# visinf/fldr-vfi

Hardware: AMD Instinct MI355X
Metric: 4K frame-pairs interpolated/sec (higher is better)
Workload: dtype f32 (3x3 convs: 3 x fp16-split MFMA with fp32 accumulation — error against fp64 within 1.5x (mean) / 2x (max) of the exact fp32-MFMA kernel's on every layer shape, tests/test_gpu_parity.py::test_split_fp16_conv_is_fp32_equivalent; rest fp32/fp64); 1 GPU; single 3840x2160 frame pair per step (padded 2304x3840), fLDRnet 5-scale test path (--papermodel --test5scales), t=0.5, shipped checkpoint weights, fp64 output frame; 4 distinct pairs per GPU rotated through the loop; parallelism=dp1 (independent pairs, no data-path collective), pairs_in_flight=3, distinct_pairs_per_gpu=4, setup_threads_per_rank=16, pyramid_bytes_per_pair=283046400

## Files before the change

fldr-vfi_amd/csrc/conv_ring_kernels.hip:

```cpp
#include "spk_common.h"

#ifndef RING_SLOTS
#define RING_SLOTS 3
#endif
#define RING_NLOAD 4
#define RING_RW_MAX_CHUNKS 4
#ifndef RING_RW_SLOTS
#define RING_RW_SLOTS 5
#endif
#ifndef RING_RW_INFLIGHT
#define RING_RW_INFLIGHT 2
#endif
#ifndef RING_NT_STORES
#define RING_NT_STORES 0
#endif
#ifndef RING_PD_THIN
#define RING_PD_THIN 1
#endif
#define RING_SPIN_LIMIT (1 << 21)
#ifndef RING_LOADER_PRIO
#define RING_LOADER_PRIO 0
#endif
#ifndef RING_FIN_PRIO
#define RING_FIN_PRIO 0
#endif

#ifdef RING_STAMPS
__device__ unsigned long long fldr_ring_stamp_buf[4 * 8];
__device__ unsigned long long fldr_ring_trace[4 * 24 * 4];
FLDR_HOOK int fldr_debug_read_ring_trace(unsigned long long* host) {
    return (int)hipMemcpyFromSymbol(host, HIP_SYMBOL(fldr_ring_trace), sizeof(unsigned long long) * 4 * 24 * 4);
}
#define RSTAMP(var) unsigned long long var; { __builtin_amdgcn_sched_barrier(0); asm volatile("s_memtime %0\n\ts_waitcnt lgkmcnt(0)" : "=s"(var) :: "memory"); __builtin_amdgcn_sched_barrier(0); }
FLDR_HOOK int fldr_debug_read_ring_stamps(unsigned long long* host) {
    return (int)hipMemcpyFromSymbol(host, HIP_SYMBOL(fldr_ring_stamp_buf), sizeof(unsigned long long) * 32);
}
#else
#define RSTAMP(var)
#endif

__device__ int fldr_ring_timeouts;
static int g_ring_spin_limit = RING_SPIN_LIMIT;
FLDR_HOOK int fldr_debug_ring_spin_limit(int v) {
    g_ring_spin_limit = v < 0 ? RING_SPIN_LIMIT : v;
    return g_ring_spin_limit;
}
FLDR_HOOK int fldr_debug_ring_timeouts(void) {
    int v = -1;
    if (hipMemcpyFromSymbol(&v, HIP_SYMBOL(fldr_ring_timeouts), sizeof(int)) != hipSuccess) return -1;
    return v;
}

FLDR_TU_STATUS(ring)
int fldr_ring_timeouts_read(int reset) {
    int v = -1;
    if (hipMemcpyFromSymbol(&v, HIP_SYMBOL(fldr_ring_timeouts), sizeof(int)) != hipSuccess) return -1;
    if (v > 0 && reset) { const int z = 0; if (hipMemcpyToSymbol(HIP_SYMBOL(fldr_ring_timeouts), &z, sizeof(int)) != hipSuccess) return -1; }
    return v;
}

template <int NMT, int TW = SPK_TW, bool RW = false>
struct RingCfg {
    static constexpr int W_BYTES = SPK_STEPS * NMT * 2 * 1024;
    static constexpr int NBLK = SPK_STEPS * NMT * 2;
    static constexpr int NWL = (NBLK + RING_NLOAD - 1) / RING_NLOAD;
    static constexpr int IW = TW + 2;
    static constexpr int CB = TW / 16;
    static constexpr int PLANE = (SPK_IH * IW * 16 + 255) / 256 * 256;
    static constexpr int NXI = (SPK_IH * IW + 63) / 64;
    static constexpr int K_DMA = (RW ? 0 : NWL) + NXI;
    static constexpr int IN_OFF = RW ? 0 : W_BYTES;
    static constexpr int STAGE = IN_OFF + 4 * PLANE;
    static constexpr int SLOTS = RW ? RING_RW_SLOTS : RING_SLOTS;
    static constexpr int INFLIGHT = RW ? RING_RW_INFLIGHT : 1;
    static constexpr int WRES_OFF = SLOTS * STAGE;
    static constexpr int CTR_OFF = WRES_OFF + (RW ? RING_RW_MAX_CHUNKS * W_BYTES : 0);
    static constexpr int BIAS_OFF = CTR_OFF + 64;
    static constexpr int LDS_BYTES = BIAS_OFF + 64 * NMT;
    static_assert(SLOTS <= 8 && INFLIGHT + 2 <= SLOTS && INFLIGHT * K_DMA <= 15, "ring shape");
    static_assert(TW == 16 || TW == 32, "tile width");
    static_assert(TW != SPK_TW || PLANE == SPK_PLANE, "the 32-pixel plane is the barrier pipeline's");
    static_assert(PLANE / 16 >= 64 && NXI * 64 >= SPK_IH * IW, "DMA pieces cover the plane");
    static_assert(K_DMA <= 15, "counted vmcnt wait uses the 4 low bits");
    static_assert(LDS_BYTES <= 160 * 1024, "ring does not fit the LDS");
};

__device__ __forceinline__ uint32_t ring_peek(uint32_t lds_addr) {
    uint32_t v;
    asm volatile("ds_read_b32 %0, %1\n\ts_waitcnt lgkmcnt(0)" : "=v"(v) : "v"(lds_addr) : "memory");
    return (uint32_t)__builtin_amdgcn_readfirstlane((int)v);
}

__device__ __forceinline__ void ring_wait_ge(uint32_t lds_addr, uint32_t target, int& limit) {
    if (ring_peek(lds_addr) >= target) return;
    bool landed = false;
    for (int spins = 0; spins < limit && !landed; spins += 8) {
#pragma unroll
        for (int j = 0; j < 8; ++j) {
            __builtin_amdgcn_s_sleep(1);
            if (ring_peek(lds_addr) >= target) { landed = true; break; }
        }
    }
#ifndef RING_AB_NOFAULT
    if (!landed) limit = -1;
#endif
}
__device__ __forceinline__ void ring_report_fault(int lane) {
    if (lane == 0) {
        atomicAdd(&fldr_ring_timeouts, 1);
        fldr_status_raise_ring();
    }
}

__device__ __forceinline__ void ring_signal(uint32_t lds_addr, int lane) {
    __builtin_amdgcn_sched_barrier(0);
    if (lane == 0) asm volatile("ds_add_u32 %0, %1" :: "v"(lds_addr), "v"(1u) : "memory");
    __builtin_amdgcn_sched_barrier(0);
}

template <int NMT, int TERMS, bool HAS_RES, int NC, int TW, bool ML = false, bool RW = false>
__global__ __launch_bounds__((NC + RING_NLOAD) * 64) void conv3x3_ring_kernel(SpkArgs a) {
    using Cfg = RingCfg<NMT, TW, RW>;
    constexpr int SLOTS = Cfg::SLOTS;
    constexpr int CB = Cfg::CB;
    constexpr int RING_NCONS = NC;
    constexpr int MTOT = 16 * NMT;
    extern __shared__ __attribute__((aligned(256))) unsigned char smem[];
    const int tid = threadIdx.x, lane = tid & 63;
    const int wave = __builtin_amdgcn_readfirstlane(tid >> 6);
    const int n_chunks = a.n_chunks;
    const uint32_t ctr = (uint32_t)(uintptr_t)(klptr_t)(smem + Cfg::CTR_OFF);
#ifdef RING_AB_CONSTLIMIT
    int spin_limit = RING_SPIN_LIMIT;
#else
    int spin_limit = a.spin_limit;
#endif

    if (tid < 16) reinterpret_cast<uint32_t*>(smem + Cfg::CTR_OFF)[tid] = 0u;
    if (tid >= 64 && tid < 64 + 16 * NMT) {
        const int u0 = (blockIdx.x & 7) * a.units_per_xcd + (blockIdx.x >> 3);
        int co = (u0 % a.groups) * 16 * NMT + (tid - 64);
        co = co < a.cout ? co : a.cout - 1;
        reinterpret_cast<float*>(smem + Cfg::BIAS_OFF)[tid - 64] = a.bias ? a.bias[co] : 0.0f;
    }
    const int xcd = blockIdx.x & 7, slot_id = blockIdx.x >> 3;
    const int u_end = min((xcd + 1) * a.units_per_xcd, a.n_units);
    const int u_first = xcd * a.units_per_xcd + slot_id;
    if constexpr (RW) {
        const int g0 = (u_first < a.n_units ? u_first : 0) % a.groups;
        const int sub = a.pack_nmt / NMT, pgrp = g0 / sub, msel = (g0 - pgrp * sub) * NMT;
        const int pack_w_bytes = SPK_STEPS * a.pack_nmt * 2 * 1024;
        const char* wsrc = reinterpret_cast<const char*>(a.wpack + SPK_HDR) + (int64_t)pgrp * n_chunks * pack_w_bytes;
        for (int b = wave; b < n_chunks * Cfg::NBLK; b += NC + RING_NLOAD) {
            const int c = b / Cfg::NBLK, blk = b - c * Cfg::NBLK;
            const int step = blk / (2 * NMT), mk = blk - step * 2 * NMT;
            __builtin_amdgcn_global_load_lds((kgptr_t)(wsrc + (int64_t)c * pack_w_bytes + ((step * a.pack_nmt + msel) * 2 + mk) * 1024 + lane * 16),
                                             (klptr_t)(smem + Cfg::WRES_OFF + c * Cfg::W_BYTES + blk * 1024), 16, 0, 0);
        }
        __builtin_amdgcn_s_waitcnt(0x0F70);
    }
    __syncthreads();
    if (u_first >= u_end) return;
    const int my_units = (u_end - u_first + a.wgs_per_xcd - 1) / a.wgs_per_xcd;
    const int total = my_units * n_chunks;
    const int grp0 = u_first % a.groups;

    if (wave >= RING_NCONS) {
        __builtin_amdgcn_s_setprio(RING_LOADER_PRIO);
        const int lw = wave - RING_NCONS;
        const int ip = lw, ikind = ip >> 1, igrp = ip & 1;
        const char* zero_blk = reinterpret_cast<const char*>(a.wpack + 4);
        const int sub = a.pack_nmt / NMT;
        const int pgrp = grp0 / sub, msel = (grp0 - pgrp * sub) * NMT;
        const int pack_w_bytes = SPK_STEPS * a.pack_nmt * 2 * 1024;
        int w_blk[Cfg::NWL], x_piece[Cfg::NXI];
        uint32_t w_voff[Cfg::NWL];
#pragma unroll
        for (int i = 0; i < Cfg::NWL; ++i) {
            w_blk[i] = min(lw * Cfg::NWL + i, Cfg::NBLK - 1);
            const int step = w_blk[i] / (2 * NMT), mk = w_blk[i] - step * 2 * NMT;
            w_voff[i] = (uint32_t)((step * a.pack_nmt + msel) * 2 + mk) * 1024u + (uint32_t)lane * 16u;
        }
#pragma unroll
        for (int i = 0; i < Cfg::NXI; ++i) x_piece[i] = min(i * 64, Cfg::PLANE / 16 - 64);
        unsigned long long tab_ptr;
        long long tab_bs;
        {
            const auto* kt = (const __attribute__((address_space(4))) unsigned long long*)__builtin_amdgcn_kernarg_segment_ptr();
            const int l = lane < SPK_MAX_GROUPS ? lane : 0;
            unsigned long long e = kt[l];
            tab_bs = (long long)kt[SPK_MAX_GROUPS + l];
            const bool up2 = (e & 1ull) != 0ull;
            const long long plane = up2 ? (long long)(a.H >> 1) * (a.W >> 1) * 16 : (long long)a.H * a.W * 16;
            if (e != 0ull && ikind) e += (unsigned long long)plane;
            tab_ptr = e;
        }
        int iss_u = u_first, iss_c = 0, iss_n = 0;
        uint32_t g_full[Cfg::NXI], g_half[Cfg::NXI];
        unsigned long long ml_base = 0ull;
        long long ml_plane = 0;
        auto issue_geometry = [&]() {
            int uH = a.H, uW = a.W, tiles_x = a.tiles_x, tile, ty;
            const int t = spk_div(iss_u, a.m_groups, a.groups);
            if constexpr (ML) {
                int l = 0;
                for (int k = 1; k < a.n_levels; ++k) l = t * a.groups >= a.lv[k].unit0 ? k : l;
                uH = a.lv[l].H; uW = a.lv[l].W; tiles_x = a.lv[l].tiles_x;
                tile = t - a.lv[l].unit0 / a.groups;
                iss_n = 0;
                ml_base = a.grp_ptr[0] + (unsigned long long)a.lv[l].in_off;
                ml_plane = (long long)uH * uW * 16;
                ty = tile / tiles_x;
            } else {
                iss_n = spk_div(t, a.m_tiles, a.n_tiles);
                tile = t - iss_n * a.n_tiles;
                ty = spk_div(tile, a.m_tiles_x, a.tiles_x);
            }
            const int oy0 = ty * SPK_TH, ox0 = (tile - ty * tiles_x) * TW;
#pragma unroll
            for (int i = 0; i < Cfg::NXI; ++i) {
                const int e = x_piece[i] + lane;
                const int y = e / Cfg::IW, x = e % Cfg::IW;
                const int gy = oy0 - 1 + y, gx = ox0 - 1 + x;
                const bool ok = e < SPK_IH * Cfg::IW && gy >= 0 && gy < uH && gx >= 0 && gx < uW;
                g_full[i] = ok ? (uint32_t)(gy * uW + gx) * 16u : ~0u;
                g_half[i] = ok ? (uint32_t)((gy >> 1) * (uW >> 1) + (gx >> 1)) * 16u : ~0u;
            }
        };
        const char* const iss_w = reinterpret_cast<const char*>(a.wpack + SPK_HDR) + (int64_t)pgrp * n_chunks * pack_w_bytes;
        issue_geometry();
        int st = 0;
        uint32_t free_target = 0;
#ifdef RING_STAMPS
        unsigned long long ls_prep = 0, ls_free = 0, ls_fire = 0, ls_land = 0;
        RSTAMP(l_begin)
#endif
        for (int k = 0; k < total; ++k) {
            RSTAMP(l0)
            const char* wbase = iss_w + (int64_t)iss_c * pack_w_bytes;
            const int gi = iss_c * 2 + igrp;
            const uint32_t e_lo = __builtin_amdgcn_readlane((int)(uint32_t)tab_ptr, gi), e_hi = __builtin_amdgcn_readlane((int)(uint32_t)(tab_ptr >> 32), gi);
            const uint32_t b_lo = __builtin_amdgcn_readlane((int)(uint32_t)tab_bs, gi), b_hi = __builtin_amdgcn_readlane((int)(uint32_t)((unsigned long long)tab_bs >> 32), gi);
            unsigned long long e = ((unsigned long long)e_hi << 32) | e_lo;
            const long long bs = (long long)(((unsigned long long)b_hi << 32) | b_lo);
            if constexpr (ML) e = e == 0ull ? 0ull : ml_base + (unsigned long long)((2 * gi + ikind) * ml_plane);
            const bool nul = e == 0ull, up2 = (e & 1ull) != 0ull;
            const char* base = reinterpret_cast<const char*>(static_cast<uintptr_t>(e & ~1ull)) + (int64_t)iss_n * bs;
            const char* dptr[Cfg::NXI];
#pragma unroll
            for (int i = 0; i < Cfg::NXI; ++i) {
                const uint32_t off = up2 ? g_half[i] : g_full[i];
                dptr[i] = (off != ~0u && !nul) ? base + off : zero_blk;
            }
            if (++iss_c == n_chunks) { iss_c = 0; iss_u += a.wgs_per_xcd; if (iss_u < u_end) issue_geometry(); }
            RSTAMP(l1)
            if (free_target) ring_wait_ge(ctr + 32 + 4 * st, free_target, spin_limit);
            if (spin_limit < 0) break;
            RSTAMP(l2)
            unsigned char* stage = smem + st * Cfg::STAGE;
#if defined(RING_ABLATE) && RING_ABLATE == 3
            if (k >= SLOTS) { wbase = reinterpret_cast<const char*>(a.wpack + SPK_HDR); for (int i = 0; i < Cfg::NXI; ++i) dptr[i] = zero_blk; }
#endif
            if constexpr (!RW) {
#pragma unroll
                for (int i = 0; i < Cfg::NWL; ++i)
                    __builtin_amdgcn_global_load_lds((kgptr_t)(wbase + w_voff[i]), (klptr_t)(stage + w_blk[i] * 1024), 16, 0, 0);
            }
#pragma unroll
            for (int i = 0; i < Cfg::NXI; ++i)
                __builtin_amdgcn_global_load_lds((kgptr_t)dptr[i], (klptr_t)(stage + Cfg::IN_OFF + ip * Cfg::PLANE + x_piece[i] * 16), 16, 0, 0);
            RSTAMP(l3)
            if (k >= Cfg::INFLIGHT) {
                __builtin_amdgcn_s_waitcnt(0x0F70 | (Cfg::INFLIGHT * Cfg::K_DMA));
                ring_signal(ctr + 4 * ((st + SLOTS - Cfg::INFLIGHT) % SLOTS), lane);
            }
            RSTAMP(l4)
#ifdef RING_STAMPS
            ls_prep += l1 - l0; ls_free += l2 - l1; ls_fire += l3 - l2; ls_land += l4 - l3;
            if (blockIdx.x == 0 && (lw == 0 || lw == 3) && lane == 0 && k < 24) {
                unsigned long long* tr = fldr_ring_trace + ((lw == 0 ? 2 : 3) * 24 + k) * 4;
                tr[0] = l1; tr[1] = l2; tr[2] = l3; tr[3] = l4;
            }
#endif
            if (++st == SLOTS) { st = 0; free_target += RING_NCONS; }
        }
        if (spin_limit < 0) { ring_report_fault(lane); __builtin_amdgcn_s_waitcnt(0x0F70); return; }
        if constexpr (Cfg::INFLIGHT == 2) {
            if (total >= 2) {
                __builtin_amdgcn_s_waitcnt(0x0F70 | Cfg::K_DMA);
                ring_signal(ctr + 4 * ((st + SLOTS - 2) % SLOTS), lane);
            }
        } else {
            static_assert(Cfg::INFLIGHT == 1, "drain sequence");
        }
        __builtin_amdgcn_s_waitcnt(0x0F70);
        ring_signal(ctr + 4 * ((st + SLOTS - 1) % SLOTS), lane);
#ifdef RING_STAMPS
        RSTAMP(l_end)
        if ((blockIdx.x == 0 || blockIdx.x == 101) && wave == RING_NCONS && lane == 0) {
            unsigned long long* o = fldr_ring_stamp_buf + ((blockIdx.x == 0 ? 0 : 2) + 1) * 8;
            o[0] = ls_prep; o[1] = ls_free; o[2] = ls_fire; o[3] = ls_land; o[5] = total; o[6] = l_end - l_begin;
        }
#endif
        return;
    }

    constexpr int ROWS = SPK_TH / NC;
    const int cw = wave;
    const int lj = lane & 15, lg = lane >> 4;
    constexpr int NQ = CB * ROWS;
    int boff[NQ];
#pragma unroll
    for (int q = 0; q < NQ; ++q)
        boff[q] = Cfg::IN_OFF + (lg & 1) * Cfg::PLANE + ((ROWS * cw + q / CB) * Cfg::IW + (q % CB) * 16 + lj) * 16;
    const int tap_sel = lg >> 1;
    f4 acc[NMT][NQ];
#pragma unroll
    for (int m = 0; m < NMT; ++m)
#pragma unroll
        for (int q = 0; q < NQ; ++q) acc[m][q] = f4{0.0f, 0.0f, 0.0f, 0.0f};
    int cur_u = u_first, cur_c = 0;
    const float inv_scale = a.wpack[0];
    int uH = a.H, uW = a.W;
    int64_t HW = (int64_t)a.H * a.W;
    uint32_t HW32 = (uint32_t)HW;
    int64_t u_spk_off = 0, u_f32_off = 0, u_res_off = 0;
    auto unit_decode = [&](int u, int& n, int& ty, int& tx) __attribute__((always_inline)) {
        const int t = spk_div(u, a.m_groups, a.groups);
        if constexpr (ML) {
            int l = 0;
            for (int k = 1; k < a.n_levels; ++k) l = t * a.groups >= a.lv[k].unit0 ? k : l;
            uH = a.lv[l].H; uW = a.lv[l].W; HW = (int64_t)uH * uW; HW32 = (uint32_t)HW;
            u_spk_off = a.lv[l].out_spk_off; u_f32_off = a.lv[l].out_f32_off; u_res_off = a.lv[l].res_off;
            const int tile = t - a.lv[l].unit0 / a.groups;
            n = 0; ty = tile / a.lv[l].tiles_x; tx = tile - ty * a.lv[l].tiles_x;
        } else {
            n = spk_div(t, a.m_tiles, a.n_tiles);
            const int tile = t - n * a.n_tiles;
            ty = spk_div(tile, a.m_tiles_x, a.tiles_x); tx = tile - ty * a.tiles_x;
        }
    };
    const int gout = (a.cout_store + 7) >> 3;
    const int cbase = grp0 * MTOT;
    float bias_r[NMT][4];
#pragma unroll
    for (int m = 0; m < NMT; ++m) {
        const f4 bv = *reinterpret_cast<const f4*>(smem + Cfg::BIAS_OFF + (m * 16 + lg * 4) * 4);
#pragma unroll
        for (int r = 0; r < 4; ++r) bias_r[m][r] = bv[r];
    }
    auto bias_of = [&](int m) __attribute__((always_inline)) -> f4 { return f4{bias_r[m][0], bias_r[m][1], bias_r[m][2], bias_r[m][3]}; };
    auto unit_pixels = [&](int u, uint32_t (&po)[NQ], int& n) {
        int ty, tx;
        unit_decode(u, n, ty, tx);
        const int ox0 = tx * TW;
#pragma unroll
        for (int q = 0; q < NQ; ++q) {
            const int oy = ty * SPK_TH + ROWS * cw + q / CB;
            const int ox = ox0 + (q % CB) * 16 + lj;
            po[q] = (oy < uH && ox < uW) ? (uint32_t)(oy * uW + ox) : ~0u;
        }
    };
    float res_r[HAS_RES ? NMT : 1][HAS_RES ? NQ : 1][4];
    auto residual_prefetch = [&]() {
        uint32_t po[NQ]; int n;
        unit_pixels(cur_u, po, n);
        if (a.res_spk) {
            const char* resn = reinterpret_cast<const char*>(a.residual) + u_res_off + (int64_t)n * ((a.cout_store + 7) >> 3) * 2 * HW * 16;
#pragma unroll
            for (int m = 0; m < NMT; ++m)
#pragma unroll
                for (int q = 0; q < NQ; ++q) {
                    int co0 = cbase + m * 16 + lg * 4;
                    co0 = co0 < a.cout_store ? co0 : 0;
                    const uint32_t off = ((uint32_t)(co0 >> 3) * 2u * HW32 + (po[q] != ~0u ? po[q] : 0u)) * 16u + (uint32_t)((co0 >> 2) & 1) * 8u;
                    const h4 hi = *reinterpret_cast<const h4*>(resn + off), lo = *reinterpret_cast<const h4*>(resn + (off + HW32 * 16u));
#pragma unroll
                    for (int r = 0; r < 4; ++r) res_r[HAS_RES ? m : 0][HAS_RES ? q : 0][r] = (float)hi[r] + (float)lo[r];
                }
            return;
        }
        const float* resn = reinterpret_cast<const float*>(reinterpret_cast<const char*>(a.residual) + u_res_off) + (int64_t)n * a.cout_store * HW;
#pragma unroll
        for (int m = 0; m < NMT; ++m)
#pragma unroll
            for (int q = 0; q < NQ; ++q)
#pragma unroll
                for (int r = 0; r < 4; ++r) {
                    int co = cbase + m * 16 + lg * 4 + r;
                    co = co < a.cout_store ? co : a.cout_store - 1;
                    res_r[HAS_RES ? m : 0][HAS_RES ? q : 0][r] = resn[(uint32_t)co * HW32 + (po[q] != ~0u ? po[q] : 0u)];
                }
    };
    const float relu_floor = a.relu ? 0.0f : -3.402823466e+38f;
    const bool grp_full = cbase + MTOT <= a.cout_store && !(a.cout_store & 7);
#ifdef RING_STAMPS
    unsigned long long cs_f_dec = 0, cs_f_fast = 0, cs_f_b0 = 0, fq0 = 0;
#endif
    auto finish_store = [&]() {
        RSTAMP(f0)
        int lj = lane & 15, lg = lane >> 4;
        asm volatile("" : "+v"(lj), "+v"(lg));
        int n, ty, tx;
        unit_decode(cur_u, n, ty, tx);
        const int oy0 = ty * SPK_TH + ROWS * cw, ox0 = tx * TW;
        char* outn = a.out_f32 ? reinterpret_cast<char*>(a.out_f32 + (int64_t)n * a.cout_store * HW) + u_f32_off : nullptr;
        char* spkn = a.out_spk ? reinterpret_cast<char*>(a.out_spk) + (int64_t)n * a.out_spk_bstride + u_spk_off : nullptr;
        const bool inside = oy0 + ROWS <= uH && ox0 + TW <= uW;
        const bool poisoned = spin_limit < 0;
        RSTAMP(f1)
        if (grp_full && inside) {
            const uint32_t p0 = (uint32_t)(oy0 * uW + ox0 + lj);
            float abs_sum = 0.0f;
#pragma unroll
            for (int q = 0; q < NQ; ++q)
#pragma unroll
                for (int m = 0; m < NMT; ++m) {
                    const f4 bsv = bias_of(m);
#pragma unroll
                    for (int r = 0; r < 4; ++r) {
                        float v = fmaxf(acc[m][q][r] * inv_scale + bsv[r], relu_floor);
                        if constexpr (HAS_RES) v += res_r[HAS_RES ? m : 0][HAS_RES ? q : 0][r];
                        acc[m][q][r] = v;
                        abs_sum += fabsf(v);
                    }
                }
            auto emit = [&](auto guardedc) __attribute__((always_inline)) {
                constexpr bool GUARDED = decltype(guardedc)::value;
                bool range_bad = false;
#pragma unroll
                for (int q = 0; q < NQ; ++q) {
                    const uint32_t pq = p0 + (uint32_t)((q / CB) * uW + (q % CB) * 16);
#ifdef RING_STAMPS
                    if (q == 1) { RSTAMP(fq) fq0 = fq; }
#endif
#pragma unroll
                    for (int m = 0; m < NMT; ++m) {
                        const int co0 = cbase + m * 16 + lg * 4;
                        float ov[4];
                        h4 ohi, olo;
#pragma unroll
                        for (int r = 0; r < 4; ++r) {
                            ov[r] = acc[m][q][r];
                            acc[m][q][r] = 0.0f;
                            _Float16 h, l;
                            if constexpr (GUARDED) spk_split(ov[r], h, l, range_bad); else fldr_split_plain(ov[r], h, l);
                            ohi[r] = h; olo[r] = l;
                        }
                        if (outn) {
                            const uint32_t off = ((uint32_t)co0 * HW32 + pq) * 4u;
#pragma unroll
                            for (int r = 0; r < 4; ++r) *reinterpret_cast<float*>(outn + (off + (uint32_t)r * HW32 * 4u)) = ov[r];
                        }
                        if (spkn) {
#if defined(RING_ABLATE) && RING_ABLATE == 6
                            asm volatile("" :: "v"(ohi), "v"(olo));
#else
                            const uint32_t off = ((uint32_t)(co0 >> 3) * 2u * HW32 + pq) * 16u + (uint32_t)(lg & 1) * 8u;
#if RING_NT_STORES
                            __builtin_nontemporal_store(ohi, reinterpret_cast<h4*>(spkn + off));
                            __builtin_nontemporal_store(olo, reinterpret_cast<h4*>(spkn + (off + HW32 * 16u)));
#else
                            *reinterpret_cast<h4*>(spkn + off) = ohi;
                            *reinterpret_cast<h4*>(spkn + (off + HW32 * 16u)) = olo;
#endif
#endif
                        }
                    }
                }
                if constexpr (GUARDED) { if (a.out_spk) fldr_note_range(range_bad); }
            };
            if (!poisoned) {
                if (fldr_guard_trips(abs_sum)) emit(std::true_type{}); else emit(std::false_type{});
#ifdef RING_STAMPS
                { RSTAMP(f2) cs_f_dec += f1 - f0; cs_f_fast += f2 - f1; cs_f_b0 += fq0 - f1; }
#endif
                return;
            }
        }
        uint32_t po[NQ];
#pragma unroll
        for (int q = 0; q < NQ; ++q) {
            const int oy = oy0 + q / CB, ox = ox0 + (q % CB) * 16 + lj;
            po[q] = (oy < uH && ox < uW) ? (uint32_t)(oy * uW + ox) : ~0u;
        }
        const bool quads = !(a.cout_store & 3);
        bool range_bad = false;
#pragma unroll
        for (int q = 0; q < NQ; ++q)
#pragma unroll
            for (int m = 0; m < NMT; ++m) {
                const int co0 = cbase + m * 16 + lg * 4;
                float ov[4];
                h4 ohi, olo;
                const f4 bsv = bias_of(m);
                float xs[4];
#pragma unroll
                for (int r = 0; r < 4; ++r) {
                    float v = fmaxf(acc[m][q][r] * inv_scale + bsv[r], relu_floor);
                    if constexpr (HAS_RES) v += res_r[HAS_RES ? m : 0][HAS_RES ? q : 0][r];
                    ov[r] = v;
                    acc[m][q][r] = 0.0f;
                    xs[r] = co0 + r < a.cout_store ? v : 0.0f;
                }
                {
                    _Float16 h[4], l[4];
                    fldr_split_hl_group(xs, h, l, range_bad);
#pragma unroll
                    for (int r = 0; r < 4; ++r) { ohi[r] = h[r]; olo[r] = l[r]; }
                }
                if (poisoned) {
#pragma unroll
                    for (int r = 0; r < 4; ++r) { ov[r] = __builtin_nanf(""); ohi[r] = (_Float16)__builtin_nanf(""); olo[r] = (_Float16)__builtin_nanf(""); }
                }
                if (outn) {
                    const uint32_t off = ((uint32_t)co0 * HW32 + po[q]) * 4u;
                    if (quads) {
                        if (co0 < a.cout_store && po[q] != ~0u) {
#pragma unroll
                            for (int r = 0; r < 4; ++r) *reinterpret_cast<float*>(outn + (off + (uint32_t)r * HW32 * 4u)) = ov[r];
                        }
                    } else {
#pragma unroll
                        for (int r = 0; r < 4; ++r)
                            if (co0 + r < a.cout_store && po[q] != ~0u) *reinterpret_cast<float*>(outn + (off + (uint32_t)r * HW32 * 4u)) = ov[r];
                    }
                }
                if (spkn) {
                    const int go = co0 >> 3;
                    if (go < gout && po[q] != ~0u) {
                        const uint32_t off = ((uint32_t)go * 2u * HW32 + po[q]) * 16u + (uint32_t)(lg & 1) * 8u;
                        *reinterpret_cast<h4*>(spkn + off) = ohi;
                        *reinterpret_cast<h4*>(spkn + (off + HW32 * 16u)) = olo;
                    }
                }
            }
        if (a.out_spk && spin_limit >= 0) fldr_note_range(range_bad);
    };

    int st_cur = 0;
    uint32_t full_target = RING_NLOAD;
#ifdef RING_STAMPS
    unsigned long long cs_wait = 0, cs_steps = 0, cs_fin = 0;
    RSTAMP(c_begin)
#endif
    auto steps = [&]() __attribute__((always_inline)) {
        const unsigned char* sb = smem + st_cur * Cfg::STAGE;
        const unsigned char* win = (RW ? smem + Cfg::WRES_OFF + cur_c * Cfg::W_BYTES : sb) + lane * 16;
        constexpr int PD = (NMT == 1 && TERMS == 3) ? RING_PD_THIN : 1;
        constexpr int NB = PD + 1;
        h8 bh[NB][NQ], bl[NB][NQ], ah[NB][NMT], al[PD > 1 ? NB : 1][NMT];
        auto tap_off = [&](int s) {
            const int tA = 2 * s, tB = 2 * s + 1 < 9 ? 2 * s + 1 : 8;
            const int offA = ((tA / 3) * Cfg::IW + tA % 3) * 16, offB = ((tB / 3) * Cfg::IW + tB % 3) * 16;
            return tap_sel ? offB : offA;
        };
        auto ld_bh = [&](int buf, int s) {
            const int toff = tap_off(s);
#pragma unroll
            for (int q = 0; q < NQ; ++q) bh[buf][q] = *reinterpret_cast<const h8*>(sb + boff[q] + toff);
        };
        auto ld_ah = [&](int buf, int s) {
#pragma unroll
            for (int m = 0; m < NMT; ++m) ah[buf][m] = *reinterpret_cast<const h8*>(win + ((s * NMT + m) * 2 + 0) * 1024);
        };
        auto ld_bl = [&](int buf, int s) {
            if constexpr (TERMS > 1) {
                const int toff = tap_off(s);
#pragma unroll
                for (int q = 0; q < NQ; ++q) bl[buf][q] = *reinterpret_cast<const h8*>(sb + 2 * Cfg::PLANE + boff[q] + toff);
            }
        };
        auto ld_al = [&](int s, int buf = 0) {
            if constexpr (TERMS > 1) {
#pragma unroll
                for (int m = 0; m < NMT; ++m) al[buf][m] = *reinterpret_cast<const h8*>(win + ((s * NMT + m) * 2 + 1) * 1024);
            }
        };
        auto ld = [&](int buf, int s) { ld_bh(buf, s); ld_ah(buf, s); ld_bl(buf, s); };
        constexpr int N_MFMA = NQ * TERMS * NMT, N_DS = TERMS > 1 ? 2 * NQ + 2 * NMT : NQ + NMT;
#ifdef RING_NTAIL
        constexpr int N_TAIL = N_MFMA >= 12 ? RING_NTAIL : (N_MFMA >= 6 ? 2 : 0);
#else
        constexpr int N_TAIL = N_MFMA >= 12 ? 4 : (N_MFMA >= 6 ? 2 : 0);
#endif
        ld(0, 0);
        ld_al(0);
        if constexpr (PD > 1) { ld(1, 1); ld_al(1, 1); }
        __builtin_amdgcn_sched_barrier(0);
#pragma unroll
        for (int s = 0; s < SPK_STEPS; ++s) {
#if defined(RING_ABLATE) && RING_ABLATE == 1
            if (s + 1 < SPK_STEPS) { for (int q = 0; q < NQ; ++q) { bh[(s + 1) & 1][q] = bh[s & 1][q]; bl[(s + 1) & 1][q] = bl[s & 1][q]; }
                                              for (int m = 0; m < NMT; ++m) { ah[(s + 1) & 1][m] = ah[s & 1][m]; } }
#else
            if constexpr (PD > 1) {
                if (s + PD < SPK_STEPS) { ld((s + PD) % NB, s + PD); ld_al(s + PD, (s + PD) % NB); }
            } else {
                if (s > 0) ld_al(s);
                if (s + 1 < SPK_STEPS) ld((s + 1) & 1, s + 1);
            }
#endif
#pragma unroll
            for (int term = 0; term < TERMS; ++term) {
#pragma unroll
                for (int m = 0; m < NMT; ++m)
#pragma unroll
                    for (int q = 0; q < NQ; ++q) {
                        const h8 av = term == 2 ? al[PD > 1 ? s % NB : 0][m] : ah[s % NB][m];
                        const h8 bv = term == 1 ? bl[s % NB][q] : bh[s % NB][q];
#if defined(RING_ABLATE) && RING_ABLATE == 2
                        asm volatile("" :: "v"(av), "v"(bv));
#else
                        acc[m][q] = __builtin_amdgcn_mfma_f32_16x16x32_f16(av, bv, acc[m][q], 0, 0, 0);
#endif
                    }
            }
            spk_step_pattern_n<N_MFMA, N_DS, N_TAIL, 0>(s + PD < SPK_STEPS);
        }
    };
    int g = 0;
#ifdef RING_STAMPS
    unsigned long long c0 = 0, c1 = 0, c2 = 0;
#endif
    auto iter_begin = [&]() __attribute__((always_inline)) {
#ifdef RING_STAMPS
        { RSTAMP(t) c0 = t; }
#endif
#if defined(RING_ABLATE) && RING_ABLATE == 5
        if (g < SLOTS)
#endif
        ring_wait_ge(ctr + 4 * st_cur, full_target, spin_limit);
#ifdef RING_STAMPS
        { RSTAMP(t) c1 = t; }
#endif
    };
    auto iter_end = [&]() __attribute__((always_inline)) {
        if (spin_limit >= 0) ring_signal(ctr + 32 + 4 * st_cur, lane);
#ifdef RING_STAMPS
        { RSTAMP(t) c2 = t; }
#endif
    };
    auto iter_close = [&]() __attribute__((always_inline)) {
#ifdef RING_STAMPS
        RSTAMP(c3)
        cs_wait += c1 - c0; cs_steps += c2 - c1; cs_fin += c3 - c2;
        if (blockIdx.x == 0 && (wave == 0 || wave == 4) && lane == 0 && g < 24) {
            unsigned long long* tr = fldr_ring_trace + ((wave == 0 ? 0 : 1) * 24 + g) * 4;
            tr[0] = c0; tr[1] = c1; tr[2] = c2; tr[3] = c3;
        }
#endif
        if (++st_cur == SLOTS) { st_cur = 0; full_target += RING_NLOAD; }
        ++g;
    };
    while (g < total) {
        const bool last = cur_c == n_chunks - 1;
        if constexpr (HAS_RES) { if (last) residual_prefetch(); }
        iter_begin();
        steps();
        iter_end();
        if (last) {
            if constexpr (HAS_RES) __builtin_amdgcn_s_waitcnt(0x0F70);
            if (RING_FIN_PRIO) __builtin_amdgcn_s_setprio(RING_FIN_PRIO);
#if defined(RING_ABLATE) && RING_ABLATE == 4
            for (int m = 0; m < NMT; ++m) for (int q = 0; q < NQ; ++q) { asm volatile("" :: "v"(acc[m][q])); acc[m][q] = f4{0.0f, 0.0f, 0.0f, 0.0f}; }
            cur_c = 0; cur_u += a.wgs_per_xcd;
            iter_close();
#else
            finish_store();
            cur_c = 0; cur_u += a.wgs_per_xcd;
            iter_close();
#endif
            if (RING_FIN_PRIO) __builtin_amdgcn_s_setprio(0);
        } else {
            ++cur_c;
            iter_close();
        }
    }
    if (spin_limit < 0) ring_report_fault(lane);
#ifdef RING_STAMPS
    RSTAMP(c_end)
    if ((blockIdx.x == 0 || blockIdx.x == 101) && wave == 0 && lane == 0) {
        unsigned long long* o = fldr_ring_stamp_buf + (blockIdx.x == 0 ? 0 : 2) * 8;
        o[0] = cs_wait; o[1] = cs_steps; o[2] = cs_fin; o[3] = cs_f_dec; o[4] = cs_f_fast; o[7] = cs_f_b0; o[5] = total; o[6] = c_end - c_begin;
    }
#endif
}

struct Ring32Cfg {
    static constexpr int NBLK = 18;
    static constexpr int W_BYTES = NBLK * 1024;
    static constexpr int NWL = (NBLK + RING_NLOAD - 1) / RING_NLOAD;
    static constexpr int IW = SPK_TW + 2;
    static constexpr int PLANE = SPK_IH * IW * 16;
    static constexpr int NXI = (SPK_IH * IW + 63) / 64;
    static constexpr int K_DMA = NWL + NXI;
    static constexpr int STAGE = W_BYTES + 4 * PLANE;
    static constexpr int SLOTS = 4;
    static constexpr int CTR_OFF = SLOTS * STAGE;
    static constexpr int BIAS_OFF = CTR_OFF + 64;
    static constexpr int LDS_BYTES = BIAS_OFF + 128;
    static_assert(K_DMA <= 15 && LDS_BYTES <= 160 * 1024, "ring32 shape");
};

__global__ __launch_bounds__((8 + RING_NLOAD) * 64) void conv3x3_ring32_kernel(SpkArgs a) {
    using Cfg = Ring32Cfg;
    constexpr int SLOTS = Cfg::SLOTS, NC = 8;
    extern __shared__ __attribute__((aligned(256))) unsigned char smem[];
    const int tid = threadIdx.x, lane = tid & 63;
    const int wave = __builtin_amdgcn_readfirstlane(tid >> 6);
    const int n_chunks = a.n_chunks;
    const uint32_t ctr = (uint32_t)(uintptr_t)(klptr_t)(smem + Cfg::CTR_OFF);
#ifdef RING_AB_CONSTLIMIT
    int spin_limit = RING_SPIN_LIMIT;
#else
    int spin_limit = a.spin_limit;
#endif
    if (tid < 16) reinterpret_cast<uint32_t*>(smem + Cfg::CTR_OFF)[tid] = 0u;
    if (tid >= 64 && tid < 96) {
        const int u0 = (blockIdx.x & 7) * a.units_per_xcd + (blockIdx.x >> 3);
        const int co = (u0 % a.groups) * 32 + (tid - 64);
        reinterpret_cast<float*>(smem + Cfg::BIAS_OFF)[tid - 64] = (a.bias && co < a.cout) ? a.bias[co] : 0.0f;
    }
    __syncthreads();
    const int xcd = blockIdx.x & 7, slot_id = blockIdx.x >> 3;
    const int u_end = min((xcd + 1) * a.units_per_xcd, a.n_units);
    const int u_first = xcd * a.units_per_xcd + slot_id;
    if (u_first >= u_end) return;
    const int my_units = (u_end - u_first + a.wgs_per_xcd - 1) / a.wgs_per_xcd;
    const int total = my_units * n_chunks;
    const int grp0 = u_first % a.groups;

    if (wave >= NC) {
        const int lw = wave - NC;
        const int ip = lw, ikind = ip >> 1, igrp = ip & 1;
        const char* zero_blk = reinterpret_cast<const char*>(a.wpack + 4);
        int w_blk[Cfg::NWL], x_piece[Cfg::NXI];
#pragma unroll
        for (int i = 0; i < Cfg::NWL; ++i) w_blk[i] = min(lw * Cfg::NWL + i, Cfg::NBLK - 1);
#pragma unroll
        for (int i = 0; i < Cfg::NXI; ++i) x_piece[i] = min(i * 64, Cfg::PLANE / 16 - 64);
        unsigned long long tab_ptr;
        long long tab_bs;
        {
            const auto* kt = (const __attribute__((address_space(4))) unsigned long long*)__builtin_amdgcn_kernarg_segment_ptr();
            const int l = lane < SPK_MAX_GROUPS ? lane : 0;
            unsigned long long e = kt[l];
            tab_bs = (long long)kt[SPK_MAX_GROUPS + l];
            const bool up2 = (e & 1ull) != 0ull;
            const long long plane = up2 ? (long long)(a.H >> 1) * (a.W >> 1) * 16 : (long long)a.H * a.W * 16;
            if (e != 0ull && ikind) e += (unsigned long long)plane;
            tab_ptr = e;
        }
        int iss_u = u_first, iss_c = 0, iss_n = 0;
        uint32_t g_full[Cfg::NXI], g_half[Cfg::NXI];
        auto issue_geometry = [&]() {
            const int t = spk_div(iss_u, a.m_groups, a.groups);
            iss_n = spk_div(t, a.m_tiles, a.n_tiles);
            const int tile = t - iss_n * a.n_tiles;
            const int ty = spk_div(tile, a.m_tiles_x, a.tiles_x);
            const int oy0 = ty * SPK_TH, ox0 = (tile - ty * a.tiles_x) * SPK_TW;
#pragma unroll
            for (int i = 0; i < Cfg::NXI; ++i) {
                const int e = x_piece[i] + lane;
                const int y = e / Cfg::IW, x = e % Cfg::IW;
                const int gy = oy0 - 1 + y, gx = ox0 - 1 + x;
                const bool ok = gy >= 0 && gy < a.H && gx >= 0 && gx < a.W;
                g_full[i] = ok ? (uint32_t)(gy * a.W + gx) * 16u : ~0u;
                g_half[i] = ok ? (uint32_t)((gy >> 1) * (a.W >> 1) + (gx >> 1)) * 16u : ~0u;
            }
        };
        const char* const iss_w = reinterpret_cast<const char*>(a.wpack) + a.w32_off + (int64_t)grp0 * n_chunks * Cfg::W_BYTES;
        issue_geometry();
        int st = 0;
        uint32_t free_target = 0;
        for (int k = 0; k < total; ++k) {
            const char* wbase = iss_w + (int64_t)iss_c * Cfg::W_BYTES + lane * 16;
            const int gi = iss_c * 2 + igrp;
            const uint32_t e_lo = __builtin_amdgcn_readlane((int)(uint32_t)tab_ptr, gi), e_hi = __builtin_amdgcn_readlane((int)(uint32_t)(tab_ptr >> 32), gi);
            const uint32_t b_lo = __builtin_amdgcn_readlane((int)(uint32_t)tab_bs, gi), b_hi = __builtin_amdgcn_readlane((int)(uint32_t)((unsigned long long)tab_bs >> 32), gi);
            const unsigned long long e = ((unsigned long long)e_hi << 32) | e_lo;
            const long long bs = (long long)(((unsigned long long)b_hi << 32) | b_lo);
            const bool nul = e == 0ull, up2 = (e & 1ull) != 0ull;
            const char* base = reinterpret_cast<const char*>(static_cast<uintptr_t>(e & ~1ull)) + (int64_t)iss_n * bs;
            const char* dptr[Cfg::NXI];
#pragma unroll
            for (int i = 0; i < Cfg::NXI; ++i) {
                const uint32_t off = up2 ? g_half[i] : g_full[i];
                dptr[i] = (off != ~0u && !nul) ? base + off : zero_blk;
            }
            if (++iss_c == n_chunks) { iss_c = 0; iss_u += a.wgs_per_xcd; if (iss_u < u_end) issue_geometry(); }
            if (free_target) ring_wait_ge(ctr + 32 + 4 * st, free_target, spin_limit);
            if (spin_limit < 0) break;
            unsigned char* stage = smem + st * Cfg::STAGE;
#pragma unroll
            for (int i = 0; i < Cfg::NWL; ++i)
                __builtin_amdgcn_global_load_lds((kgptr_t)(wbase + w_blk[i] * 1024), (klptr_t)(stage + w_blk[i] * 1024), 16, 0, 0);
#pragma unroll
            for (int i = 0; i < Cfg::NXI; ++i)
                __builtin_amdgcn_global_load_lds((kgptr_t)dptr[i], (klptr_t)(stage + Cfg::W_BYTES + ip * Cfg::PLANE + x_piece[i] * 16), 16, 0, 0);
            if (k > 0) {
                __builtin_amdgcn_s_waitcnt(0x0F70 | Cfg::K_DMA);
                ring_signal(ctr + 4 * ((st + SLOTS - 1) % SLOTS), lane);
            }
            if (++st == SLOTS) { st = 0; free_target += NC; }
        }
        if (spin_limit < 0) { ring_report_fault(lane); __builtin_amdgcn_s_waitcnt(0x0F70); return; }
        __builtin_amdgcn_s_waitcnt(0x0F70);
        ring_signal(ctr + 4 * ((st + SLOTS - 1) % SLOTS), lane);
        return;
    }

    typedef float f16v __attribute__((ext_vector_type(16)));
    const int cw = wave;
    const int lj = lane & 31, lh = lane >> 5;
    const uint32_t b_lane = (uint32_t)(Cfg::W_BYTES + lh * Cfg::PLANE + (cw * Cfg::IW + lj) * 16);
    f16v acc;
#pragma unroll
    for (int r = 0; r < 16; ++r) acc[r] = 0.0f;
    int cur_u = u_first, cur_c = 0;
    const float inv_scale = a.wpack[0];
    const int64_t HW = (int64_t)a.H * a.W;
    const uint32_t HW32 = (uint32_t)HW;
    float bias_r[16];
#pragma unroll
    for (int r = 0; r < 16; ++r) bias_r[r] = reinterpret_cast<const float*>(smem + Cfg::BIAS_OFF)[(r & 3) + 8 * (r >> 2) + 4 * lh];
    const float relu_floor = a.relu ? 0.0f : -3.402823466e+38f;
    auto finish_store = [&]() {
        const int t = spk_div(cur_u, a.m_groups, a.groups);
        const int n = spk_div(t, a.m_tiles, a.n_tiles);
        const int tile = t - n * a.n_tiles;
        const int ty = spk_div(tile, a.m_tiles_x, a.tiles_x), tx = tile - ty * a.tiles_x;
        const int oy = ty * SPK_TH + cw, ox = tx * SPK_TW + lj;
        const bool ok = oy < a.H && ox < a.W;
        unsigned char* spkn = a.out_spk + (int64_t)n * a.out_spk_bstride;
        const uint32_t pq = ok ? (uint32_t)(oy * a.W + ox) : 0u;
        float abs_sum = 0.0f;
#pragma unroll
        for (int r = 0; r < 16; ++r) {
            acc[r] = fmaxf(acc[r] * inv_scale + bias_r[r], relu_floor);
            abs_sum += fabsf(acc[r]);
        }
        const bool poisoned = spin_limit < 0;
        const bool guard = fldr_guard_trips(abs_sum);
        bool bad = false;
#pragma unroll
        for (int r0 = 0; r0 < 16; r0 += 4) {
            const int co0 = grp0 * 32 + 8 * (r0 >> 2) + 4 * lh;
            h4 ohi, olo;
#pragma unroll
            for (int r = 0; r < 4; ++r) {
                const float v = acc[r0 + r];
                acc[r0 + r] = 0.0f;
                _Float16 h, l;
                if (guard) spk_split(v, h, l, bad); else fldr_split_plain(v, h, l);
                ohi[r] = h; olo[r] = l;
            }
            if (poisoned) {
#pragma unroll
                for (int r = 0; r < 4; ++r) { ohi[r] = (_Float16)__builtin_nanf(""); olo[r] = (_Float16)__builtin_nanf(""); }
            }
            if (ok) {
                const uint32_t off = ((uint32_t)(co0 >> 3) * 2u * HW32 + pq) * 16u + (uint32_t)lh * 8u;
                *reinterpret_cast<h4*>(spkn + off) = ohi;
                *reinterpret_cast<h4*>(spkn + (off + HW32 * 16u)) = olo;
            }
        }
        if (guard && !poisoned) fldr_note_range(bad);
    };
    int st_cur = 0, g = 0;
    uint32_t full_target = RING_NLOAD;
    while (g < total) {
        const bool last = cur_c == n_chunks - 1;
        ring_wait_ge(ctr + 4 * st_cur, full_target, spin_limit);
        {
            const unsigned char* sb = smem + st_cur * Cfg::STAGE;
            const unsigned char* wb = sb + lane * 16;
            const unsigned char* xb = sb + b_lane;
            h8 Ah[3], Al[3], Bh[3], Bl[3];
            auto ld = [&](int t) __attribute__((always_inline)) {
                const int off = ((t / 3) * Cfg::IW + t % 3) * 16;
                Ah[t % 3] = *reinterpret_cast<const h8*>(wb + (2 * t) * 1024);
                Al[t % 3] = *reinterpret_cast<const h8*>(wb + (2 * t + 1) * 1024);
                Bh[t % 3] = *reinterpret_cast<const h8*>(xb + off);
                Bl[t % 3] = *reinterpret_cast<const h8*>(xb + 2 * Cfg::PLANE + off);
            };
            ld(0); ld(1);
            __builtin_amdgcn_sched_barrier(0);
#pragma unroll
            for (int t = 0; t < 9; ++t) {
                if (t + 2 < 9) ld(t + 2);
                acc = __builtin_amdgcn_mfma_f32_32x32x16_f16(Ah[t % 3], Bh[t % 3], acc, 0, 0, 0);
                acc = __builtin_amdgcn_mfma_f32_32x32x16_f16(Ah[t % 3], Bl[t % 3], acc, 0, 0, 0);
                acc = __builtin_amdgcn_mfma_f32_32x32x16_f16(Al[t % 3], Bh[t % 3], acc, 0, 0, 0);
                __builtin_amdgcn_sched_barrier(0);
            }
        }
        if (spin_limit >= 0) ring_signal(ctr + 32 + 4 * st_cur, lane);
        if (last) { finish_store(); cur_c = 0; cur_u += a.wgs_per_xcd; } else ++cur_c;
        if (++st_cur == SLOTS) { st_cur = 0; full_target += RING_NLOAD; }
        ++g;
    }
    if (spin_limit < 0) ring_report_fault(lane);
}

#ifdef FLDR_TEST_HOOKS
template <int NMT>
struct RingRowCfg {
    static constexpr int NBLK = 3 * NMT * 2;
    static constexpr int W_BYTES = NBLK * 1024;
    static constexpr int NWL = (NBLK + RING_NLOAD - 1) / RING_NLOAD;
    static constexpr int IW = SPK_TW + 2;
    static constexpr int PLANE = SPK_TH * IW * 16;
    static constexpr int NXI = (SPK_TH * IW + 63) / 64;
    static constexpr int K_DMA = NWL + 2 * NXI;
    static constexpr int STAGE = W_BYTES + 8 * PLANE;
    static constexpr int SLOTS = 3;
    static constexpr int CTR_OFF = SLOTS * STAGE;
    static constexpr int BIAS_OFF = CTR_OFF + 64;
    static constexpr int LDS_BYTES = BIAS_OFF + 64 * NMT;
    static_assert(K_DMA <= 15 && LDS_BYTES <= 160 * 1024 && PLANE % 256 == 0, "ring-row shape");
};

template <int NMT>
__global__ __launch_bounds__((8 + RING_NLOAD) * 64) void conv3x3_ringrow_kernel(SpkArgs a, const float* __restrict__ wrow) {
    using Cfg = RingRowCfg<NMT>;
    constexpr int SLOTS = Cfg::SLOTS, NC = 8, NQ = 2;
    extern __shared__ __attribute__((aligned(256))) unsigned char smem[];
    const int tid = threadIdx.x, lane = tid & 63;
    const int wave = __builtin_amdgcn_readfirstlane(tid >> 6);
    const int n32 = a.n_chunks;
    const int n_items = 3 * n32;
    const uint32_t ctr = (uint32_t)(uintptr_t)(klptr_t)(smem + Cfg::CTR_OFF);
#ifdef RING_AB_CONSTLIMIT
    int spin_limit = RING_SPIN_LIMIT;
#else
    int spin_limit = a.spin_limit;
#endif
    if (tid < 16) reinterpret_cast<uint32_t*>(smem + Cfg::CTR_OFF)[tid] = 0u;
    if (tid >= 64 && tid < 64 + 16 * NMT) {
        const int u0 = (blockIdx.x & 7) * a.units_per_xcd + (blockIdx.x >> 3);
        const int co = (u0 % a.groups) * 16 * NMT + (tid - 64);
        reinterpret_cast<float*>(smem + Cfg::BIAS_OFF)[tid - 64] = (a.bias && co < a.cout) ? a.bias[co] : 0.0f;
    }
    __syncthreads();
    const int xcd = blockIdx.x & 7, slot_id = blockIdx.x >> 3;
    const int u_end = min((xcd + 1) * a.units_per_xcd, a.n_units);
    const int u_first = xcd * a.units_per_xcd + slot_id;
    if (u_first >= u_end) return;
    const int my_units = (u_end - u_first + a.wgs_per_xcd - 1) / a.wgs_per_xcd;
    const int total = my_units * n_items;
    const int grp0 = u_first % a.groups;

    if (wave >= NC) {
        const int lw = wave - NC;
        const char* zero_blk = reinterpret_cast<const char*>(a.wpack + 4);
        int w_blk[Cfg::NWL], x_piece[Cfg::NXI];
#pragma unroll
        for (int i = 0; i < Cfg::NWL; ++i) w_blk[i] = min(lw * Cfg::NWL + i, Cfg::NBLK - 1);
#pragma unroll
        for (int i = 0; i < Cfg::NXI; ++i) x_piece[i] = min(i * 64, Cfg::PLANE / 16 - 64);
        unsigned long long tab_ptr;
        long long tab_bs;
        {
            const auto* kt = (const __attribute__((address_space(4))) unsigned long long*)__builtin_amdgcn_kernarg_segment_ptr();
            const int l = lane < SPK_MAX_GROUPS ? lane : 0;
            tab_ptr = kt[l];
            tab_bs = (long long)kt[SPK_MAX_GROUPS + l];
        }
        int iss_u = u_first, iss_i = 0, iss_n = 0;
        int gy0[Cfg::NXI], gx0[Cfg::NXI];
        auto issue_geometry = [&]() {
            const int t = spk_div(iss_u, a.m_groups, a.groups);
            iss_n = spk_div(t, a.m_tiles, a.n_tiles);
            const int tile = t - iss_n * a.n_tiles;
            const int ty = spk_div(tile, a.m_tiles_x, a.tiles_x);
            const int oy0 = ty * SPK_TH, ox0 = (tile - ty * a.tiles_x) * SPK_TW;
#pragma unroll
            for (int i = 0; i < Cfg::NXI; ++i) {
                const int e = x_piece[i] + lane;
                const int y = e / Cfg::IW, x = e - y * Cfg::IW;
                gy0[i] = oy0 - 1 + y; gx0[i] = ox0 - 1 + x;
            }
        };
        const char* const iss_w = reinterpret_cast<const char*>(wrow) + (int64_t)grp0 * n_items * Cfg::W_BYTES;
        issue_geometry();
        int st = 0;
        uint32_t free_target = 0;
        for (int k = 0; k < total; ++k) {
            const int c32 = iss_i / 3, dy = iss_i - 3 * c32;
            const char* wbase = iss_w + (int64_t)iss_i * Cfg::W_BYTES + lane * 16;
            const int gi = c32 * 4 + lw;
            const uint32_t e_lo = __builtin_amdgcn_readlane((int)(uint32_t)tab_ptr, gi), e_hi = __builtin_amdgcn_readlane((int)(uint32_t)(tab_ptr >> 32), gi);
            const uint32_t b_lo = __builtin_amdgcn_readlane((int)(uint32_t)tab_bs, gi), b_hi = __builtin_amdgcn_readlane((int)(uint32_t)((unsigned long long)tab_bs >> 32), gi);
            const unsigned long long e = ((unsigned long long)e_hi << 32) | e_lo;
            const long long bs = (long long)(((unsigned long long)b_hi << 32) | b_lo);
            const bool nul = e == 0ull, up2 = (e & 1ull) != 0ull;
            const char* base = reinterpret_cast<const char*>(static_cast<uintptr_t>(e & ~1ull)) + (int64_t)iss_n * bs;
            const long long plane_b = up2 ? (long long)(a.H >> 1) * (a.W >> 1) * 16 : (long long)a.H * a.W * 16;
            const char* dhi[Cfg::NXI];
            const char* dlo[Cfg::NXI];
#pragma unroll
            for (int i = 0; i < Cfg::NXI; ++i) {
                const int gy = gy0[i] + dy, gx = gx0[i];
                const bool ok = !nul && gy >= 0 && gy < a.H && gx >= 0 && gx < a.W;
                const uint32_t off = up2 ? (uint32_t)((gy >> 1) * (a.W >> 1) + (gx >> 1)) * 16u : (uint32_t)(gy * a.W + gx) * 16u;
                dhi[i] = ok ? base + off : zero_blk;
                dlo[i] = ok ? base + plane_b + off : zero_blk;
            }
            if (++iss_i == n_items) { iss_i = 0; iss_u += a.wgs_per_xcd; if (iss_u < u_end) issue_geometry(); }
            if (free_target) ring_wait_ge(ctr + 32 + 4 * st, free_target, spin_limit);
            if (spin_limit < 0) break;
            unsigned char* stage = smem + st * Cfg::STAGE;
#pragma unroll
            for (int i = 0; i < Cfg::NWL; ++i)
                __builtin_amdgcn_global_load_lds((kgptr_t)(wbase + w_blk[i] * 1024), (klptr_t)(stage + w_blk[i] * 1024), 16, 0, 0);
#pragma unroll
            for (int i = 0; i < Cfg::NXI; ++i) {
                __builtin_amdgcn_global_load_lds((kgptr_t)dhi[i], (klptr_t)(stage + Cfg::W_BYTES + lw * Cfg::PLANE + x_piece[i] * 16), 16, 0, 0);
                __builtin_amdgcn_global_load_lds((kgptr_t)dlo[i], (klptr_t)(stage + Cfg::W_BYTES + (4 + lw) * Cfg::PLANE + x_piece[i] * 16), 16, 0, 0);
            }
            if (k > 0) {
                __builtin_amdgcn_s_waitcnt(0x0F70 | Cfg::K_DMA);
                ring_signal(ctr + 4 * ((st + SLOTS - 1) % SLOTS), lane);
            }
            if (++st == SLOTS) { st = 0; free_target += NC; }
        }
        if (spin_limit < 0) { ring_report_fault(lane); __builtin_amdgcn_s_waitcnt(0x0F70); return; }
        __builtin_amdgcn_s_waitcnt(0x0F70);
        ring_signal(ctr + 4 * ((st + SLOTS - 1) % SLOTS), lane);
        return;
    }

    const int cw = wave;
    const int lj = lane & 15, lg = lane >> 4;
    int boff[NQ];
#pragma unroll
    for (int q = 0; q < NQ; ++q) boff[q] = Cfg::W_BYTES + lg * Cfg::PLANE + (cw * Cfg::IW + q * 16 + lj) * 16;
    f4 acc[NMT][NQ];
#pragma unroll
    for (int m = 0; m < NMT; ++m)
#pragma unroll
        for (int q = 0; q < NQ; ++q) acc[m][q] = f4{0.0f, 0.0f, 0.0f, 0.0f};
    int cur_u = u_first, cur_i = 0;
    const float inv_scale = a.wpack[0];
    const int64_t HW = (int64_t)a.H * a.W;
    const uint32_t HW32 = (uint32_t)HW;
    float bias_r[NMT][4];
#pragma unroll
    for (int m = 0; m < NMT; ++m) {
        const f4 bv = *reinterpret_cast<const f4*>(smem + Cfg::BIAS_OFF + (m * 16 + lg * 4) * 4);
#pragma unroll
        for (int r = 0; r < 4; ++r) bias_r[m][r] = bv[r];
    }
    const float relu_floor = a.relu ? 0.0f : -3.402823466e+38f;
    auto finish_store = [&]() {
        const int t = spk_div(cur_u, a.m_groups, a.groups);
        const int n = spk_div(t, a.m_tiles, a.n_tiles);
        const int tile = t - n * a.n_tiles;
        const int ty = spk_div(tile, a.m_tiles_x, a.tiles_x), tx = tile - ty * a.tiles_x;
        const int oy = ty * SPK_TH + cw;
        unsigned char* spkn = a.out_spk + (int64_t)n * a.out_spk_bstride;
        float abs_sum = 0.0f;
#pragma unroll
        for (int m = 0; m < NMT; ++m)
#pragma unroll
            for (int q = 0; q < NQ; ++q)
#pragma unroll
                for (int r = 0; r < 4; ++r) {
                    acc[m][q][r] = fmaxf(acc[m][q][r] * inv_scale + bias_r[m][r], relu_floor);
                    abs_sum += fabsf(acc[m][q][r]);
                }
        const bool guard = fldr_guard_trips(abs_sum);
        const bool poisoned = spin_limit < 0;
        bool bad = false;
#pragma unroll
        for (int q = 0; q < NQ; ++q) {
            const int ox = tx * SPK_TW + q * 16 + lj;
            const bool ok = oy < a.H && ox < a.W;
            const uint32_t pq = ok ? (uint32_t)(oy * a.W + ox) : 0u;
#pragma unroll
            for (int m = 0; m < NMT; ++m) {
                const int co0 = grp0 * 16 * NMT + m * 16 + lg * 4;
                h4 ohi, olo;
#pragma unroll
                for (int r = 0; r < 4; ++r) {
                    const float v = acc[m][q][r];
                    acc[m][q][r] = 0.0f;
                    _Float16 h, l;
                    if (guard) spk_split(v, h, l, bad); else fldr_split_plain(v, h, l);
                    ohi[r] = h; olo[r] = l;
                }
                if (poisoned) {
#pragma unroll
                    for (int r = 0; r < 4; ++r) { ohi[r] = (_Float16)__builtin_nanf(""); olo[r] = (_Float16)__builtin_nanf(""); }
                }
                if (ok) {
                    const uint32_t off = ((uint32_t)(co0 >> 3) * 2u * HW32 + pq) * 16u + (uint32_t)(lg & 1) * 8u;
                    *reinterpret_cast<h4*>(spkn + off) = ohi;
                    *reinterpret_cast<h4*>(spkn + (off + HW32 * 16u)) = olo;
                }
            }
        }
        if (guard && !poisoned) fldr_note_range(bad);
    };
    int st_cur = 0, g = 0;
    uint32_t full_target = RING_NLOAD;
    while (g < total) {
        const bool last = cur_i == n_items - 1;
        ring_wait_ge(ctr + 4 * st_cur, full_target, spin_limit);
        {
            const unsigned char* sb = smem + st_cur * Cfg::STAGE;
            const unsigned char* win = sb + lane * 16;
            h8 bh[2][NQ], bl[2][NQ], ah[2][NMT], al[NMT];
            auto ld = [&](int buf, int s) __attribute__((always_inline)) {
#pragma unroll
                for (int q = 0; q < NQ; ++q) bh[buf][q] = *reinterpret_cast<const h8*>(sb + boff[q] + s * 16);
#pragma unroll
                for (int m = 0; m < NMT; ++m) ah[buf][m] = *reinterpret_cast<const h8*>(win + ((s * NMT + m) * 2 + 0) * 1024);
#pragma unroll
                for (int q = 0; q < NQ; ++q) bl[buf][q] = *reinterpret_cast<const h8*>(sb + 4 * Cfg::PLANE + boff[q] + s * 16);
            };
            auto ld_al = [&](int s) __attribute__((always_inline)) {
#pragma unroll
                for (int m = 0; m < NMT; ++m) al[m] = *reinterpret_cast<const h8*>(win + ((s * NMT + m) * 2 + 1) * 1024);
            };
            constexpr int N_MFMA = NQ * 3 * NMT, N_DS = 2 * NQ + 2 * NMT;
            constexpr int N_TAIL = N_MFMA >= 12 ? 4 : 2;
            ld(0, 0);
            ld_al(0);
            __builtin_amdgcn_sched_barrier(0);
#pragma unroll
            for (int s = 0; s < 3; ++s) {
                if (s > 0) ld_al(s);
                if (s + 1 < 3) ld((s + 1) & 1, s + 1);
#pragma unroll
                for (int term = 0; term < 3; ++term)
#pragma unroll
                    for (int m = 0; m < NMT; ++m)
#pragma unroll
                        for (int q = 0; q < NQ; ++q) {
                            const h8 av = term == 2 ? al[m] : ah[s & 1][m];
                            const h8 bv = term == 1 ? bl[s & 1][q] : bh[s & 1][q];
                            acc[m][q] = __builtin_amdgcn_mfma_f32_16x16x32_f16(av, bv, acc[m][q], 0, 0, 0);
                        }
                spk_step_pattern_n<N_MFMA, N_DS, N_TAIL, 0>(s + 1 < 3);
            }
        }
        if (spin_limit >= 0) ring_signal(ctr + 32 + 4 * st_cur, lane);
        if (last) { finish_store(); cur_i = 0; cur_u += a.wgs_per_xcd; } else ++cur_i;
        if (++st_cur == SLOTS) { st_cur = 0; full_target += RING_NLOAD; }
        ++g;
    }
    if (spin_limit < 0) ring_report_fault(lane);
}

__global__ void ringrow_prepack_kernel(const float* __restrict__ w, const float* __restrict__ hdr, float* __restrict__ dst, int cout, int cin, int nmt,
                                       int n32, int64_t total_h8) {
    const int64_t i = (int64_t)blockIdx.x * 256 + threadIdx.x;
    if (i >= total_h8) return;
    const float scale = hdr[1];
    const int lane = (int)(i % 64), kind = (int)((i / 64) % 2), m = (int)((i / 128) % nmt), dx = (int)((i / (128 * nmt)) % 3);
    const int dy = (int)((i / (128 * nmt * 3)) % 3), c32 = (int)((i / (128 * nmt * 9)) % n32), gr = (int)(i / ((int64_t)128 * nmt * 9 * n32));
    const int co = gr * 16 * nmt + m * 16 + (lane & 15);
    h8 v;
#pragma unroll
    for (int j = 0; j < 8; ++j) {
        const int c = c32 * 32 + (lane >> 4) * 8 + j;
        const float x = (co < cout && c < cin) ? w[((int64_t)co * cin + c) * 9 + dy * 3 + dx] * scale : 0.0f;
        const _Float16 h = (_Float16)x;
        v[j] = kind == 0 ? h : (_Float16)(x - (float)h);
    }
    reinterpret_cast<h8*>(dst)[i] = v;
}
FLDR_HOOK int64_t fldr_debug_ringrow_pack_floats(int cout, int cin) {
    if (cin % 32 || (cout % 48 && cout % 32)) return FLDR_E_SHAPE;
    const int nmt = cout % 48 == 0 ? 3 : 2;
    return (int64_t)(cout / (16 * nmt)) * (cin / 32) * 9 * nmt * 2 * 256;
}
FLDR_HOOK int fldr_debug_ringrow_prepack(const float* weight, const float* wpack, float* wrow, int cout, int cin, fldr_stream_t stream) {
    const int64_t nf = fldr_debug_ringrow_pack_floats(cout, cin);
    if (nf < 0) return (int)nf;
    const int nmt = cout % 48 == 0 ? 3 : 2;
    hipLaunchKernelGGL(ringrow_prepack_kernel, dim3(fldr_cdiv(nf / 4, 256)), dim3(256), 0, fldr_s(stream), weight, wpack, wrow, cout, cin, nmt, cin / 32, nf / 4);
    FLDR_LAUNCH_RET();
}
template <int NMT>
static int ringrow_launch(SpkArgs& a, const float* wrow, int N, int wgs_per_xcd_max, hipStream_t s) {
    using Cfg = RingRowCfg<NMT>;
    static std::atomic<uint64_t> attr_done{0};
    if (int e = fldr_set_max_lds(reinterpret_cast<const void*>(&conv3x3_ringrow_kernel<NMT>), Cfg::LDS_BYTES, attr_done)) return e;
    a.groups = a.cout / (16 * NMT);
    if (int e = spk_fill_geometry(a, N, wgs_per_xcd_max, SPK_TW)) return e;
    a.spin_limit = g_ring_spin_limit;
    hipLaunchKernelGGL(conv3x3_ringrow_kernel<NMT>, dim3(8 * a.wgs_per_xcd), dim3((8 + RING_NLOAD) * 64), Cfg::LDS_BYTES, s, a, wrow);
    FLDR_LAUNCH_RET();
}
int fldr_spk_ringrow_dispatch(SpkArgs& a, const float* wrow, int N, int wgs_per_xcd_max, hipStream_t s) {
    if (a.cout % 48 == 0) { a.n_chunks = a.n_chunks / 2; return ringrow_launch<3>(a, wrow, N, wgs_per_xcd_max, s); }
    a.n_chunks = a.n_chunks / 2;
    return ringrow_launch<2>(a, wrow, N, wgs_per_xcd_max, s);
}
#endif

static int g_ring_consumers = 8;
FLDR_HOOK int fldr_debug_ring_consumers(int v) { if (v == 4 || v == 8) g_ring_consumers = v; return g_ring_consumers; }

template <int NMT, int TERMS, bool HAS_RES, int NC, int TW, bool RW = false>
static int ring_launch3(SpkArgs& a, int N, int wgs_per_xcd_max, hipStream_t s, int walk_h) {
    using Cfg = RingCfg<NMT, TW, RW>;
    static std::atomic<uint64_t> attr_done{0};
    if (int e = fldr_set_max_lds(reinterpret_cast<const void*>(&conv3x3_ring_kernel<NMT, TERMS, HAS_RES, NC, TW, false, RW>), Cfg::LDS_BYTES, attr_done)) return e;
    if (int e = spk_fill_geometry(a, N, wgs_per_xcd_max, TW, walk_h)) return e;
    a.spin_limit = g_ring_spin_limit;
    hipLaunchKernelGGL((conv3x3_ring_kernel<NMT, TERMS, HAS_RES, NC, TW, false, RW>), dim3(8 * a.wgs_per_xcd), dim3((NC + RING_NLOAD) * 64), Cfg::LDS_BYTES, s, a);
    FLDR_LAUNCH_RET();
}

#ifndef RING_RW_DEFAULT
#define RING_RW_DEFAULT 0
#endif
#ifdef FLDR_TEST_HOOKS
static int g_ring_resident = RING_RW_DEFAULT;
FLDR_HOOK int fldr_debug_ring_resident(int v) { if (v == 0 || v == 1) g_ring_resident = v; return g_ring_resident; }
#endif

#ifndef RING_NARROW_COST
#define RING_NARROW_COST 0.65
#endif
static int g_ring_tile_width = 0;
FLDR_HOOK int fldr_debug_ring_tile_width(int v) { if (v == 0 || v == 16 || v == 32) g_ring_tile_width = v; return g_ring_tile_width; }

static int ring_pick_tile_width(const SpkArgs& a, int N, int wgs_per_xcd_max, int walk_h) {
    if (g_ring_tile_width) return g_ring_tile_width;
    const int64_t wgs = 8ll * wgs_per_xcd_max;
    const int64_t ty = fldr_cdiv(walk_h, SPK_TH);
    const int64_t u32 = (int64_t)N * fldr_cdiv(a.W, 32) * ty * a.groups, u16 = (int64_t)N * fldr_cdiv(a.W, 16) * ty * a.groups;
    if (u32 <= wgs / 2) return 32;
    const double c32 = (double)((u32 + wgs - 1) / wgs), c16 = (double)((u16 + wgs - 1) / wgs) * RING_NARROW_COST;
    return c16 < c32 ? 16 : 32;
}

template <int NMT, int TERMS, bool HAS_RES>
static int ring_launch2(SpkArgs& a, int N, int wpx, hipStream_t s, int walk_h) {
#ifdef FLDR_TEST_HOOKS
    if constexpr (NMT == 1 && TERMS == 3) {
        if (g_ring_resident && a.n_chunks <= RING_RW_MAX_CHUNKS && g_ring_tile_width != 16) {
            const int64_t units = (int64_t)N * fldr_cdiv(a.W, SPK_TW) * fldr_cdiv(walk_h, SPK_TH) * a.groups;
            if (g_ring_consumers == 4 || (g_ring_tile_width == 0 && units >= 32ll * wpx)) return ring_launch3<NMT, TERMS, HAS_RES, 4, 32, true>(a, N, wpx, s, walk_h);
            return ring_launch3<NMT, TERMS, HAS_RES, 8, 32, true>(a, N, wpx, s, walk_h);
        }
    }
#endif
    if (g_ring_consumers == 4) return ring_launch3<NMT, TERMS, HAS_RES, 4, 32>(a, N, wpx, s, walk_h);
    if constexpr (NMT == 1 && TERMS == 3) {
        const int64_t units = (int64_t)N * fldr_cdiv(a.W, SPK_TW) * fldr_cdiv(walk_h, SPK_TH) * a.groups;
        if (g_ring_consumers == 8 && g_ring_tile_width == 0 && units >= 32ll * wpx) return ring_launch3<NMT, TERMS, HAS_RES, 4, 32>(a, N, wpx, s, walk_h);
    }
    if constexpr (TERMS == 3) {
        if (ring_pick_tile_width(a, N, wpx, walk_h) == 16) return ring_launch3<NMT, TERMS, HAS_RES, 8, 16>(a, N, wpx, s, walk_h);
    }
    return ring_launch3<NMT, TERMS, HAS_RES, 8, 32>(a, N, wpx, s, walk_h);
}

template <int NMT, int TERMS>
static int ring_launch(SpkArgs& a, int N, int wpx, hipStream_t s, int walk_h) {
    return a.residual ? ring_launch2<NMT, TERMS, true>(a, N, wpx, s, walk_h) : ring_launch2<NMT, TERMS, false>(a, N, wpx, s, walk_h);
}

#ifndef RING32_DEFAULT
#define RING32_DEFAULT 1
#endif
static int g_ring32 = RING32_DEFAULT;
FLDR_HOOK int fldr_debug_ring32(int v) { if (v >= 0 && v <= 2) g_ring32 = v; return g_ring32; }
static int ring32_launch(SpkArgs& a, int N, int wgs_per_xcd_max, hipStream_t s, int walk_h) {
    static std::atomic<uint64_t> attr_done{0};
    if (int e = fldr_set_max_lds(reinterpret_cast<const void*>(&conv3x3_ring32_kernel), Ring32Cfg::LDS_BYTES, attr_done)) return e;
    a.groups = a.cout / 32;
    if (int e = spk_fill_geometry(a, N, wgs_per_xcd_max, SPK_TW, walk_h)) return e;
    a.spin_limit = g_ring_spin_limit;
    hipLaunchKernelGGL(conv3x3_ring32_kernel, dim3(8 * a.wgs_per_xcd), dim3((8 + RING_NLOAD) * 64), Ring32Cfg::LDS_BYTES, s, a);
    FLDR_LAUNCH_RET();
}

#ifndef RING32_ROUND_COST
#define RING32_ROUND_COST 0.8
#endif
static bool ring32_pays(const SpkArgs& a, int N, int wgs_per_xcd_max, int walk_h) {
    if (g_ring32 == 2) return true;
    if (a.cout != 96) return false;
    const int64_t wgs = 8ll * wgs_per_xcd_max, tx32 = fldr_cdiv(a.W, 32), ty = fldr_cdiv(walk_h, SPK_TH);
    const int64_t u48 = (int64_t)N * tx32 * ty * a.groups, u16 = (int64_t)N * fldr_cdiv(a.W, 16) * ty * a.groups, u32 = (int64_t)N * tx32 * ty * (a.cout / 32);
    if (u32 <= wgs) return false;
    const double c48 = (double)((u48 + wgs - 1) / wgs), c16 = (double)((u16 + wgs - 1) / wgs) * RING_NARROW_COST;
    const double c32 = (double)((u32 + wgs - 1) / wgs) * RING32_ROUND_COST;
    return c32 < (c48 < c16 ? c48 : c16);
}

int fldr_spk_ring_dispatch(SpkArgs& a, int N, int nmt, int terms, int wgs_per_xcd_max, hipStream_t s, int walk_h) {
    if (walk_h <= 0 || walk_h > a.H) walk_h = a.H;
    if (g_ring32 && terms == 3 && nmt >= 2 && a.w32_off && a.cout_store == a.cout && !a.residual && !a.out_f32 && a.out_spk && g_ring_consumers == 8 &&
        g_ring_tile_width == 0 && ring32_pays(a, N, wgs_per_xcd_max, walk_h))
        return ring32_launch(a, N, wgs_per_xcd_max, s, walk_h);
    if (terms == 1) {
        if (nmt == 1) return ring_launch<1, 1>(a, N, wgs_per_xcd_max, s, walk_h);
        if (nmt == 2) return ring_launch<2, 1>(a, N, wgs_per_xcd_max, s, walk_h);
        return ring_launch<3, 1>(a, N, wgs_per_xcd_max, s, walk_h);
    }
    if (nmt == 1) return ring_launch<1, 3>(a, N, wgs_per_xcd_max, s, walk_h);
    if (nmt == 2) return ring_launch<2, 3>(a, N, wgs_per_xcd_max, s, walk_h);
    return ring_launch<3, 3>(a, N, wgs_per_xcd_max, s, walk_h);
}

template <int NMT, int TERMS, bool HAS_RES>
static int ring_launch_levels(SpkArgs& a, int n_units, int wgs_per_xcd_max, hipStream_t s) {
    using Cfg = RingCfg<NMT, 32>;
    static std::atomic<uint64_t> attr_done{0};
    if (int e = fldr_set_max_lds(reinterpret_cast<const void*>(&conv3x3_ring_kernel<NMT, TERMS, HAS_RES, 8, 32, true>), Cfg::LDS_BYTES, attr_done)) return e;
    a.tiles_x = 1; a.n_tiles = 1; a.m_tiles = 0; a.m_tiles_x = 0;
    a.n_units = n_units;
    a.units_per_xcd = (a.n_units + 7) / 8;
    a.units_per_xcd = (a.units_per_xcd + a.groups - 1) / a.groups * a.groups;
    a.wgs_per_xcd = spk_right_size(a.units_per_xcd, wgs_per_xcd_max, a.groups);
    if (((int64_t)a.n_units + 8 * a.units_per_xcd) * a.groups >= (1ll << 32)) return FLDR_E_SHAPE;
    a.m_groups = (uint32_t)((1ull << 32) / (uint32_t)a.groups) + 1u;
    a.spin_limit = g_ring_spin_limit;
    hipLaunchKernelGGL((conv3x3_ring_kernel<NMT, TERMS, HAS_RES, 8, 32, true>), dim3(8 * a.wgs_per_xcd), dim3((8 + RING_NLOAD) * 64), Cfg::LDS_BYTES, s, a);
    FLDR_LAUNCH_RET();
}

int fldr_spk_ring_dispatch_levels(SpkArgs& a, int n_units, int nmt, int terms, int wgs_per_xcd_max, hipStream_t s) {
#define RING_LV(NMT_, T_) (a.residual ? ring_launch_levels<NMT_, T_, true>(a, n_units, wgs_per_xcd_max, s) : ring_launch_levels<NMT_, T_, false>(a, n_units, wgs_per_xcd_max, s))
    if (terms == 1) return nmt == 1 ? RING_LV(1, 1) : (nmt == 2 ? RING_LV(2, 1) : RING_LV(3, 1));
    return nmt == 1 ? RING_LV(1, 3) : (nmt == 2 ? RING_LV(2, 3) : RING_LV(3, 3));
#undef RING_LV
}
```

fldr-vfi_amd/csrc/conv_spk_kernels.hip:

```cpp
#include "common.h"
#include <hip/hip_fp16.h>

#ifdef SPK_STAMPS
__device__ unsigned long long fldr_spk_stamp_buf[4 * 8];
#define KSTAMP(var) unsigned long long var; { __builtin_amdgcn_sched_barrier(0); asm volatile("s_memtime %0\n\ts_waitcnt lgkmcnt(0)" : "=s"(var) :: "memory"); __builtin_amdgcn_sched_barrier(0); }
FLDR_HOOK int fldr_debug_read_spk_stamps(unsigned long long* host) {
    return (int)hipMemcpyFromSymbol(host, HIP_SYMBOL(fldr_spk_stamp_buf), sizeof(unsigned long long) * 32);
}
#else
#define KSTAMP(var)
#endif

#include "spk_common.h"
#include <mutex>

#ifdef FLDR_TEST_HOOKS
template <int NMT, int TERMS, bool HAS_RES>
__global__ __launch_bounds__(512, 2) void conv3x3_spk_kernel(SpkArgs a) {
    using Cfg = SpkCfg<NMT>;
    constexpr int MTOT = 16 * NMT;
    extern __shared__ __attribute__((aligned(256))) unsigned char smem[];
    const int tid = threadIdx.x, lane = tid & 63;
    const int wave = __builtin_amdgcn_readfirstlane(tid >> 6);
    const int lj = lane & 15, lg = lane >> 4;
    const int n_chunks = a.n_chunks;

    const int xcd = blockIdx.x & 7, slot = blockIdx.x >> 3;
    const int u_end = min((xcd + 1) * a.units_per_xcd, a.n_units);
    const int u_first = xcd * a.units_per_xcd + slot;
    if (u_first >= u_end) return;
    const int my_units = (u_end - u_first + a.wgs_per_xcd - 1) / a.wgs_per_xcd;
    const int total = my_units * n_chunks;

    const bool early = wave >= 4;
    if (early) __builtin_amdgcn_s_setprio(1);

    constexpr int K_DMA = Cfg::NWI + 3;
    const int ip = wave >> 1;
    const int ikind = ip >> 1, igrp = ip & 1;
    const char* zero_blk = reinterpret_cast<const char*>(a.wpack + 4);
    int w_piece[Cfg::NWI], x_piece[3];
    uint32_t w_voff[Cfg::NWI];
    const int grp0 = u_first % a.groups, sub = a.pack_nmt / NMT;
    const int pgrp = grp0 / sub, msel = (grp0 - pgrp * sub) * NMT;
    const int pack_w_bytes = SPK_STEPS * a.pack_nmt * 2 * 1024;
#pragma unroll
    for (int i = 0; i < Cfg::NWI; ++i) {
        w_piece[i] = min(i * 512 + wave * 64, Cfg::PIECES - 64);
        const int b = w_piece[i] >> 6, step = b / (2 * NMT), mk = b - step * 2 * NMT;
        w_voff[i] = (uint32_t)((step * a.pack_nmt + msel) * 2 + mk) * 1024u + (uint32_t)lane * 16u;
    }
#pragma unroll
    for (int i = 0; i < 3; ++i) x_piece[i] = min(((wave & 1) * 3 + i) * 64, SPK_PLANE / 16 - 64);
    unsigned long long tab_ptr;
    long long tab_bs;
    {
        const auto* kt = (const __attribute__((address_space(4))) unsigned long long*)__builtin_amdgcn_kernarg_segment_ptr();
        const int l = lane < SPK_MAX_GROUPS ? lane : 0;
        unsigned long long e = kt[l];
        tab_bs = (long long)kt[SPK_MAX_GROUPS + l];
        const bool up2 = (e & 1ull) != 0ull;
        const long long plane = up2 ? (long long)(a.H >> 1) * (a.W >> 1) * 16 : (long long)a.H * a.W * 16;
        if (e != 0ull && ikind) e += (unsigned long long)plane;
        tab_ptr = e;
    }
    int iss_u = u_first, iss_c = 0;
    uint32_t g_full[3], g_half[3];
    int iss_n = 0;
    const char* const iss_w = reinterpret_cast<const char*>(a.wpack + SPK_HDR) + (int64_t)pgrp * n_chunks * pack_w_bytes;
    auto issue_geometry = [&]() {
        const int t = spk_div(iss_u, a.m_groups, a.groups);
        iss_n = spk_div(t, a.m_tiles, a.n_tiles);
        const int tile = t - iss_n * a.n_tiles;
        const int ty = spk_div(tile, a.m_tiles_x, a.tiles_x);
        const int oy0 = ty * SPK_TH, ox0 = (tile - ty * a.tiles_x) * SPK_TW;
#pragma unroll
        for (int i = 0; i < 3; ++i) {
            const int e = x_piece[i] + lane;
            const int y = e / SPK_IW, x = e % SPK_IW;
            const int gy = oy0 - 1 + y, gx = ox0 - 1 + x;
            const bool ok = e < SPK_IH * SPK_IW && gy >= 0 && gy < a.H && gx >= 0 && gx < a.W;
            g_full[i] = ok ? (uint32_t)(gy * a.W + gx) * 16u : ~0u;
            g_half[i] = ok ? (uint32_t)((gy >> 1) * (a.W >> 1) + (gx >> 1)) * 16u : ~0u;
        }
    };
    const char* wbase = nullptr;
    const char* dptr[3];
    auto issue_prepare = [&]() {
        const bool live = iss_u < u_end;
#if defined(SPK_ABLATE) && (SPK_ABLATE == 4 || SPK_ABLATE == 5)
        wbase = reinterpret_cast<const char*>(a.wpack + SPK_HDR);
#else
        wbase = live ? iss_w + (int64_t)iss_c * pack_w_bytes : reinterpret_cast<const char*>(a.wpack + SPK_HDR);
#endif
        const int gi = live ? iss_c * 2 + igrp : 0;
        const uint32_t e_lo = __builtin_amdgcn_readlane((int)(uint32_t)tab_ptr, gi), e_hi = __builtin_amdgcn_readlane((int)(uint32_t)(tab_ptr >> 32), gi);
        const uint32_t b_lo = __builtin_amdgcn_readlane((int)(uint32_t)tab_bs, gi), b_hi = __builtin_amdgcn_readlane((int)(uint32_t)((unsigned long long)tab_bs >> 32), gi);
        const unsigned long long e = ((unsigned long long)e_hi << 32) | e_lo;
        const long long bs = (long long)(((unsigned long long)b_hi << 32) | b_lo);
        const bool nul = e == 0ull || !live, up2 = (e & 1ull) != 0ull;
        const char* base = reinterpret_cast<const char*>(static_cast<uintptr_t>(e & ~1ull)) + (int64_t)iss_n * bs;
#pragma unroll
        for (int i = 0; i < 3; ++i) {
#if defined(SPK_ABLATE) && (SPK_ABLATE == 3 || SPK_ABLATE == 5)
            dptr[i] = zero_blk;
#else
            const uint32_t off = up2 ? g_half[i] : g_full[i];
            dptr[i] = (off != ~0u && !nul) ? base + off : zero_blk;
#endif
        }
        if (live && ++iss_c == n_chunks) { iss_c = 0; iss_u += a.wgs_per_xcd; if (iss_u < u_end) issue_geometry(); }
    };
    auto issue_fire = [&](int j, unsigned char* stage) {
        if (j < Cfg::NWI) {
            const int jj = j < Cfg::NWI ? j : 0;
            __builtin_amdgcn_global_load_lds((kgptr_t)(wbase + w_voff[jj]), (klptr_t)(stage + w_piece[jj] * 16), 16, 0, 0);
        } else {
            const int jj = j >= Cfg::NWI ? j - Cfg::NWI : 0;
            __builtin_amdgcn_global_load_lds((kgptr_t)dptr[jj], (klptr_t)(stage + Cfg::W_BYTES + ip * SPK_PLANE + x_piece[jj] * 16), 16, 0, 0);
        }
    };

    int boff[2];
#pragma unroll
    for (int p = 0; p < 2; ++p) boff[p] = Cfg::W_BYTES + (lg & 1) * SPK_PLANE + (wave * SPK_IW + p * 16 + lj) * 16;
    const int tap_sel = lg >> 1;
    f4 acc[NMT][2];
#pragma unroll
    for (int m = 0; m < NMT; ++m)
#pragma unroll
        for (int p = 0; p < 2; ++p) acc[m][p] = f4{0.0f, 0.0f, 0.0f, 0.0f};
    int cur_u = u_first, cur_c = 0;
    const float inv_scale = a.wpack[0];
    const int64_t HW = (int64_t)a.H * a.W;
    const int gout = (a.cout_store + 7) >> 3;
    const int cbase = grp0 * MTOT;
    float bias_r[NMT][4];
#pragma unroll
    for (int m = 0; m < NMT; ++m)
#pragma unroll
        for (int r = 0; r < 4; ++r) {
            int co = cbase + m * 16 + lg * 4 + r;
            co = co < a.cout ? co : a.cout - 1;
            bias_r[m][r] = a.bias ? a.bias[co] : 0.0f;
        }

    float res_r[NMT][2][4];
    float ov[NMT][2][4];
    h4 ohi[NMT][2], olo[NMT][2];
    uint32_t st_po[2];
    int st_n = 0;
    const uint32_t HW32 = (uint32_t)HW;
    auto unit_pixels = [&](int u, uint32_t (&po)[2], int& n) {
        const int t = spk_div(u, a.m_groups, a.groups);
        n = spk_div(t, a.m_tiles, a.n_tiles);
        const int tile = t - n * a.n_tiles;
        const int ty = spk_div(tile, a.m_tiles_x, a.tiles_x);
        const int oy = ty * SPK_TH + wave;
        const int ox0 = (tile - ty * a.tiles_x) * SPK_TW;
#pragma unroll
        for (int p = 0; p < 2; ++p) {
            const int ox = ox0 + p * 16 + lj;
            po[p] = (oy < a.H && ox < a.W) ? (uint32_t)(oy * a.W + ox) : ~0u;
        }
    };
    auto residual_prefetch = [&]() {
        uint32_t po[2]; int n;
        unit_pixels(cur_u, po, n);
        const float* resn = a.residual + (int64_t)n * a.cout_store * HW;
#pragma unroll
        for (int m = 0; m < NMT; ++m)
#pragma unroll
            for (int p = 0; p < 2; ++p)
#pragma unroll
                for (int r = 0; r < 4; ++r) {
                    int co = cbase + m * 16 + lg * 4 + r;
                    co = co < a.cout_store ? co : a.cout_store - 1;
                    res_r[m][p][r] = resn[(uint32_t)co * HW32 + (po[p] != ~0u ? po[p] : 0u)];
                }
    };
    bool range_bad = false;
    auto finish = [&]() {
        unit_pixels(cur_u, st_po, st_n);
#pragma unroll
        for (int m = 0; m < NMT; ++m)
#pragma unroll
            for (int p = 0; p < 2; ++p) {
#pragma unroll
                for (int r = 0; r < 4; ++r) {
                    float v = acc[m][p][r] * inv_scale + bias_r[m][r];
                    if (a.relu) v = fmaxf(v, 0.0f);
                    if constexpr (HAS_RES) v += res_r[m][p][r];
                    ov[m][p][r] = v;
                    acc[m][p][r] = 0.0f;
                    const float x = cbase + m * 16 + lg * 4 + r < a.cout_store ? v : 0.0f;
                    _Float16 h, l;
                    spk_split(x, h, l, range_bad);
                    ohi[m][p][r] = h; olo[m][p][r] = l;
                }
            }
    };
    auto store = [&]() {
        if (a.out_f32) {
            char* outn = reinterpret_cast<char*>(a.out_f32 + (int64_t)st_n * a.cout_store * HW);
            const bool quads = !(a.cout_store & 3);
#pragma unroll
            for (int p = 0; p < 2; ++p)
#pragma unroll
                for (int m = 0; m < NMT; ++m) {
                    const int co0 = cbase + m * 16 + lg * 4;
                    const uint32_t off = ((uint32_t)co0 * HW32 + st_po[p]) * 4u;
                    if (quads) {
                        if (co0 < a.cout_store && st_po[p] != ~0u) {
#pragma unroll
                            for (int r = 0; r < 4; ++r) *reinterpret_cast<float*>(outn + (off + (uint32_t)r * HW32 * 4u)) = ov[m][p][r];
                        }
                    } else {
#pragma unroll
                        for (int r = 0; r < 4; ++r)
                            if (co0 + r < a.cout_store && st_po[p] != ~0u) *reinterpret_cast<float*>(outn + (off + (uint32_t)r * HW32 * 4u)) = ov[m][p][r];
                    }
                }
        }
        if (a.out_spk) {
            char* spkn = reinterpret_cast<char*>(a.out_spk) + (int64_t)st_n * a.out_spk_bstride;
#pragma unroll
            for (int p = 0; p < 2; ++p)
#pragma unroll
                for (int m = 0; m < NMT; ++m) {
                    const int go = (cbase + m * 16 + lg * 4) >> 3;
                    if (go < gout && st_po[p] != ~0u) {
                        const uint32_t off = ((uint32_t)go * 2u * HW32 + st_po[p]) * 16u + (uint32_t)(lg & 1) * 8u;
                        *reinterpret_cast<h4*>(spkn + off) = ohi[m][p];
                        *reinterpret_cast<h4*>(spkn + (off + HW32 * 16u)) = olo[m][p];
                    }
                }
        }
    };

    issue_geometry();
#pragma unroll
    for (int st = 0; st < 2; ++st) {
        issue_prepare();
#pragma unroll
        for (int j = 0; j < K_DMA; ++j) issue_fire(j, smem + st * Cfg::STAGE);
    }
    if (early) issue_prepare();
    __builtin_amdgcn_s_waitcnt(0x0F70);
    __builtin_amdgcn_s_barrier();

    int st_cur = 0, st_iss = 2;
    bool store_pending = false;
#ifdef SPK_STAMPS
    unsigned long long ks_top = 0, ks_steps = 0, ks_fin = 0, ks_wait = 0, ks_bar = 0;
    KSTAMP(k_begin)
#endif
    for (int g = 0; g < total; ++g) {
        KSTAMP(k0)
        const bool last = cur_c == n_chunks - 1;
        if (!early) {
#if !defined(SPK_ABLATE) || SPK_ABLATE != 7
            if (store_pending) { store(); store_pending = false; }
#endif
            issue_prepare();
        }
        if constexpr (HAS_RES) { if (last) residual_prefetch(); }
        unsigned char* sdst = smem + st_iss * Cfg::STAGE;
        const unsigned char* sb = smem + st_cur * Cfg::STAGE;
        const unsigned char* win = sb + lane * 16;
        h8 bh[2][2], bl[2][2], ah[2][NMT], al[2][NMT];
        auto ld = [&](int buf, int s) {
            const int tA = 2 * s, tB = 2 * s + 1 < 9 ? 2 * s + 1 : 8;
            const int offA = ((tA / 3) * SPK_IW + tA % 3) * 16, offB = ((tB / 3) * SPK_IW + tB % 3) * 16;
            const int toff = tap_sel ? offB : offA;
#pragma unroll
            for (int p = 0; p < 2; ++p) bh[buf][p] = *reinterpret_cast<const h8*>(sb + boff[p] + toff);
#pragma unroll
            for (int m = 0; m < NMT; ++m) ah[buf][m] = *reinterpret_cast<const h8*>(win + ((s * NMT + m) * 2 + 0) * 1024);
            if constexpr (TERMS > 1) {
#pragma unroll
                for (int p = 0; p < 2; ++p) bl[buf][p] = *reinterpret_cast<const h8*>(sb + 2 * SPK_PLANE + boff[p] + toff);
#pragma unroll
                for (int m = 0; m < NMT; ++m) al[buf][m] = *reinterpret_cast<const h8*>(win + ((s * NMT + m) * 2 + 1) * 1024);
            }
        };
        constexpr int N_MFMA = 2 * TERMS * NMT, N_DS = TERMS > 1 ? 4 + 2 * NMT : 2 + NMT;
        constexpr int N_TAIL = N_MFMA >= 12 ? 4 : (N_MFMA >= 6 ? 2 : 0);
        KSTAMP(k1)
        ld(0, 0);
        __builtin_amdgcn_sched_barrier(0);
#pragma unroll
        for (int s = 0; s < SPK_STEPS; ++s) {
            const int j0 = (s * K_DMA + SPK_STEPS - 1) / SPK_STEPS, j1 = ((s + 1) * K_DMA + SPK_STEPS - 1) / SPK_STEPS;
#pragma unroll
            for (int j = 0; j < K_DMA; ++j)
                if (j >= j0 && j < j1) issue_fire(j, sdst);
#if defined(SPK_ABLATE) && SPK_ABLATE == 1
            if (s + 1 < SPK_STEPS) { for (int p = 0; p < 2; ++p) { bh[(s + 1) & 1][p] = bh[s & 1][p]; bl[(s + 1) & 1][p] = bl[s & 1][p]; }
                                    for (int m = 0; m < NMT; ++m) { ah[(s + 1) & 1][m] = ah[s & 1][m]; al[(s + 1) & 1][m] = al[s & 1][m]; } }
#else
            if (s + 1 < SPK_STEPS) ld((s + 1) & 1, s + 1);
#endif
#pragma unroll
            for (int term = 0; term < TERMS; ++term)
#pragma unroll
                for (int m = 0; m < NMT; ++m)
#pragma unroll
                    for (int p = 0; p < 2; ++p) {
                        const h8 av = term == 2 ? al[s & 1][m] : ah[s & 1][m];
                        const h8 bv = term == 1 ? bl[s & 1][p] : bh[s & 1][p];
#if defined(SPK_ABLATE) && SPK_ABLATE == 2
                        asm volatile("" :: "v"(av), "v"(bv));
#else
                        acc[m][p] = __builtin_amdgcn_mfma_f32_16x16x32_f16(av, bv, acc[m][p], 0, 0, 0);
#endif
                    }
            spk_step_pattern<N_MFMA, N_DS, N_TAIL, K_DMA>(s);
        }
        KSTAMP(k2)
        if (last) {
            finish();
            store_pending = true;
            cur_c = 0; cur_u += a.wgs_per_xcd;
        } else {
            ++cur_c;
        }
        KSTAMP(k3)
        if (early) {
#if !defined(SPK_ABLATE) || SPK_ABLATE != 7
            if (store_pending) { store(); store_pending = false; __builtin_amdgcn_s_waitcnt(0x0F70); }
#endif
            issue_prepare();
        }
        __builtin_amdgcn_s_waitcnt(0x0F70 | Cfg::K_MIN);
        KSTAMP(k4)
        __builtin_amdgcn_s_barrier();
        KSTAMP(k5)
#ifdef SPK_STAMPS
        ks_top += k1 - k0; ks_steps += k2 - k1; ks_fin += k3 - k2; ks_wait += k4 - k3; ks_bar += k5 - k4;
#endif
        st_cur = st_cur == 2 ? 0 : st_cur + 1;
        st_iss = st_iss == 2 ? 0 : st_iss + 1;
    }
    if (store_pending) store();
    if (a.out_spk) fldr_note_range(range_bad);
#ifdef SPK_STAMPS
    KSTAMP(k_end)
    if ((blockIdx.x == 0 || blockIdx.x == 101) && (wave == 0 || wave == 4) && lane == 0) {
        unsigned long long* o = fldr_spk_stamp_buf + ((blockIdx.x == 0 ? 0 : 2) + (wave == 0 ? 0 : 1)) * 8;
        o[0] = ks_top; o[1] = ks_steps; o[2] = ks_fin; o[3] = ks_wait; o[4] = ks_bar; o[5] = total; o[6] = k_end - k_begin;
    }
#endif
}
#endif

__global__ void spk_pack_kernel(const float* __restrict__ src, int64_t src_bstride, unsigned char* __restrict__ dst,
                                int64_t dst_bstride, int C, int64_t HW) {
    const int64_t pix = (int64_t)blockIdx.x * 256 + threadIdx.x;
    const int g = blockIdx.y, n = blockIdx.z;
    if (pix >= HW) return;
    const float* s = src + (int64_t)n * src_bstride + (int64_t)g * 8 * HW + pix;
    float x[8];
#pragma unroll
    for (int k = 0; k < 8; ++k) x[k] = g * 8 + k < C ? s[(int64_t)k * HW] : 0.0f;
    h8 hi, lo;
    bool bad = false;
    { _Float16 hs[8], ls[8]; fldr_split_hl_group(x, hs, ls, bad);
#pragma unroll
      for (int k = 0; k < 8; ++k) { hi[k] = hs[k]; lo[k] = ls[k]; } }
    fldr_note_range(bad);
    unsigned char* d = dst + (int64_t)n * dst_bstride + ((int64_t)g * 2 * HW + pix) * 16;
    *reinterpret_cast<h8*>(d) = hi;
    *reinterpret_cast<h8*>(d + HW * 16) = lo;
}

__global__ void spk_unpack_kernel(const unsigned char* __restrict__ src, int64_t src_bstride, float* __restrict__ dst,
                                  int C, int64_t HW) {
    const int64_t pix = (int64_t)blockIdx.x * 256 + threadIdx.x;
    const int g = blockIdx.y, n = blockIdx.z;
    if (pix >= HW) return;
    const unsigned char* s = src + (int64_t)n * src_bstride + ((int64_t)g * 2 * HW + pix) * 16;
    const h8 hi = *reinterpret_cast<const h8*>(s), lo = *reinterpret_cast<const h8*>(s + HW * 16);
#pragma unroll
    for (int k = 0; k < 8; ++k)
        if (g * 8 + k < C) dst[((int64_t)n * C + g * 8 + k) * HW + pix] = (float)hi[k] + (float)lo[k];
}

FLDR_TU_STATUS(spk)

namespace {
struct DevStatus { fldr_status_block* host = nullptr; fldr_status_block* host_dev = nullptr; float* poison = nullptr; };
std::mutex g_status_mu;
DevStatus g_status[64];
DevStatus* status_of_current_device() {
    int dev = 0;
    if (hipGetDevice(&dev) != hipSuccess || dev < 0 || dev >= 64) return nullptr;
    std::lock_guard<std::mutex> lk(g_status_mu);
    DevStatus& st = g_status[dev];
    if (st.host) return &st;
    fldr_status_block* h = nullptr;
    fldr_status_block* hd = nullptr;
    float* p = nullptr;
    if (hipHostMalloc(reinterpret_cast<void**>(&h), sizeof(fldr_status_block), hipHostMallocMapped | hipHostMallocCoherent) != hipSuccess) return nullptr;
    *h = fldr_status_block{};
    bool ok = hipHostGetDevicePointer(reinterpret_cast<void**>(&hd), h, 0) == hipSuccess && hipMalloc(reinterpret_cast<void**>(&p), 256) == hipSuccess &&
              hipMemset(p, 0, 256) == hipSuccess;
    int (*binders[])(fldr_status_block*, float*) = {fldr_status_bind_spk, fldr_status_bind_ring, fldr_status_bind_conv, fldr_status_bind_s2, fldr_status_bind_split,
                                                    fldr_status_bind_warp, fldr_status_bind_gather, fldr_status_bind_acc64, fldr_status_bind_dec23};
    for (auto b : binders) ok = ok && b(hd, p) == 0;
    ok = ok && hipDeviceSynchronize() == hipSuccess;
    if (!ok) { if (p) (void)hipFree(p); (void)hipHostFree(h); return nullptr; }
    st.host_dev = hd; st.poison = p; st.host = h;
    return &st;
}
}

const float* fldr_status_poison_ptr(void) {
    DevStatus* st = status_of_current_device();
    return st ? st->poison : nullptr;
}

extern "C" int fldr_status_word(const volatile int** host_words) {
    FLDR_CHECK_ARG(host_words);
    DevStatus* st = status_of_current_device();
    if (!st) return FLDR_E_STATUS;
    *host_words = &st->host->range;
    return 0;
}

extern "C" int fldr_range_status(int reset) {
    if (hipDeviceSynchronize() != hipSuccess) return -1;
    int v = 0;
    int (*readers[])(int) = {fldr_range_read_spk, fldr_range_read_ring, fldr_range_read_conv, fldr_range_read_s2, fldr_range_read_split, fldr_range_read_warp, fldr_range_read_gather, fldr_range_read_acc64, fldr_range_read_dec23};
    for (auto r : readers) { const int x = r(reset); if (x < 0) return x; v |= x ? 1 : 0; }
    if (reset) {
        int dev = 0;
        if (hipGetDevice(&dev) == hipSuccess && dev >= 0 && dev < 64) { std::lock_guard<std::mutex> lk(g_status_mu); if (g_status[dev].host) g_status[dev].host->range = 0; }
    }
    return v;
}
extern "C" int fldr_ring_status(int reset) {
    if (hipDeviceSynchronize() != hipSuccess) return -1;
    const int v = fldr_ring_timeouts_read(reset);
    if (reset && v >= 0) {
        int dev = 0;
        if (hipGetDevice(&dev) == hipSuccess && dev >= 0 && dev < 64) {
            std::lock_guard<std::mutex> lk(g_status_mu);
            if (g_status[dev].host) {
                g_status[dev].host->ring = 0;
                if (hipMemset(g_status[dev].poison, 0, 4) != hipSuccess || hipDeviceSynchronize() != hipSuccess) return -1;
            }
        }
    }
    return v;
}

extern "C" int fldr_sizeof_desc(int which) {
    switch (which) {
        case 0: return (int)sizeof(fldr_conv_desc);
        case 1: return (int)sizeof(fldr_spk_conv_desc);
        case 2: return (int)sizeof(fldr_prep_desc);
        case 3: return (int)sizeof(fldr_pca_level);
        case 4: return (int)sizeof(fldr_splat_acc_desc);
        case 5: return (int)sizeof(fldr_splat_gather_desc);
        default: return FLDR_E_ARG;
    }
}

extern "C" int64_t fldr_spk_bytes(int C, int H, int W) {
    if (C <= 0 || H <= 0 || W <= 0) return FLDR_E_ARG;
    return (int64_t)((C + 7) / 8) * 2 * H * W * 16;
}

extern "C" int fldr_spk_pack(const float* src, int64_t src_bstride, void* dst, int N, int C, int H, int W, fldr_stream_t stream) {
    FLDR_CHECK_ARG(src && dst && N > 0 && C > 0 && H > 0 && W > 0);
    const int64_t HW = (int64_t)H * W;
    hipLaunchKernelGGL(spk_pack_kernel, dim3(fldr_cdiv(HW, 256), (C + 7) / 8, N), dim3(256), 0, fldr_s(stream), src, src_bstride,
                       reinterpret_cast<unsigned char*>(dst), fldr_spk_bytes(C, H, W), C, HW);
    FLDR_LAUNCH_RET();
}

extern "C" int fldr_spk_unpack(const void* src, float* dst, int N, int C, int H, int W, fldr_stream_t stream) {
    FLDR_CHECK_ARG(src && dst && N > 0 && C > 0 && H > 0 && W > 0);
    const int64_t HW = (int64_t)H * W;
    hipLaunchKernelGGL(spk_unpack_kernel, dim3(fldr_cdiv(HW, 256), (C + 7) / 8, N), dim3(256), 0, fldr_s(stream),
                       reinterpret_cast<const unsigned char*>(src), fldr_spk_bytes(C, H, W), dst, C, HW);
    FLDR_LAUNCH_RET();
}

__global__ void spk_absmax_kernel(const float* __restrict__ w, int64_t n, float* __restrict__ hdr) {
    __shared__ float red[256];
    float m = 0.0f;
    for (int64_t i = threadIdx.x; i < n; i += 256) m = fmaxf(m, fabsf(w[i]));
    red[threadIdx.x] = m;
    __syncthreads();
    for (int s = 128; s > 0; s >>= 1) {
        if (threadIdx.x < s) red[threadIdx.x] = fmaxf(red[threadIdx.x], red[threadIdx.x + s]);
        __syncthreads();
    }
    if (threadIdx.x < SPK_HDR) {
        const float mx = red[0];
        float scale = 1.0f;
        if (mx > 0.0f) scale = exp2f(floorf(log2f(8192.0f / mx)));
        const float v[SPK_HDR] = {1.0f / scale, scale, mx, 0.0f, 0.0f, 0.0f, 0.0f, 0.0f};
        hdr[threadIdx.x] = v[threadIdx.x];
    }
}

__global__ void spk_prepack_kernel(const float* __restrict__ w, float* __restrict__ wp, int cout, int cin, int nmt,
                                   int n_chunks, int64_t total_h8) {
    const int64_t i = (int64_t)blockIdx.x * 256 + threadIdx.x;
    if (i >= total_h8) return;
    const float scale = wp[1];
    const int lane = (int)(i % 64);
    const int kind = (int)((i / 64) % 2);
    const int m = (int)((i / 128) % nmt);
    const int s = (int)((i / (128 * nmt)) % SPK_STEPS);
    const int ch = (int)((i / (128 * nmt * SPK_STEPS)) % n_chunks);
    const int gr = (int)(i / ((int64_t)128 * nmt * SPK_STEPS * n_chunks));
    const int li = lane & 15, lg = lane >> 4;
    const int co = gr * 16 * nmt + m * 16 + li;
    const int tap = 2 * s + (lg >> 1);
    h8 v;
#pragma unroll
    for (int j = 0; j < 8; ++j) {
        const int c = ch * 16 + (lg & 1) * 8 + j;
        float x = (tap < 9 && co < cout && c < cin) ? w[((int64_t)co * cin + c) * 9 + tap] * scale : 0.0f;
        const _Float16 h = (_Float16)x;
        v[j] = kind == 0 ? h : (_Float16)(x - (float)h);
    }
    reinterpret_cast<h8*>(wp + SPK_HDR)[i] = v;
}

__global__ void spk_prepack32_kernel(const float* __restrict__ w, const float* __restrict__ hdr, float* __restrict__ dst, int cout, int cin,
                                     int n_chunks, int64_t total_h8) {
    const int64_t i = (int64_t)blockIdx.x * 256 + threadIdx.x;
    if (i >= total_h8) return;
    const float scale = hdr[1];
    const int lane = (int)(i % 64), kind = (int)((i / 64) % 2), tap = (int)((i / 128) % 9);
    const int ch = (int)((i / (128 * 9)) % n_chunks), gr = (int)(i / ((int64_t)128 * 9 * n_chunks));
    const int co = gr * 32 + (lane & 31);
    h8 v;
#pragma unroll
    for (int j = 0; j < 8; ++j) {
        const int c = ch * 16 + (lane >> 5) * 8 + j;
        const float x = (co < cout && c < cin) ? w[((int64_t)co * cin + c) * 9 + tap] * scale : 0.0f;
        const _Float16 h = (_Float16)x;
        v[j] = kind == 0 ? h : (_Float16)(x - (float)h);
    }
    reinterpret_cast<h8*>(dst)[i] = v;
}

extern "C" int64_t fldr_conv_spk_prepack_size(int cout, int cin) {
    if (cout <= 0 || cin <= 0 || cout > 96 || cin > SPK_MAX_GROUPS * 8) return FLDR_E_ARG;
    return SPK_HDR + spk_first_section_floats(cout, cin) + spk_r32_section_floats(cout, cin);
}

extern "C" int fldr_conv_spk_prepack(const float* weight, float* wpack, int cout, int cin, fldr_stream_t stream) {
    FLDR_CHECK_ARG(weight && wpack);
    const int64_t total = fldr_conv_spk_prepack_size(cout, cin);
    if (total < 0) return (int)total;
    int nmt, groups;
    spk_geometry(cout, nmt, groups);
    const int n_chunks = (cin + 15) / 16;
    const int64_t first = spk_first_section_floats(cout, cin), total_h8 = first / 4;
    hipLaunchKernelGGL(spk_absmax_kernel, dim3(1), dim3(256), 0, fldr_s(stream), weight, (int64_t)cout * cin * 9, wpack);
    hipLaunchKernelGGL(spk_prepack_kernel, dim3(fldr_cdiv(total_h8, 256)), dim3(256), 0, fldr_s(stream), weight, wpack, cout, cin,
                       nmt, n_chunks, total_h8);
    if (spk_has_r32_section(cout)) {
        const int64_t r_h8 = spk_r32_section_floats(cout, cin) / 4;
        hipLaunchKernelGGL(spk_prepack32_kernel, dim3(fldr_cdiv(r_h8, 256)), dim3(256), 0, fldr_s(stream), weight, wpack, wpack + SPK_HDR + first,
                           cout, cin, n_chunks, r_h8);
    }
    FLDR_LAUNCH_RET();
}

static int g_spk_wgs_per_xcd = 32;
static int g_spk_small_units = 96;
FLDR_HOOK int fldr_debug_spk_small_units(int v) { if (v != 0) g_spk_small_units = v; return g_spk_small_units; }
FLDR_HOOK int fldr_debug_spk_wgs_per_xcd(int v) { if (v > 0) g_spk_wgs_per_xcd = v; return g_spk_wgs_per_xcd; }
static int g_spk_variant = 1;
FLDR_HOOK int fldr_debug_spk_variant(int v) { if (v >= 0) g_spk_variant = v; return g_spk_variant; }

#ifdef FLDR_TEST_HOOKS
template <int NMT, int TERMS, bool HAS_RES>
static int spk_launch2(SpkArgs& a, int N, hipStream_t s) {
    using Cfg = SpkCfg<NMT>;
    static std::atomic<uint64_t> attr_done{0};
    if (int e = fldr_set_max_lds(reinterpret_cast<const void*>(&conv3x3_spk_kernel<NMT, TERMS, HAS_RES>), Cfg::LDS_BYTES, attr_done)) return e;
    if (int e = spk_fill_geometry(a, N, g_spk_wgs_per_xcd)) return e;
    hipLaunchKernelGGL((conv3x3_spk_kernel<NMT, TERMS, HAS_RES>), dim3(8 * a.wgs_per_xcd), dim3(512), Cfg::LDS_BYTES, s, a);
    FLDR_LAUNCH_RET();
}

template <int NMT, int TERMS>
static int spk_launch(SpkArgs& a, int N, hipStream_t s) {
    return a.residual ? spk_launch2<NMT, TERMS, true>(a, N, s) : spk_launch2<NMT, TERMS, false>(a, N, s);
}
#endif

static int spk_conv_run(const fldr_spk_conv_desc* d, int rows, fldr_stream_t stream) {
    FLDR_CHECK_ARG(d && rows >= 0 && rows <= d->H);
    const int walk_h = rows ? rows : d->H;
    FLDR_CHECK_ARG(d->wpack && (d->out_f32 || d->out_spk) && d->n_src >= 1 && d->n_src <= FLDR_CONV_MAX_SRC);
    FLDR_CHECK_ARG(d->N > 0 && d->cin > 0 && d->cin <= SPK_MAX_GROUPS * 8 && d->cout > 0 && d->cout <= 96);
    FLDR_CHECK_ARG(d->cout_store > 0 && d->cout_store <= d->cout && d->H > 0 && d->W > 0);
    FLDR_CHECK_ARG(!d->residual || d->out_f32 || (d->precision & 2));
    FLDR_CHECK_ARG(!(d->precision & ~3) && (!(d->precision & 2) || (d->residual && g_spk_variant == 1)));
    if ((int64_t)d->cout_store * d->H * d->W * 4 >= (1ll << 32) || fldr_spk_bytes(96, d->H, d->W) >= (1ll << 32)) return FLDR_E_SHAPE;
    SpkArgs a;
    a.res_spk = (d->precision & 2) ? 1 : 0;
    int gsum = 0, csum = 0;
    for (int s = 0; s < d->n_src; ++s) {
        FLDR_CHECK_ARG(d->src[s] && d->src_c[s] > 0);
        if (d->src_up2[s] && ((d->H | d->W) & 1)) return FLDR_E_SHAPE;
        if (s + 1 < d->n_src && (d->src_c[s] & 7)) return FLDR_E_SHAPE;
        const int ng = (d->src_c[s] + 7) / 8;
        if (gsum + ng > SPK_MAX_GROUPS) return FLDR_E_ARG;
        const int64_t plane = d->src_up2[s] ? (int64_t)(d->H >> 1) * (d->W >> 1) * 16 : (int64_t)d->H * d->W * 16;
        for (int g = 0; g < ng; ++g) {
            a.grp_ptr[gsum + g] = (unsigned long long)(reinterpret_cast<uintptr_t>(d->src[s]) + (uint64_t)g * 2 * plane) | (d->src_up2[s] ? 1ull : 0ull);
            a.grp_bstride[gsum + g] = d->src_bstride[s];
        }
        gsum += ng; csum += d->src_c[s];
    }
    if (csum != d->cin) return FLDR_E_SHAPE;
    for (int g = gsum; g < SPK_MAX_GROUPS; ++g) { a.grp_ptr[g] = 0ull; a.grp_bstride[g] = 0; }
    a.n_levels = 0;
    a.wpack = d->wpack; a.bias = d->bias; a.residual = d->residual;
    a.out_f32 = d->out_f32; a.out_spk = reinterpret_cast<unsigned char*>(d->out_spk);
    a.out_spk_bstride = fldr_spk_bytes(d->cout_store, d->H, d->W);
    a.n_chunks = (d->cin + 15) / 16; a.cout = d->cout; a.cout_store = d->cout_store;
    a.H = d->H; a.W = d->W; a.relu = d->relu;
    int nmt, groups;
    spk_geometry(d->cout, nmt, groups);
    a.groups = groups; a.pack_nmt = nmt;
    a.w32_off = spk_has_r32_section(d->cout) ? (SPK_HDR + spk_first_section_floats(d->cout, d->cin)) * 4 : 0;
    if (nmt > 1) {
        const int64_t units = (int64_t)d->N * fldr_cdiv(d->W, SPK_TW) * fldr_cdiv(walk_h, SPK_TH) * groups;
        if (units <= g_spk_small_units) { a.groups = (d->cout + 15) / 16; nmt = 1; }
    }
    hipStream_t s = fldr_s(stream);
    if (g_spk_variant == 1) return fldr_spk_ring_dispatch(a, d->N, nmt, (d->precision & 1) ? 1 : 3, g_spk_wgs_per_xcd, s, walk_h);
#ifndef FLDR_TEST_HOOKS
    return FLDR_E_ARG;
#else
    if (d->precision & 1) {
        if (nmt == 1) return spk_launch<1, 1>(a, d->N, s);
        if (nmt == 2) return spk_launch<2, 1>(a, d->N, s);
        return spk_launch<3, 1>(a, d->N, s);
    }
    if (nmt == 1) return spk_launch<1, 3>(a, d->N, s);
    if (nmt == 2) return spk_launch<2, 3>(a, d->N, s);
    return spk_launch<3, 3>(a, d->N, s);
#endif
}
extern "C" int fldr_conv2d_spk(const fldr_spk_conv_desc* d, fldr_stream_t stream) { return spk_conv_run(d, 0, stream); }
extern "C" int fldr_conv2d_spk_rows(const fldr_spk_conv_desc* d, int rows, fldr_stream_t stream) { return spk_conv_run(d, rows, stream); }

#ifdef FLDR_TEST_HOOKS
int fldr_spk_ringrow_dispatch(SpkArgs& a, const float* wrow, int N, int wgs_per_xcd_max, hipStream_t s);
FLDR_HOOK int fldr_debug_conv2d_ringrow(const fldr_spk_conv_desc* d, const float* wrow, fldr_stream_t stream) {
    FLDR_CHECK_ARG(d && wrow && d->wpack && d->out_spk && !d->out_f32 && !d->residual && d->n_src >= 1 && d->n_src <= FLDR_CONV_MAX_SRC);
    FLDR_CHECK_ARG(d->N > 0 && d->cin > 0 && d->cin % 32 == 0 && d->cin <= SPK_MAX_GROUPS * 8 && d->cout > 0 && d->cout <= 96 && d->cout_store == d->cout);
    FLDR_CHECK_ARG((d->cout % 48 == 0 || d->cout % 32 == 0) && d->precision == 0 && d->H > 0 && d->W > 0);
    if (fldr_spk_bytes(96, d->H, d->W) >= (1ll << 32)) return FLDR_E_SHAPE;
    SpkArgs a;
    a.res_spk = 0;
    int gsum = 0;
    for (int s = 0; s < d->n_src; ++s) {
        FLDR_CHECK_ARG(d->src[s] && d->src_c[s] > 0 && !(d->src_c[s] & 7));
        if (d->src_up2[s] && ((d->H | d->W) & 1)) return FLDR_E_SHAPE;
        const int ng = d->src_c[s] / 8;
        if (gsum + ng > SPK_MAX_GROUPS) return FLDR_E_ARG;
        const int64_t plane = d->src_up2[s] ? (int64_t)(d->H >> 1) * (d->W >> 1) * 16 : (int64_t)d->H * d->W * 16;
        for (int g = 0; g < ng; ++g) {
            a.grp_ptr[gsum + g] = (unsigned long long)(reinterpret_cast<uintptr_t>(d->src[s]) + (uint64_t)g * 2 * plane) | (d->src_up2[s] ? 1ull : 0ull);
            a.grp_bstride[gsum + g] = d->src_bstride[s];
        }
        gsum += ng;
    }
    if (gsum * 8 != d->cin) return FLDR_E_SHAPE;
    for (int g = gsum; g < SPK_MAX_GROUPS; ++g) { a.grp_ptr[g] = 0ull; a.grp_bstride[g] = 0; }
    a.n_levels = 0;
    a.wpack = d->wpack; a.bias = d->bias; a.residual = nullptr; a.out_f32 = nullptr;
    a.out_spk = reinterpret_cast<unsigned char*>(d->out_spk);
    a.out_spk_bstride = fldr_spk_bytes(d->cout_store, d->H, d->W);
    a.n_chunks = d->cin / 16; a.cout = d->cout; a.cout_store = d->cout_store;
    a.H = d->H; a.W = d->W; a.relu = d->relu; a.pack_nmt = 0; a.w32_off = 0;
    return fldr_spk_ringrow_dispatch(a, wrow, d->N, g_spk_wgs_per_xcd, fldr_s(stream));
}
#endif

extern "C" int fldr_conv2d_spk_levels(const fldr_spk_conv_desc* descs, int n_levels, fldr_stream_t stream) {
    FLDR_CHECK_ARG(descs && n_levels >= 1 && n_levels <= SPK_MAX_LEVELS);
    if (n_levels == 1) return fldr_conv2d_spk(descs, stream);
    if (g_spk_variant != 1) return FLDR_E_ARG;
    const fldr_spk_conv_desc& d0 = descs[0];
    FLDR_CHECK_ARG(d0.wpack && (d0.out_f32 || d0.out_spk) && d0.n_src == 1 && d0.src[0] && d0.N == 1);
    FLDR_CHECK_ARG(d0.cin > 0 && d0.cin <= SPK_MAX_GROUPS * 8 && d0.cout > 0 && d0.cout <= 96 && d0.cout_store > 0 && d0.cout_store <= d0.cout);
    FLDR_CHECK_ARG(!d0.residual || d0.out_f32 || (d0.precision & 2));
    FLDR_CHECK_ARG(!(d0.precision & ~3) && (!(d0.precision & 2) || d0.residual));
    SpkArgs a;
    a.res_spk = (d0.precision & 2) ? 1 : 0;
    const int ng = (d0.cin + 7) / 8;
    for (int g = 0; g < SPK_MAX_GROUPS; ++g) { a.grp_ptr[g] = g < ng ? (unsigned long long)reinterpret_cast<uintptr_t>(d0.src[0]) : 0ull; a.grp_bstride[g] = 0; }
    a.wpack = d0.wpack; a.bias = d0.bias; a.residual = d0.residual;
    a.out_f32 = d0.out_f32; a.out_spk = reinterpret_cast<unsigned char*>(d0.out_spk);
    a.out_spk_bstride = 0;
    a.n_chunks = (d0.cin + 15) / 16; a.cout = d0.cout; a.cout_store = d0.cout_store;
    a.H = d0.H; a.W = d0.W; a.relu = d0.relu;
    int nmt, groups;
    spk_geometry(d0.cout, nmt, groups);
    a.groups = groups; a.pack_nmt = nmt; a.w32_off = 0;
    a.n_levels = n_levels;
    int64_t units = 0;
    for (int l = 0; l < n_levels; ++l) {
        const fldr_spk_conv_desc& d = descs[l];
        FLDR_CHECK_ARG(d.n_src == 1 && d.src[0] && d.N == 1 && d.H > 0 && d.W > 0 && !d.src_up2[0] && d.src_c[0] == d0.cin);
        FLDR_CHECK_ARG(d.wpack == d0.wpack && d.bias == d0.bias && d.cin == d0.cin && d.cout == d0.cout && d.cout_store == d0.cout_store);
        FLDR_CHECK_ARG(d.relu == d0.relu && d.precision == d0.precision);
        FLDR_CHECK_ARG(!d.residual == !d0.residual && !d.out_f32 == !d0.out_f32 && !d.out_spk == !d0.out_spk);
        if ((int64_t)d.cout_store * d.H * d.W * 4 >= (1ll << 32) || fldr_spk_bytes(96, d.H, d.W) >= (1ll << 32)) return FLDR_E_SHAPE;
        SpkArgs::SpkLevel& v = a.lv[l];
        v.H = d.H; v.W = d.W; v.tiles_x = fldr_cdiv(d.W, SPK_TW); v.n_tiles = v.tiles_x * fldr_cdiv(d.H, SPK_TH);
        v.unit0 = (int32_t)units; v.pad = 0; v.m_tiles_x = 0; v.pad2 = 0;
        v.in_off = reinterpret_cast<const char*>(d.src[0]) - reinterpret_cast<const char*>(d0.src[0]);
        v.out_spk_off = d.out_spk ? reinterpret_cast<const char*>(d.out_spk) - reinterpret_cast<const char*>(d0.out_spk) : 0;
        v.out_f32_off = d.out_f32 ? reinterpret_cast<const char*>(d.out_f32) - reinterpret_cast<const char*>(d0.out_f32) : 0;
        v.res_off = d.residual ? reinterpret_cast<const char*>(d.residual) - reinterpret_cast<const char*>(d0.residual) : 0;
        units += (int64_t)v.n_tiles * groups;
    }
    for (int l = n_levels; l < SPK_MAX_LEVELS; ++l) { a.lv[l] = a.lv[n_levels - 1]; a.lv[l].unit0 = 0x7fffffff; }
    if (units >= (1 << 28)) return FLDR_E_SHAPE;
    return fldr_spk_ring_dispatch_levels(a, (int)units, nmt, (d0.precision & 1) ? 1 : 3, g_spk_wgs_per_xcd, fldr_s(stream));
}
```

fldr-vfi_amd/csrc/spk_common.h:

```cpp
#pragma once
#include "common.h"
#include "row_plan.h"

typedef _Float16 h8 __attribute__((ext_vector_type(8)));
typedef _Float16 h4 __attribute__((ext_vector_type(4)));
typedef float f4 __attribute__((ext_vector_type(4)));
typedef __attribute__((address_space(1))) const void* kgptr_t;
typedef __attribute__((address_space(3))) void* klptr_t;

#define SPK_MAX_GROUPS 14
#define SPK_MAX_LEVELS 8
#define SPK_TH 8
#define SPK_TW 32
#define SPK_IH (SPK_TH + 2)
static_assert(SPK_TH == FLDR_PLAN_TH_CONV, "row_plan.h: 3x3 tile height");
#define SPK_IW (SPK_TW + 2)
#define SPK_PLANE 5632
#define SPK_IN_BYTES (4 * SPK_PLANE)
#define SPK_STEPS 5
#define SPK_HDR 8

struct SpkArgs {
    unsigned long long grp_ptr[SPK_MAX_GROUPS];
    int64_t grp_bstride[SPK_MAX_GROUPS];
    const float* wpack;
    const float* bias;
    const float* residual;
    float* out_f32;
    unsigned char* out_spk;
    int64_t out_spk_bstride;
    int32_t n_chunks, cout, cout_store;
    int32_t H, W;
    int32_t relu;
    int32_t res_spk;
    int32_t tiles_x, n_tiles, groups;
    int32_t pack_nmt;
    int32_t n_units, units_per_xcd, wgs_per_xcd;
    int32_t n_levels;
    int32_t spin_limit;
    struct SpkLevel {
        int32_t H, W, tiles_x, n_tiles, unit0, pad;
        uint32_t m_tiles_x, pad2;
        int64_t in_off, out_spk_off, out_f32_off, res_off;
    } lv[SPK_MAX_LEVELS];
    uint32_t m_groups, m_tiles, m_tiles_x;
    int64_t w32_off;
};

static inline void spk_geometry(int cout, int& nmt, int& groups) {
    if (cout <= 16)      { nmt = 1; groups = 1; }
    else if (cout <= 32) { nmt = 2; groups = 1; }
    else if (cout <= 48) { nmt = 3; groups = 1; }
    else if (cout <= 64) { nmt = 2; groups = 2; }
    else                 { nmt = 3; groups = (cout + 47) / 48; }
}
static inline int64_t spk_first_section_floats(int cout, int cin) {
    int nmt, groups;
    spk_geometry(cout, nmt, groups);
    return (int64_t)groups * ((cin + 15) / 16) * SPK_STEPS * nmt * 2 * 64 * 4;
}
static inline bool spk_has_r32_section(int cout) { return cout == 64 || cout == 96; }
static inline int64_t spk_r32_section_floats(int cout, int cin) { return spk_has_r32_section(cout) ? (int64_t)(cout / 32) * ((cin + 15) / 16) * 18 * 256 : 0; }

template <int NMT>
struct SpkCfg {
    static constexpr int W_BYTES = SPK_STEPS * NMT * 2 * 1024;
    static constexpr int PIECES = W_BYTES / 16;
    static constexpr int NWI = (PIECES + 511) / 512;
    static constexpr int STAGE = W_BYTES + SPK_IN_BYTES;
    static constexpr int LDS_BYTES = 3 * STAGE;
    static constexpr int K_MIN = 3 + NWI;
    static_assert(PIECES % 64 == 0, "weight slab must be a whole number of wave-wide DMA pieces");
};

__device__ __forceinline__ int spk_div(int u, uint32_t m, int d) {
    return d == 1 ? u : (int)__umulhi((uint32_t)u, m);
}

__device__ __forceinline__ void spk_split(float x, _Float16& hi, _Float16& lo, bool& bad) { fldr_split_hl(x, hi, lo, bad); }

template <int N_MFMA, int N_DS, int I>
struct SpkInterleave {
    static __device__ __forceinline__ void run() {
        constexpr int cnt = (N_MFMA * (I + 1)) / N_DS - (N_MFMA * I) / N_DS;
        if constexpr (cnt > 0) __builtin_amdgcn_sched_group_barrier(0x008, cnt, 0);
        __builtin_amdgcn_sched_group_barrier(0x100, 1, 0);
        SpkInterleave<N_MFMA, N_DS, I + 1>::run();
    }
};
template <int NV, int I>
struct SpkInterleaveV {
    static __device__ __forceinline__ void run() {
        __builtin_amdgcn_sched_group_barrier(0x008, 1, 0);
        __builtin_amdgcn_sched_group_barrier(0x010, 1, 0);
        SpkInterleaveV<NV, I + 1>::run();
    }
};
template <int NV>
struct SpkInterleaveV<NV, NV> {
    static __device__ __forceinline__ void run() {}
};
template <int N_MFMA, int N_DS>
struct SpkInterleave<N_MFMA, N_DS, N_DS> {
    static __device__ __forceinline__ void run() {}
};

template <int N_MFMA, int N_DS, int N_TAIL, int NV>
__device__ __forceinline__ void spk_step_pattern_n(bool reads) {
    SpkInterleaveV<NV, 0>::run();
    constexpr int rest = N_MFMA - NV;
    if (reads) {
        constexpr int tail = rest - N_TAIL >= N_DS / 2 ? N_TAIL : 0;
        SpkInterleave<rest - tail, N_DS, 0>::run();
        if constexpr (tail > 0) __builtin_amdgcn_sched_group_barrier(0x008, tail, 0);
    } else {
        if constexpr (rest > 0) __builtin_amdgcn_sched_group_barrier(0x008, rest, 0);
    }
}
template <int N_MFMA, int N_DS, int N_TAIL, int K_DMA>
__device__ __forceinline__ void spk_step_pattern(int s) {
    const int nv = ((s + 1) * K_DMA + SPK_STEPS - 1) / SPK_STEPS - (s * K_DMA + SPK_STEPS - 1) / SPK_STEPS;
    const bool reads = s + 1 < SPK_STEPS;
    if (nv == 0) spk_step_pattern_n<N_MFMA, N_DS, N_TAIL, 0>(reads);
    else if (nv == 1) spk_step_pattern_n<N_MFMA, N_DS, N_TAIL, 1>(reads);
    else spk_step_pattern_n<N_MFMA, N_DS, N_TAIL, 2>(reads);
}

#ifndef SPK_RIGHT_SIZE
#define SPK_RIGHT_SIZE 1
#endif
static inline int spk_right_size(int upx, int wpx_max, int groups) {
    int w = upx < wpx_max ? upx : wpx_max;
    w = w / groups * groups;
    if (w < groups) w = groups;
#if SPK_RIGHT_SIZE
    const int rounds = (upx + w - 1) / w;
    int need = (upx + rounds - 1) / rounds;
    need = (need + groups - 1) / groups * groups;
    if (need < w) w = need;
#endif
    return w;
}

static inline int spk_fill_geometry(SpkArgs& a, int N, int wgs_per_xcd_max, int tile_w = SPK_TW, int walk_h = 0) {
    a.tiles_x = fldr_cdiv(a.W, tile_w);
    a.n_tiles = a.tiles_x * fldr_cdiv(walk_h > 0 && walk_h < a.H ? walk_h : a.H, SPK_TH);
    a.n_units = N * a.n_tiles * a.groups;
    a.units_per_xcd = (a.n_units + 7) / 8;
    a.units_per_xcd = (a.units_per_xcd + a.groups - 1) / a.groups * a.groups;
    a.wgs_per_xcd = spk_right_size(a.units_per_xcd, wgs_per_xcd_max, a.groups);
    const int64_t dmax = a.n_tiles > a.groups ? a.n_tiles : a.groups;
    if (((int64_t)a.n_units + 8 * a.units_per_xcd) * dmax >= (1ll << 32)) return FLDR_E_SHAPE;
    a.m_groups = (uint32_t)((1ull << 32) / (uint32_t)a.groups) + 1u;
    a.m_tiles = (uint32_t)((1ull << 32) / (uint32_t)a.n_tiles) + 1u;
    a.m_tiles_x = (uint32_t)((1ull << 32) / (uint32_t)a.tiles_x) + 1u;
    return 0;
}

int fldr_spk_ring_dispatch(SpkArgs& a, int N, int nmt, int terms, int wgs_per_xcd_max, hipStream_t s, int walk_h = 0);
int fldr_spk_ring_dispatch_levels(SpkArgs& a, int n_units, int nmt, int terms, int wgs_per_xcd_max, hipStream_t s);
```

fldr-vfi_amd/fldr_hip.py:

```python
import ctypes
import os

import torch

_HERE = os.path.dirname(os.path.abspath(__file__))
LIB_PATH = os.environ.get("FLDR_LIB") or os.path.join(_HERE, "libfldr_hip.so")

MAX_SRC = 12
_c_float_p = ctypes.c_void_p


class ConvDesc(ctypes.Structure):
    _fields_ = [
        ("src", ctypes.c_void_p * MAX_SRC),
        ("src_bstride", ctypes.c_int64 * MAX_SRC),
        ("src_c", ctypes.c_int32 * MAX_SRC),
        ("src_up2", ctypes.c_int32 * MAX_SRC),
        ("n_src", ctypes.c_int32),
        ("wpack", ctypes.c_void_p),
        ("bias", ctypes.c_void_p),
        ("residual", ctypes.c_void_p),
        ("out", ctypes.c_void_p),
        ("N", ctypes.c_int32), ("cin", ctypes.c_int32), ("cout", ctypes.c_int32), ("cout_store", ctypes.c_int32),
        ("Hin", ctypes.c_int32), ("Win", ctypes.c_int32), ("Hout", ctypes.c_int32), ("Wout", ctypes.c_int32),
        ("ksize", ctypes.c_int32), ("stride", ctypes.c_int32), ("relu", ctypes.c_int32), ("precision", ctypes.c_int32),
        ("out_spk", ctypes.c_void_p),
        ("src_cstride", ctypes.c_int64 * MAX_SRC),
    ]


class PrepDesc(ctypes.Structure):
    _fields_ = [
        ("flow_lo", ctypes.c_void_p), ("I0", ctypes.c_void_p), ("I1", ctypes.c_void_p),
        ("i0_bstride", ctypes.c_int64), ("i1_bstride", ctypes.c_int64),
        ("t", ctypes.c_void_p), ("z0", ctypes.c_void_p), ("z1", ctypes.c_void_p),
        ("flow_t0", ctypes.c_void_p), ("flow_t1", ctypes.c_void_p), ("flowback_0", ctypes.c_void_p), ("flowback_1", ctypes.c_void_p),
        ("im0_tot", ctypes.c_void_p), ("im1_tot", ctypes.c_void_p),
        ("N", ctypes.c_int32), ("h", ctypes.c_int32), ("w", ctypes.c_int32), ("H", ctypes.c_int32), ("W", ctypes.c_int32),
        ("mul", ctypes.c_float), ("z_alpha0", ctypes.c_float), ("z_alpha1", ctypes.c_float), ("withmask", ctypes.c_int32),
        ("ws", ctypes.c_void_p),
        ("i0_cstride", ctypes.c_int64), ("i1_cstride", ctypes.c_int64),
        ("phase", ctypes.c_int32), ("reserved", ctypes.c_int32),
    ]


class PcaLevel(ctypes.Structure):
    _fields_ = [("planes", ctypes.c_void_p), ("out_f32", ctypes.c_void_p), ("out_spk", ctypes.c_void_p),
                ("P", ctypes.c_int32), ("H", ctypes.c_int32), ("W", ctypes.c_int32), ("reserved", ctypes.c_int32),
                ("raw_ws", ctypes.c_void_p)]


class SplatGatherDesc(ctypes.Structure):
    _fields_ = [("img", ctypes.c_void_p * 2), ("img_bstride", ctypes.c_int64 * 2), ("flow", ctypes.c_void_p * 2),
                ("flow_bstride", ctypes.c_int64 * 2), ("metric", ctypes.c_void_p * 2), ("out_f32", ctypes.c_void_p * 2),
                ("out_spk", ctypes.c_void_p * 2), ("ws", ctypes.c_void_p),
                ("ndir", ctypes.c_int32), ("N", ctypes.c_int32), ("C", ctypes.c_int32), ("H", ctypes.c_int32), ("W", ctypes.c_int32),
                ("mode", ctypes.c_int32)]


class SplatAccDesc(ctypes.Structure):
    _fields_ = [("img", ctypes.c_void_p * 2), ("img_bstride", ctypes.c_int64 * 2), ("img_cstride", ctypes.c_int64 * 2),
                ("flow", ctypes.c_void_p * 2), ("flow_bstride", ctypes.c_int64 * 2), ("metric", ctypes.c_void_p * 2),
                ("ws", ctypes.c_void_p * 2), ("out_f32", ctypes.c_void_p * 2), ("out_spk", ctypes.c_void_p * 2),
                ("nprob", ctypes.c_int32), ("N", ctypes.c_int32), ("C", ctypes.c_int32), ("H", ctypes.c_int32), ("W", ctypes.c_int32),
                ("mode", ctypes.c_int32), ("flags", ctypes.c_int32), ("reserved", ctypes.c_int32)]


class SynthRows(ctypes.Structure):
    _fields_ = [(n, ctypes.c_int32) for n in ("prep2", "splat", "enc1", "enc2", "enc3", "dec0", "dec1", "dec23")]


class SpkConvDesc(ctypes.Structure):
    _fields_ = [
        ("src", ctypes.c_void_p * MAX_SRC),
        ("src_bstride", ctypes.c_int64 * MAX_SRC),
        ("src_c", ctypes.c_int32 * MAX_SRC),
        ("src_up2", ctypes.c_int32 * MAX_SRC),
        ("n_src", ctypes.c_int32),
        ("wpack", ctypes.c_void_p),
        ("bias", ctypes.c_void_p),
        ("residual", ctypes.c_void_p),
        ("out_f32", ctypes.c_void_p),
        ("out_spk", ctypes.c_void_p),
        ("N", ctypes.c_int32), ("cin", ctypes.c_int32), ("cout", ctypes.c_int32), ("cout_store", ctypes.c_int32),
        ("H", ctypes.c_int32), ("W", ctypes.c_int32), ("relu", ctypes.c_int32), ("precision", ctypes.c_int32),
    ]


_SIGNATURES = {
    "fldr_version": (ctypes.c_int, []),
    "fldr_error_string": (ctypes.c_char_p, [ctypes.c_int]),
    "fldr_softsplat_fwd": (ctypes.c_int, [_c_float_p] * 3 + [ctypes.c_int] * 4 + [ctypes.c_void_p]),
    "fldr_softsplat_fused": (ctypes.c_int, [_c_float_p] * 5 + [ctypes.c_int] * 5 + [ctypes.c_void_p]),
    "fldr_softsplat_fused_spk": (ctypes.c_int, [_c_float_p] * 3 + [ctypes.c_void_p, _c_float_p] + [ctypes.c_int] * 5 + [ctypes.c_void_p]),
    "fldr_softsplat_pair_spk": (ctypes.c_int, [_c_float_p] * 4 + [ctypes.c_void_p, _c_float_p] + [ctypes.c_int] * 4 + [ctypes.c_void_p]),
    "fldr_resize_bilinear_spk": (ctypes.c_int, [_c_float_p] * 2 + [ctypes.c_void_p] + [ctypes.c_int] * 6 + [ctypes.c_float, ctypes.c_void_p]),
    "fldr_resize_bilinear_spk_bounds": (ctypes.c_int, [_c_float_p] * 2 + [ctypes.c_void_p, _c_float_p] + [ctypes.c_int] * 5 + [ctypes.c_float, ctypes.c_void_p]),
    "fldr_softsplat_gather_ws_floats": (ctypes.c_int64, [ctypes.c_int] * 4),
    "fldr_softsplat_gather": (ctypes.c_int, [ctypes.POINTER(SplatGatherDesc), ctypes.c_void_p]),
    "fldr_softsplat_tile_ws_floats": (ctypes.c_int64, [ctypes.c_int] * 3),
    "fldr_softsplat_acc64": (ctypes.c_int, [ctypes.POINTER(SplatAccDesc), ctypes.c_void_p]),
    "fldr_splat_bounds_upsampled_pair": (ctypes.c_int, [_c_float_p, ctypes.c_int64, _c_float_p, ctypes.c_int, ctypes.c_float, _c_float_p]
                                         + [ctypes.c_int] * 5 + [ctypes.c_void_p]),
    "fldr_softsplat_tile": (ctypes.c_int, [_c_float_p] * 5 + [ctypes.c_int] * 5 + [ctypes.c_void_p]),
    "fldr_softsplat_tile_strided": (ctypes.c_int, [_c_float_p, ctypes.c_int64, ctypes.c_int64] + [_c_float_p] * 4 + [ctypes.c_int] * 5
                                    + [ctypes.c_void_p]),
    "fldr_softsplat_tile_prebounded": (ctypes.c_int, [_c_float_p, ctypes.c_int64, ctypes.c_int64] + [_c_float_p] * 4 + [ctypes.c_int] * 5
                                       + [ctypes.c_void_p]),
    "fldr_splat_bounds_upsampled": (ctypes.c_int, [_c_float_p, ctypes.c_int64, _c_float_p, ctypes.c_int, ctypes.c_float, _c_float_p]
                                    + [ctypes.c_int] * 5 + [ctypes.c_void_p]),
    "fldr_correlation_fwd": (ctypes.c_int, [_c_float_p] * 3 + [ctypes.c_int] * 4 + [ctypes.c_void_p]),
    "fldr_debug_corr_variant": (ctypes.c_int, [ctypes.c_int]),
    "fldr_debug_splat_group_fold": (ctypes.c_int, [ctypes.c_int]),
    "fldr_debug_corr_chunk": (ctypes.c_int, [ctypes.c_int]),
    "fldr_debug_corr_xcd": (ctypes.c_int, [ctypes.c_int]),
    "fldr_softsplat_bwd": (ctypes.c_int, [_c_float_p] * 5 + [ctypes.c_int] * 4 + [ctypes.c_void_p]),
    "fldr_correlation_bwd": (ctypes.c_int, [_c_float_p] * 5 + [ctypes.c_int] * 4 + [ctypes.c_void_p]),
    "fldr_pca_project": (ctypes.c_int, [_c_float_p] * 7 + [ctypes.c_int] * 4 + [ctypes.c_void_p]),
    "fldr_pca_project_stream": (ctypes.c_int, [_c_float_p] * 8 + [ctypes.c_int] * 4 + [ctypes.c_void_p]),
    "fldr_pca_table_size": (ctypes.c_int64, [ctypes.c_int]),
    "fldr_pca_prepack": (ctypes.c_int, [_c_float_p] * 4 + [ctypes.c_int, ctypes.c_void_p]),
    "fldr_pca_project_pyramid": (ctypes.c_int, [ctypes.POINTER(PcaLevel), ctypes.c_int, _c_float_p, ctypes.c_int, _c_float_p, ctypes.c_void_p]),
    "fldr_debug_pca_workgroups": (ctypes.c_int, [ctypes.c_int]),
    "fldr_debug_pca_variant": (ctypes.c_int, [ctypes.c_int]),
    "fldr_debug_ring_tile_width": (ctypes.c_int, [ctypes.c_int]),
    "fldr_debug_ring_spin_limit": (ctypes.c_int, [ctypes.c_int]),
    "fldr_status_word": (ctypes.c_int, [ctypes.POINTER(ctypes.POINTER(ctypes.c_int))]),
    "fldr_debug_s2_vec4": (ctypes.c_int, [ctypes.c_int]),
    "fldr_bwarp": (ctypes.c_int, [_c_float_p] * 3 + [ctypes.c_int] * 5 + [ctypes.c_void_p]),
    "fldr_bwarp_tscaled": (ctypes.c_int, [_c_float_p] * 4 + [ctypes.c_int] * 7 + [ctypes.c_void_p]),
    "fldr_resize_bilinear": (ctypes.c_int, [_c_float_p] * 2 + [ctypes.c_int] * 5 + [ctypes.c_float, ctypes.c_void_p]),
    "fldr_level0_prep": (ctypes.c_int, [ctypes.POINTER(PrepDesc), ctypes.c_void_p]),
    "fldr_zmetric": (ctypes.c_int, [_c_float_p] * 3 + [ctypes.c_float, _c_float_p] + [ctypes.c_int] * 4 + [ctypes.c_void_p]),
    "fldr_conv_prepack_size": (ctypes.c_int64, [ctypes.c_int] * 3),
    "fldr_conv_prepack": (ctypes.c_int, [_c_float_p] * 2 + [ctypes.c_int] * 3 + [ctypes.c_void_p]),
    "fldr_conv2d": (ctypes.c_int, [ctypes.POINTER(ConvDesc), ctypes.c_void_p]),
    "fldr_conv_split_prepack_size": (ctypes.c_int64, [ctypes.c_int] * 2),
    "fldr_conv_split_prepack": (ctypes.c_int, [_c_float_p] * 2 + [ctypes.c_int] * 2 + [ctypes.c_void_p]),
    "fldr_conv2d_split": (ctypes.c_int, [ctypes.POINTER(ConvDesc), ctypes.c_void_p]),
    "fldr_conv_s2_prepack_size": (ctypes.c_int64, [ctypes.c_int] * 2),
    "fldr_conv_s2_prepack": (ctypes.c_int, [_c_float_p] * 2 + [ctypes.c_int] * 2 + [ctypes.c_void_p]),
    "fldr_conv2d_s2_split": (ctypes.c_int, [ctypes.POINTER(ConvDesc), ctypes.c_void_p]),
    "fldr_conv2d_s2_spk": (ctypes.c_int, [ctypes.POINTER(ConvDesc), ctypes.c_void_p]),
    "fldr_conv2d_s2_spk_pair": (ctypes.c_int, [ctypes.POINTER(ConvDesc), ctypes.POINTER(ConvDesc), ctypes.c_void_p]),
    "fldr_conv2d_s2_split_rows": (ctypes.c_int, [ctypes.POINTER(ConvDesc), ctypes.c_int, ctypes.c_int, ctypes.c_void_p]),
    "fldr_conv2d_s2_spk_rows": (ctypes.c_int, [ctypes.POINTER(ConvDesc), ctypes.c_int, ctypes.c_int, ctypes.c_void_p]),
    "fldr_conv2d_s2_spk_pair_rows": (ctypes.c_int, [ctypes.POINTER(ConvDesc), ctypes.POINTER(ConvDesc), ctypes.c_int, ctypes.c_int, ctypes.c_void_p]),
    "fldr_debug_s2_persistent": (ctypes.c_int, [ctypes.c_int]),
    "fldr_debug_s2_dma": (ctypes.c_int, [ctypes.c_int]),
    "fldr_debug_s2_wgs_per_xcd": (ctypes.c_int, [ctypes.c_int]),
    "fldr_debug_dec23_wgs_per_xcd": (ctypes.c_int, [ctypes.c_int]),
    "fldr_debug_s2_xshift": (ctypes.c_int, [ctypes.c_int]),
    "fldr_debug_dec3_xshift": (ctypes.c_int, [ctypes.c_int]),
    "fldr_debug_dec3_xcd": (ctypes.c_int, [ctypes.c_int]),
    "fldr_debug_splat_quad": (ctypes.c_int, [ctypes.c_int]),
    "fldr_spk_bytes": (ctypes.c_int64, [ctypes.c_int] * 3),
    "fldr_spk_pack": (ctypes.c_int, [_c_float_p, ctypes.c_int64, ctypes.c_void_p] + [ctypes.c_int] * 4 + [ctypes.c_void_p]),
    "fldr_spk_unpack": (ctypes.c_int, [ctypes.c_void_p, _c_float_p] + [ctypes.c_int] * 4 + [ctypes.c_void_p]),
    "fldr_conv_spk_prepack_size": (ctypes.c_int64, [ctypes.c_int] * 2),
    "fldr_conv_spk_prepack": (ctypes.c_int, [_c_float_p] * 2 + [ctypes.c_int] * 2 + [ctypes.c_void_p]),
    "fldr_conv2d_spk": (ctypes.c_int, [ctypes.POINTER(SpkConvDesc), ctypes.c_void_p]),
    "fldr_conv2d_spk_rows": (ctypes.c_int, [ctypes.POINTER(SpkConvDesc), ctypes.c_int, ctypes.c_void_p]),
    "fldr_conv2d_spk_levels": (ctypes.c_int, [ctypes.POINTER(SpkConvDesc), ctypes.c_int, ctypes.c_void_p]),
    "fldr_debug_spk_wgs_per_xcd": (ctypes.c_int, [ctypes.c_int]),
    "fldr_range_status": (ctypes.c_int, [ctypes.c_int]),
    "fldr_ring_status": (ctypes.c_int, [ctypes.c_int]),
    "fldr_debug_spk_small_units": (ctypes.c_int, [ctypes.c_int]),
    "fldr_debug_spk_variant": (ctypes.c_int, [ctypes.c_int]),
    "fldr_debug_ring_consumers": (ctypes.c_int, [ctypes.c_int]),
    "fldr_debug_ring32": (ctypes.c_int, [ctypes.c_int]),
    "fldr_debug_ring_resident": (ctypes.c_int, [ctypes.c_int]),
    "fldr_debug_ring_timeouts": (ctypes.c_int, []),
    "fldr_debug_busy_partner": (ctypes.c_int, [ctypes.c_void_p, ctypes.c_int, ctypes.c_int, ctypes.c_int, ctypes.c_int, ctypes.c_void_p]),
    "fldr_sizeof_desc": (ctypes.c_int, [ctypes.c_int]),
    "fldr_synth_tail": (ctypes.c_int, [_c_float_p, ctypes.POINTER(ctypes.c_void_p), ctypes.POINTER(ctypes.c_int64),
                                       _c_float_p, ctypes.c_double, _c_float_p, _c_float_p] + [ctypes.c_int] * 3 + [ctypes.c_void_p]),
    "fldr_dec3_prepack": (ctypes.c_int, [_c_float_p, _c_float_p, ctypes.c_void_p]),
    "fldr_dec3_synth": (ctypes.c_int, [_c_float_p] * 3 + [ctypes.POINTER(ctypes.c_void_p), ctypes.POINTER(ctypes.c_int64),
                                       _c_float_p, ctypes.c_double, _c_float_p, _c_float_p, _c_float_p] + [ctypes.c_int] * 3 + [ctypes.c_void_p]),
    "fldr_dec3_synth_strided": (ctypes.c_int, [_c_float_p] * 3 + [ctypes.POINTER(ctypes.c_void_p), ctypes.POINTER(ctypes.c_int64),
                                               ctypes.POINTER(ctypes.c_int64), _c_float_p, ctypes.c_double, _c_float_p, _c_float_p,
                                               _c_float_p] + [ctypes.c_int] * 3 + [ctypes.c_void_p]),
    "fldr_dec3_prepack_spk_size": (ctypes.c_int64, []),
    "fldr_dec3_prepack_spk": (ctypes.c_int, [_c_float_p, _c_float_p, ctypes.c_void_p]),
    "fldr_dec3_synth_spk": (ctypes.c_int, [ctypes.c_void_p, _c_float_p, _c_float_p, ctypes.POINTER(ctypes.c_void_p), ctypes.POINTER(ctypes.c_int64),
                                           ctypes.POINTER(ctypes.c_int64), _c_float_p, ctypes.c_double, _c_float_p, _c_float_p,
                                           _c_float_p] + [ctypes.c_int] * 3 + [ctypes.c_void_p]),
    "fldr_dec23_prepack_size": (ctypes.c_int64, []),
    "fldr_dec23_prepack": (ctypes.c_int, [_c_float_p, _c_float_p, ctypes.c_void_p]),
    "fldr_dec23_synth": (ctypes.c_int, [ctypes.c_void_p, ctypes.c_void_p, _c_float_p, _c_float_p, _c_float_p, _c_float_p, ctypes.POINTER(ctypes.c_void_p),
                                        ctypes.POINTER(ctypes.c_int64), ctypes.POINTER(ctypes.c_int64), _c_float_p, ctypes.c_double, _c_float_p, _c_float_p,
                                        ctypes.c_void_p] + [ctypes.c_int] * 5 + [ctypes.c_void_p]),
    "fldr_dec23_synth_u16": (ctypes.c_int, [ctypes.c_void_p, ctypes.c_void_p, _c_float_p, _c_float_p, _c_float_p, _c_float_p, ctypes.POINTER(ctypes.c_void_p),
                                            ctypes.POINTER(ctypes.c_int64), ctypes.POINTER(ctypes.c_int64), _c_float_p, ctypes.c_double, ctypes.c_void_p]
                             + [ctypes.c_int] * 6 + [ctypes.c_void_p]),
    "fldr_dec23_synth_rows": (ctypes.c_int, [ctypes.c_void_p, ctypes.c_void_p, _c_float_p, _c_float_p, _c_float_p, _c_float_p, ctypes.POINTER(ctypes.c_void_p),
                                             ctypes.POINTER(ctypes.c_int64), ctypes.POINTER(ctypes.c_int64), _c_float_p, ctypes.c_double, _c_float_p, _c_float_p,
                                             ctypes.c_void_p] + [ctypes.c_int] * 6 + [ctypes.c_void_p]),
    "fldr_dec23_synth_u16_rows": (ctypes.c_int, [ctypes.c_void_p, ctypes.c_void_p, _c_float_p, _c_float_p, _c_float_p, _c_float_p, ctypes.POINTER(ctypes.c_void_p),
                                                 ctypes.POINTER(ctypes.c_int64), ctypes.POINTER(ctypes.c_int64), _c_float_p, ctypes.c_double, ctypes.c_void_p]
                                  + [ctypes.c_int] * 7 + [ctypes.c_void_p]),
    "fldr_synth_row_plan": (ctypes.c_int, [ctypes.c_int, ctypes.c_int, ctypes.POINTER(SynthRows)]),
    "fldr_ingest_u16": (ctypes.c_int, [ctypes.c_void_p, _c_float_p] + [ctypes.c_int] * 6 + [ctypes.c_void_p]),
    "fldr_ingest_pyramid_u16": (ctypes.c_int, [ctypes.c_void_p, ctypes.POINTER(ctypes.c_void_p)] + [ctypes.c_int] * 7 + [ctypes.c_void_p]),
    "fldr_quantize_u16": (ctypes.c_int, [ctypes.c_void_p, ctypes.c_int, ctypes.c_void_p] + [ctypes.c_int] * 6 + [ctypes.c_void_p]),
    "fldr_ingest_u8": (ctypes.c_int, [ctypes.c_void_p, _c_float_p] + [ctypes.c_int] * 5 + [ctypes.c_void_p]),
    "fldr_pyramid_bicubic": (ctypes.c_int, [_c_float_p, _c_float_p] + [ctypes.c_int] * 4 + [ctypes.c_void_p]),
    "fldr_ingest_pyramid_u8": (ctypes.c_int, [ctypes.c_void_p, ctypes.POINTER(ctypes.c_void_p)] + [ctypes.c_int] * 6 + [ctypes.c_void_p]),
    "fldr_ssim_y_ws_doubles": (ctypes.c_int64, [ctypes.c_int] * 3),
    "fldr_ssim_y_u8": (ctypes.c_int, [ctypes.c_void_p, ctypes.c_void_p, ctypes.c_void_p] + [ctypes.c_int] * 3 + [ctypes.c_void_p]),
    "fldr_frame_metrics": (ctypes.c_int, [ctypes.c_void_p, ctypes.c_int, ctypes.c_void_p, ctypes.c_void_p, ctypes.c_void_p]
                           + [ctypes.c_int] * 5 + [ctypes.c_void_p]),
}

_TEST_BUILD_ONLY = ("fldr_softsplat_tile", "fldr_softsplat_tile_strided", "fldr_softsplat_tile_prebounded")
EXPORTS = tuple(n for n in _SIGNATURES if not n.startswith("fldr_debug_") and n not in _TEST_BUILD_ONLY)
HOOKS = tuple(n for n in _SIGNATURES if n.startswith("fldr_debug_") or n in _TEST_BUILD_ONLY)
TEST_LIB_PATH = os.path.join(_HERE, "libfldr_hip_test.so")
ABI_VERSION = 105
_DEFAULT_PATH = ("fldr_version", "fldr_error_string", "fldr_sizeof_desc", "fldr_range_status", "fldr_ring_status", "fldr_status_word", "fldr_pca_prepack",
                 "fldr_pca_project_pyramid", "fldr_conv2d_spk", "fldr_conv2d_spk_levels", "fldr_conv_spk_prepack", "fldr_conv2d_s2_split",
                 "fldr_conv2d_s2_spk", "fldr_conv2d_s2_spk_pair", "fldr_conv_s2_prepack", "fldr_softsplat_acc64", "fldr_level0_prep",
                 "fldr_splat_bounds_upsampled_pair", "fldr_resize_bilinear_spk", "fldr_resize_bilinear_spk_bounds", "fldr_dec3_prepack_spk",
                 "fldr_dec3_synth_spk", "fldr_spk_pack", "fldr_dec23_prepack_size", "fldr_dec23_prepack", "fldr_dec23_synth",
                 "fldr_synth_row_plan", "fldr_conv2d_s2_split_rows", "fldr_conv2d_s2_spk_rows", "fldr_conv2d_s2_spk_pair_rows", "fldr_conv2d_spk_rows",
                 "fldr_dec23_synth_rows")
_lib = None
_hooks_lib = None


def _load(path, want_hooks):
    if not os.path.exists(path):
        raise ImportError("%s is missing — build it with `make -C fldr-vfi_amd/csrc` (or `python -c 'import __graft_entry__ as g; "
                          "g.build()'`). There is no CPU/eager fallback." % path)
    l = ctypes.CDLL(path)
    variant = bool(os.environ.get("FLDR_LIB"))
    missing = []
    for name, (res, args) in _SIGNATURES.items():
        try:
            fn = getattr(l, name)
        except AttributeError:
            if name in HOOKS and (not want_hooks or variant):
                continue
            if variant and name not in _DEFAULT_PATH:
                missing.append(name)
                continue
            raise ImportError("%s does not export %s, which the default forward calls: rebuild it" % (path, name))
        fn.restype = res
        fn.argtypes = args
    for which, cls in enumerate((ConvDesc, SpkConvDesc, PrepDesc, PcaLevel, SplatAccDesc, SplatGatherDesc)):
        got = l.fldr_sizeof_desc(which)
        if got != ctypes.sizeof(cls) and not (variant and got < 0):
            raise ImportError("%s: sizeof(%s) is %d in the library, %d in this binding" % (path, cls.__name__, got, ctypes.sizeof(cls)))
    if l.fldr_version() != ABI_VERSION:
        msg = "%s reports ABI version %d, this binding is written for %d" % (path, l.fldr_version(), ABI_VERSION)
        if not variant:
            raise ImportError(msg + ": rebuild it")
        import warnings
        warnings.warn(msg + " (FLDR_LIB variant: struct sizes agree, continuing)" + (("; missing entry points: " + ", ".join(missing)) if missing else ""))
    return l


def lib():
    global _lib
    if _lib is None:
        _lib = _load(LIB_PATH, want_hooks=False)
    return _lib


def busy_partner(out, workgroups=512, lds_bytes=1024, iters=40000, kind=2):
    global _hooks_lib
    if _hooks_lib is None:
        _hooks_lib = _load(os.environ.get("FLDR_LIB") or TEST_LIB_PATH, want_hooks=True)
    if out.dtype != torch.float32 or out.numel() < workgroups * 256:
        raise ValueError("busy_partner: out must hold workgroups * 256 floats")
    _check(_hooks_lib.fldr_debug_busy_partner(_dev(out, "out"), workgroups, lds_bytes, iters, kind, _stream()), "fldr_debug_busy_partner")


class test_hooks:

    def __enter__(self):
        global _lib, _hooks_lib
        if _hooks_lib is None:
            _hooks_lib = _load(os.environ.get("FLDR_LIB") or TEST_LIB_PATH, want_hooks=True)
            for env, hook in (("FLDR_RING_CONSUMERS", "fldr_debug_ring_consumers"), ("FLDR_SPK_VARIANT", "fldr_debug_spk_variant"),
                              ("FLDR_PCA_WORKGROUPS", "fldr_debug_pca_workgroups"), ("FLDR_PCA_VARIANT", "fldr_debug_pca_variant"),
                              ("FLDR_RING_TILE_WIDTH", "fldr_debug_ring_tile_width"), ("FLDR_S2_VEC4", "fldr_debug_s2_vec4")):
                if os.environ.get(env) and hasattr(_hooks_lib, hook):
                    getattr(_hooks_lib, hook)(int(os.environ[env]))
        self._prev = _lib
        _lib = _hooks_lib
        return _hooks_lib

    def __exit__(self, *exc):
        global _lib
        _lib = self._prev
        return False


def enter_test_hooks():
    if _lib is None or _lib is not _hooks_lib:
        test_hooks().__enter__()
    return _lib


def spk_variant():
    fn = getattr(lib(), "fldr_debug_spk_variant", None)
    return 1 if fn is None else fn(-1)


class FldrError(RuntimeError):
    pass


def _check(code, what):
    if code != 0:
        raise FldrError("%s failed: %s (code %d)" % (what, lib().fldr_error_string(code).decode(), code))


_raw_stream = getattr(torch._C, "_cuda_getCurrentRawStream", None)


def _stream():
    if _raw_stream is not None:
        return ctypes.c_void_p(_raw_stream(torch.cuda.current_device()))
    return ctypes.c_void_p(torch.cuda.current_stream().cuda_stream)


def _dev(t, name, dtype=torch.float32):
    if not t.is_cuda:
        raise NotImplementedError("%s: fldr_hip has no CPU path (the reference has none either, softSplat.py:251-252)" % name)
    if t.dtype != dtype:
        raise TypeError("%s must be %s, got %s" % (name, dtype, t.dtype))
    if not t.is_contiguous():
        raise ValueError("%s must be contiguous" % name)
    return ctypes.c_void_p(t.data_ptr())


def _planes(t, name):
    if not t.is_cuda:
        raise NotImplementedError("%s: fldr_hip has no CPU path (the reference has none either, softSplat.py:251-252)" % name)
    if t.dtype != torch.float32:
        raise TypeError("%s must be float32, got %s" % (name, t.dtype))
    N, C, H, W = t.shape
    if not ((W == 1 or t.stride(3) == 1) and (H == 1 or t.stride(2) == W)):
        t = t.contiguous()
    return t, (t.stride(0) if N > 1 else 0), (t.stride(1) if C > 1 else H * W)



def softsplat_fwd(inp, flow):
    N, C, H, W = inp.shape
    assert flow.shape[1] == 2 and flow.shape[2] == H and flow.shape[3] == W
    inp, flow = inp.contiguous(), flow.contiguous()
    out = inp.new_zeros(N, C, H, W)
    _check(lib().fldr_softsplat_fwd(_dev(inp, "input"), _dev(flow, "flow"), _dev(out, "output"), N, C, H, W, _stream()),
           "fldr_softsplat_fwd")
    return out


def softsplat_bwd(inp, flow, grad_out, need_input=True, need_flow=True):
    N, C, H, W = inp.shape
    inp, flow, grad_out = inp.contiguous(), flow.contiguous(), grad_out.contiguous()
    gi = torch.empty_like(inp) if need_input else None
    gf = torch.empty_like(flow) if need_flow else None
    if gi is None and gf is None:
        return None, None
    _check(lib().fldr_softsplat_bwd(_dev(inp, "input"), _dev(flow, "flow"), _dev(grad_out, "gradOutput"),
                                    _dev(gi, "gradInput") if gi is not None else None,
                                    _dev(gf, "gradFlow") if gf is not None else None, N, C, H, W, _stream()), "fldr_softsplat_bwd")
    return gi, gf


def correlation_bwd(first, second, grad_out, need_first=True, need_second=True):
    N, C, H, W = first.shape
    first, second, grad_out = first.contiguous(), second.contiguous(), grad_out.contiguous()
    g1 = torch.empty_like(first) if need_first else None
    g2 = torch.empty_like(second) if need_second else None
    if g1 is None and g2 is None:
        return None, None
    _check(lib().fldr_correlation_bwd(_dev(first, "first"), _dev(second, "second"), _dev(grad_out, "gradOutput"),
                                      _dev(g1, "gradFirst") if g1 is not None else None,
                                      _dev(g2, "gradSecond") if g2 is not None else None, N, C, H, W, _stream()), "fldr_correlation_bwd")
    return g1, g2


_MODES = {"summation": 0, "average": 1, "linear": 2, "softmax": 3}


SPLAT_KERNEL = os.environ.get("FLDR_SPLAT", "auto")
SPLAT_FEATURES = os.environ.get("FLDR_SPLAT_FEATURES", "acc64")
if SPLAT_FEATURES not in ("acc64", "gather"):
    raise ValueError("FLDR_SPLAT_FEATURES=%r: expected 'acc64' (default) or 'gather' (the scatter kernel 'strip' of rounds 1-2 is retired)" % SPLAT_FEATURES)
if SPLAT_KERNEL not in ("auto", "acc64", "strip", "tile"):
    raise ValueError("FLDR_SPLAT=%r: expected auto | acc64 | strip | tile" % SPLAT_KERNEL)
_RETIRED_ENV = ("FLDR_PREP_SPLIT", "FLDR_LEVEL_BATCH", "FLDR_ENC3_SPLIT", "FLDR_ENC3_PAIR", "FLDR_S2_SPK", "FLDR_SPLAT_BOUNDS", "FLDR_DEC3_MFMA",
                "FLDR_RESIZE_BOUNDS", "FLDR_PCA_RAW_MIN_BYTES", "FLDR_INGEST_FUSED")
for _n in _RETIRED_ENV:
    if _n in os.environ:
        import warnings
        warnings.warn("%s is set but is no longer a switch of fldr_hip (retired; see DESIGN.md section 1 for the current ones)" % _n, stacklevel=2)
LEVEL_BATCH = True
PCA_F32 = os.environ.get("FLDR_PCA_F32", "1") != "0"


SPLAT_BOUNDS = "lowres"


def splat_bounds_upsampled(flow_lo, t, scale_mode, mul, H, W):
    N, two, h, w = flow_lo.shape
    assert two == 2 and flow_lo.stride(3) == 1 and flow_lo.stride(2) == w and flow_lo.stride(1) == h * w
    ws = torch.empty(lib().fldr_softsplat_tile_ws_floats(N, H, W), device=flow_lo.device, dtype=torch.float32)
    if t is not None:
        t = t.reshape(N).contiguous().float()
    _check(lib().fldr_splat_bounds_upsampled(ctypes.c_void_p(flow_lo.data_ptr()), flow_lo.stride(0) if N > 1 else 2 * h * w,
                                             _dev(t, "t") if t is not None else None, int(scale_mode), float(mul), _dev(ws, "ws"),
                                             N, h, w, H, W, _stream()), "fldr_splat_bounds_upsampled")
    return ws


def splat_bounds_upsampled_pair(flow_l, t, pair, mul, H, W):
    N, four, h, w = flow_l.shape
    assert four == 4 and flow_l.stride(3) == 1 and flow_l.stride(2) == w and flow_l.stride(1) == h * w
    ws = torch.empty(2 * lib().fldr_softsplat_tile_ws_floats(N, H, W), device=flow_l.device, dtype=torch.float32)
    if t is not None:
        t = t.reshape(N).contiguous().float()
    if not flow_l.is_cuda or flow_l.dtype != torch.float32:
        raise TypeError("flow_l must be a float32 device tensor")
    _check(lib().fldr_splat_bounds_upsampled_pair(ctypes.c_void_p(flow_l.data_ptr()), flow_l.stride(0) if N > 1 else 0, _dev(t, "t") if t is not None else None,
                                                  {"images": 1, "features": 2}[pair], float(mul), _dev(ws, "ws"), N, h, w, H, W, _stream()),
           "fldr_splat_bounds_upsampled_pair")
    return ws


def softsplat_fused(img, flow, metric, mode, out=None, scratch=None, kernel=None, want_spk=False, out_spk=None, bounds_ws=None):
    N, C, H, W = img.shape
    assert flow.shape[1] == 2 and flow.shape[2] == H and flow.shape[3] == W
    flow = flow.contiguous()
    if metric is not None:
        metric = metric.contiguous()
    kern = kernel or SPLAT_KERNEL
    if kern == "auto":
        kern = "acc64"
    if kern == "acc64":
        if want_spk and C <= 3:
            kern = "strip"
        else:
            r = softsplat_acc64([img], [flow], None if metric is None else [metric], mode, want_f32=not want_spk, want_spk=want_spk,
                                bounds_ws=None if bounds_ws is None else [bounds_ws])[0]
            if out is not None and not want_spk:
                out.copy_(r)
                return out
            if out_spk is not None and want_spk:
                raise ValueError("softsplat_fused(kernel='acc64') allocates its packed output")
            return r
    if kern == "tile" and not want_spk:
        img, ibs, ics = _planes(img, "img")
        ws = bounds_ws if bounds_ws is not None else torch.empty(lib().fldr_softsplat_tile_ws_floats(N, H, W), device=img.device, dtype=torch.float32)
        if out is None:
            out = torch.empty(N, C, H, W, device=img.device, dtype=torch.float32)
        if not hasattr(lib(), "fldr_softsplat_tile_strided"):
            raise FldrError("the band splat (kernel='tile' / FLDR_SPLAT=tile) is a retired generation kept in the test build only: "
                            "enter fldr_hip.test_hooks() (tests, tools) — the product splats run on fldr_softsplat_acc64")
        fn = lib().fldr_softsplat_tile_prebounded if bounds_ws is not None else lib().fldr_softsplat_tile_strided
        _check(fn(ctypes.c_void_p(img.data_ptr()), ibs, ics, _dev(flow, "flow"), _dev(metric, "metric") if metric is not None else None,
                  _dev(out, "out"), _dev(ws, "ws"), N, C, H, W, _MODES[mode], _stream()), "fldr_softsplat_tile")
        return out
    img = img.contiguous()
    if want_spk:
        ca = C + (0 if mode == "summation" else 1)
        scratch = torch.empty(N * ca * H * W, device=img.device, dtype=torch.float32)
        outp = _spk_alloc(N, C, H, W, img.device) if out_spk is None else out_spk
        assert outp.shape == (N, C, H, W) and (N == 1 or outp.bstride == ((C + 7) // 8) * 2 * H * W * 16)
        _check(lib().fldr_softsplat_fused_spk(_dev(img, "img"), _dev(flow, "flow"),
                                              _dev(metric, "metric") if metric is not None else None,
                                              ctypes.c_void_p(outp.ptr), _dev(scratch, "scratch"), N, C, H, W,
                                              _MODES[mode], _stream()), "fldr_softsplat_fused_spk")
        return outp
    ca = C + (0 if mode == "summation" else 1)
    if scratch is None:
        scratch = torch.empty(N * ca * H * W, device=img.device, dtype=torch.float32)
    if out is None:
        out = torch.empty(N, C, H, W, device=img.device, dtype=torch.float32)
    _check(lib().fldr_softsplat_fused(_dev(img, "img"), _dev(flow, "flow"),
                                      _dev(metric, "metric") if metric is not None else None,
                                      _dev(out, "out"), _dev(scratch, "scratch"), N, C, H, W, _MODES[mode], _stream()),
           "fldr_softsplat_fused")
    return out


def softsplat_acc64(imgs, flows, metrics=None, mode="softmax", want_f32=True, want_spk=False, bounds_ws=None, spk_batch=False, rows=None):
    nd = len(imgs)
    assert 1 <= nd <= 2 and len(flows) == nd
    N, C, H, W = imgs[0].shape
    assert want_f32 or want_spk
    assert not want_spk or C > 3, "packed output needs the 16-channel configuration (C > 3)"
    d = SplatAccDesc()
    keep, outs = [], []
    batch = None
    if spk_batch:
        assert nd == 2 and N == 1 and want_spk and not want_f32
        batch = _spk_alloc(2, C, H, W, imgs[0].device)
    for k in range(nd):
        im, fl = imgs[k], flows[k]
        assert im.shape == (N, C, H, W) and fl.shape == (N, 2, H, W)
        im, ibs, ics = _planes(im, "img")
        if not fl.is_cuda:
            raise NotImplementedError("fldr softsplat has no CPU path (the reference has none either, softSplat.py:251-252)")
        if fl.dtype != torch.float32:
            raise TypeError("flow must be float32")
        if not fl[0].is_contiguous():
            fl = fl.contiguous()
        keep += [im, fl]
        d.img[k], d.img_bstride[k], d.img_cstride[k] = im.data_ptr(), ibs, ics
        d.flow[k], d.flow_bstride[k] = fl.data_ptr(), (fl.stride(0) if N > 1 else 0)
        mt = metrics[k] if metrics is not None else None
        if mt is not None:
            assert mt.shape == (N, 1, H, W)
            mt = mt.contiguous()
            _dev(mt, "metric")
            keep.append(mt)
        d.metric[k] = mt.data_ptr() if mt is not None else None
        if torch.is_tensor(bounds_ws):
            ws = bounds_ws
        else:
            ws = bounds_ws[k] if bounds_ws is not None else (torch.empty(lib().fldr_softsplat_tile_ws_floats(N, H, W), device=im.device, dtype=torch.float32)
                                                            if H * W > 2304 else None)
        keep.append(ws)
        d.ws[k] = ws.data_ptr() if ws is not None else None
        o32 = torch.empty(N, C, H, W, device=im.device, dtype=torch.float32) if want_f32 else None
        if batch is not None:
            osp = batch.sample(k)
        else:
            osp = _spk_alloc(N, C, H, W, im.device) if want_spk else None
        d.out_f32[k] = o32.data_ptr() if o32 is not None else None
        d.out_spk[k] = osp.ptr if osp is not None else None
        outs.append((o32, osp) if (want_f32 and want_spk) else (osp if want_spk else o32))
    d.nprob, d.N, d.C, d.H, d.W, d.mode = nd, N, C, H, W, _MODES[mode]
    d.flags = 0 if bounds_ws is None else (2 if torch.is_tensor(bounds_ws) else 1)
    d.reserved = int(rows or 0)
    assert not torch.is_tensor(bounds_ws) or nd == 2
    _check(lib().fldr_softsplat_acc64(ctypes.byref(d), _stream()), "fldr_softsplat_acc64")
    return batch if batch is not None else outs


def softsplat_gather(imgs, flows, metrics=None, mode="softmax", want_f32=False, want_spk=True):
    nd = len(imgs)
    assert 1 <= nd <= 2 and len(flows) == nd
    N, C, H, W = imgs[0].shape
    d = SplatGatherDesc()
    keep, outs = [], []
    for k in range(nd):
        im, fl = imgs[k], flows[k]
        assert im.shape == (N, C, H, W) and fl.shape == (N, 2, H, W)
        if not im.is_cuda:
            raise NotImplementedError("fldr softsplat has no CPU path (the reference has none either, softSplat.py:251-252)")
        if im.dtype != torch.float32 or fl.dtype != torch.float32:
            raise TypeError("softsplat_gather takes float32 tensors")
        if not im[0].is_contiguous():
            im = im.contiguous()
        if not fl[0].is_contiguous():
            fl = fl.contiguous()
        keep += [im, fl]
        d.img[k], d.img_bstride[k] = im.data_ptr(), (im.stride(0) if N > 1 else 0)
        d.flow[k], d.flow_bstride[k] = fl.data_ptr(), (fl.stride(0) if N > 1 else 0)
        mt = metrics[k] if metrics is not None else None
        if mt is not None:
            mt = mt.contiguous()
            assert mt.shape == (N, 1, H, W)
            keep.append(mt)
        d.metric[k] = mt.data_ptr() if mt is not None else None
        o32 = torch.empty(N, C, H, W, device=im.device, dtype=torch.float32) if want_f32 else None
        osp = _spk_alloc(N, C, H, W, im.device) if want_spk else None
        d.out_f32[k] = o32.data_ptr() if o32 is not None else None
        d.out_spk[k] = osp.buf.data_ptr() if osp is not None else None
        outs.append((o32, osp) if (want_f32 and want_spk) else (osp if want_spk else o32))
    n = lib().fldr_softsplat_gather_ws_floats(nd, N, H, W)
    ws = torch.empty(max(int(n), 4), device=imgs[0].device, dtype=torch.float32)
    d.ws = ws.data_ptr()
    d.ndir, d.N, d.C, d.H, d.W, d.mode = nd, N, C, H, W, _MODES[mode]
    _check(lib().fldr_softsplat_gather(ctypes.byref(d), _stream()), "fldr_softsplat_gather")
    return outs


def softsplat_pair_spk(img_a, flow_a, img_b, flow_b, mode="softmax"):
    N, C, H, W = img_a.shape
    assert N == 1 and img_b.shape == img_a.shape and flow_a.shape == (1, 2, H, W) and flow_b.shape == (1, 2, H, W)
    ia, ib, fa, fb = img_a.contiguous(), img_b.contiguous(), flow_a.contiguous(), flow_b.contiguous()
    ca = C + (0 if mode == "summation" else 1)
    scratch = torch.empty(2 * ca * H * W, device=ia.device, dtype=torch.float32)
# ... 868 lines not shown
```

include/fldr_hip_test_hooks.h:

```cpp
#ifndef FLDR_HIP_TEST_HOOKS_H
#define FLDR_HIP_TEST_HOOKS_H
#include "fldr_hip.h"
#ifdef __cplusplus
extern "C" {
#endif

FLDR_API int fldr_debug_pca_variant(int v);
FLDR_API int fldr_debug_pca_workgroups(int v);
FLDR_API int fldr_debug_s2_persistent(int v);
FLDR_API int fldr_debug_s2_xshift(int v);
FLDR_API int fldr_debug_s2_vec4(int v);
FLDR_API int fldr_debug_dec3_xshift(int v);
FLDR_API int fldr_debug_splat_quad(int v);
FLDR_API int fldr_debug_dec3_xcd(int v);
FLDR_API int fldr_debug_spk_small_units(int v);
FLDR_API int fldr_debug_spk_wgs_per_xcd(int v);
FLDR_API int fldr_debug_spk_variant(int v);
FLDR_API int fldr_debug_ring_resident(int v);
FLDR_API int fldr_debug_ring32(int v);
FLDR_API int fldr_debug_ring_consumers(int v);
FLDR_API int fldr_debug_corr_variant(int v);
FLDR_API int fldr_debug_corr_xcd(int v);
FLDR_API int fldr_debug_corr_chunk(int v);
FLDR_API int fldr_debug_ring_tile_width(int v);
FLDR_API int fldr_debug_ring_spin_limit(int v);
FLDR_API int64_t fldr_debug_ringrow_pack_floats(int cout, int cin);
FLDR_API int fldr_debug_ringrow_prepack(const float* weight, const float* wpack, float* wrow, int cout, int cin, fldr_stream_t stream);
FLDR_API int fldr_debug_conv2d_ringrow(const fldr_spk_conv_desc* desc, const float* wrow, fldr_stream_t stream);
FLDR_API int fldr_debug_busy_partner(float* out, int workgroups, int lds_bytes, int iters, int kind, fldr_stream_t stream);
FLDR_API int fldr_debug_ring_timeouts(void);
FLDR_API int fldr_debug_splat_tile_variant(int v);
FLDR_API int fldr_debug_pca_variant(int v);
FLDR_API int fldr_debug_pca_workgroups(int v);
FLDR_API int fldr_debug_s2_persistent(int v);
FLDR_API int fldr_debug_s2_xshift(int v);
FLDR_API int fldr_debug_s2_vec4(int v);
FLDR_API int fldr_debug_s2_dma(int v);
FLDR_API int fldr_debug_s2_wgs_per_xcd(int v);
FLDR_API int fldr_debug_dec23_wgs_per_xcd(int v);
FLDR_API int fldr_debug_dec3_xshift(int v);
FLDR_API int fldr_debug_splat_group_fold(int v);
FLDR_API int fldr_debug_conv_occupancy(int* out4);

FLDR_API int fldr_softsplat_tile(const float* img, const float* flow, const float* metric_or_null, float* out, float* ws,
                        int N, int C, int H, int W, int mode, fldr_stream_t stream);
FLDR_API int fldr_softsplat_tile_strided(const float* img, int64_t img_bstride, int64_t img_cstride, const float* flow,
                                const float* metric_or_null, float* out, float* ws, int N, int C, int H, int W, int mode,
                                fldr_stream_t stream);
FLDR_API int fldr_softsplat_tile_prebounded(const float* img, int64_t img_bstride, int64_t img_cstride, const float* flow,
                                   const float* metric_or_null, float* out, float* ws, int N, int C, int H, int W, int mode,
                                   fldr_stream_t stream);

#ifdef __cplusplus
}
#endif
#endif
```

Baseline: 543.4 frame-pairs/s.

## Add row-summed weight path for 3x3 convs over nearest-upsampled input chunks

For input chunks that come from 2x nearest-upsampled sources, adjacent output rows see duplicated input rows, so the vertical taps can be pre-summed per output-row parity. A new prepacked weight section holds these row-summed weights, and a new consumer step loop runs 3 MFMA steps per parity instead of 5. Loaders fetch the row-summed weights for the chunks marked in rs_mask. This cuts MFMA and LDS work on decoder convs with cout<=32, at the cost of a larger weight pack, more template instances, and a changed fp16 split rounding of the summed weights.

```diff
diff --git a/fldr-vfi_amd/csrc/conv_ring_kernels.hip b/fldr-vfi_amd/csrc/conv_ring_kernels.hip
--- a/fldr-vfi_amd/csrc/conv_ring_kernels.hip
+++ b/fldr-vfi_amd/csrc/conv_ring_kernels.hip
@@ -59,10 +59,11 @@
     return v;
 }
 
-template <int NMT, int TW = SPK_TW, bool RW = false>
+template <int NMT, int TW = SPK_TW, bool RW = false, bool RS = false>
 struct RingCfg {
-    static constexpr int W_BYTES = SPK_STEPS * NMT * 2 * 1024;
-    static constexpr int NBLK = SPK_STEPS * NMT * 2;
+    static constexpr int WSTEPS = RS ? 2 * SPK_RS_STEPS : SPK_STEPS;
+    static constexpr int W_BYTES = WSTEPS * NMT * 2 * 1024;
+    static constexpr int NBLK = WSTEPS * NMT * 2;
     static constexpr int NWL = (NBLK + RING_NLOAD - 1) / RING_NLOAD;
     static constexpr int IW = TW + 2;
     static constexpr int CB = TW / 16;
@@ -78,6 +79,7 @@
     static constexpr int BIAS_OFF = CTR_OFF + 64;
     static constexpr int LDS_BYTES = BIAS_OFF + 64 * NMT;
     static_assert(SLOTS <= 8 && INFLIGHT + 2 <= SLOTS && INFLIGHT * K_DMA <= 15, "ring shape");
+    static_assert(!(RW && RS), "the resident-weight test variant has no row-summed form");
     static_assert(TW == 16 || TW == 32, "tile width");
     static_assert(TW != SPK_TW || PLANE == SPK_PLANE, "the 32-pixel plane is the barrier pipeline's");
     static_assert(PLANE / 16 >= 64 && NXI * 64 >= SPK_IH * IW, "DMA pieces cover the plane");
@@ -118,9 +120,10 @@
     __builtin_amdgcn_sched_barrier(0);
 }
 
-template <int NMT, int TERMS, bool HAS_RES, int NC, int TW, bool ML = false, bool RW = false>
+template <int NMT, int TERMS, bool HAS_RES, int NC, int TW, bool ML = false, bool RW = false, bool RS = false>
 __global__ __launch_bounds__((NC + RING_NLOAD) * 64) void conv3x3_ring_kernel(SpkArgs a) {
-    using Cfg = RingCfg<NMT, TW, RW>;
+    using Cfg = RingCfg<NMT, TW, RW, RS>;
+    static_assert(!RS || (TERMS == 3 && !ML), "row-summed chunks: the 3-term split, single-level launches");
     constexpr int SLOTS = Cfg::SLOTS;
     constexpr int CB = Cfg::CB;
     constexpr int RING_NCONS = NC;
@@ -175,11 +178,14 @@
         const int pack_w_bytes = SPK_STEPS * a.pack_nmt * 2 * 1024;
         int w_blk[Cfg::NWL], x_piece[Cfg::NXI];
         uint32_t w_voff[Cfg::NWL];
+        uint32_t w_voff_rs[RS ? Cfg::NWL : 1];
 #pragma unroll
         for (int i = 0; i < Cfg::NWL; ++i) {
             w_blk[i] = min(lw * Cfg::NWL + i, Cfg::NBLK - 1);
             const int step = w_blk[i] / (2 * NMT), mk = w_blk[i] - step * 2 * NMT;
-            w_voff[i] = (uint32_t)((step * a.pack_nmt + msel) * 2 + mk) * 1024u + (uint32_t)lane * 16u;
+            if constexpr (RS) w_voff_rs[i] = (uint32_t)((step * a.pack_nmt + msel) * 2 + mk) * 1024u + (uint32_t)lane * 16u;
+            const int step5 = RS ? min(step, SPK_STEPS - 1) : step;
+            w_voff[i] = (uint32_t)((step5 * a.pack_nmt + msel) * 2 + mk) * 1024u + (uint32_t)lane * 16u;
         }
 #pragma unroll
         for (int i = 0; i < Cfg::NXI; ++i) x_piece[i] = min(i * 64, Cfg::PLANE / 16 - 64);
@@ -228,6 +234,9 @@
             }
         };
         const char* const iss_w = reinterpret_cast<const char*>(a.wpack + SPK_HDR) + (int64_t)pgrp * n_chunks * pack_w_bytes;
+        const int rs_w_bytes = 2 * SPK_RS_STEPS * a.pack_nmt * 2 * 1024;
+        const char* const iss_wrs = reinterpret_cast<const char*>(a.wpack) + a.wrs_off;
+        const int rs_mask = RS ? a.rs_mask : 0;
         issue_geometry();
         int st = 0;
         uint32_t free_target = 0;
@@ -238,6 +247,8 @@
         for (int k = 0; k < total; ++k) {
             RSTAMP(l0)
             const char* wbase = iss_w + (int64_t)iss_c * pack_w_bytes;
+            const bool rs_fill = RS && ((rs_mask >> iss_c) & 1);
+            if constexpr (RS) { if (rs_fill) wbase = iss_wrs + (int64_t)iss_c * rs_w_bytes; }
             const int gi = iss_c * 2 + igrp;
             const uint32_t e_lo = __builtin_amdgcn_readlane((int)(uint32_t)tab_ptr, gi), e_hi = __builtin_amdgcn_readlane((int)(uint32_t)(tab_ptr >> 32), gi);
             const uint32_t b_lo = __builtin_amdgcn_readlane((int)(uint32_t)tab_bs, gi), b_hi = __builtin_amdgcn_readlane((int)(uint32_t)((unsigned long long)tab_bs >> 32), gi);
@@ -263,8 +274,11 @@
 #endif
             if constexpr (!RW) {
 #pragma unroll
-                for (int i = 0; i < Cfg::NWL; ++i)
-                    __builtin_amdgcn_global_load_lds((kgptr_t)(wbase + w_voff[i]), (klptr_t)(stage + w_blk[i] * 1024), 16, 0, 0);
+                for (int i = 0; i < Cfg::NWL; ++i) {
+                    uint32_t voff = w_voff[i];
+                    if constexpr (RS) voff = rs_fill ? w_voff_rs[i] : voff;
+                    __builtin_amdgcn_global_load_lds((kgptr_t)(wbase + voff), (klptr_t)(stage + w_blk[i] * 1024), 16, 0, 0);
+                }
             }
 #pragma unroll
             for (int i = 0; i < Cfg::NXI; ++i)
@@ -619,6 +633,59 @@
             spk_step_pattern_n<N_MFMA, N_DS, N_TAIL, 0>(s + PD < SPK_STEPS);
         }
     };
+    auto steps_rs = [&]() __attribute__((always_inline)) {
+        constexpr int NP = ROWS;
+        static_assert(ROWS == 1 || ROWS == 2, "row parities of a consumer wave");
+        const int py0 = ROWS == 1 ? (cw & 1) : 0;
+        const unsigned char* sb = smem + st_cur * Cfg::STAGE + py0 * (Cfg::IW * 16);
+        const unsigned char* win = smem + st_cur * Cfg::STAGE + py0 * (SPK_RS_STEPS * NMT * 2 * 1024) + lane * 16;
+        h8 bh[2][NQ], bl[2][NQ], ah[2][NP][NMT], al[NP][NMT];
+        auto tap_off = [&](int s) {
+            const int tA = 2 * s, tB = 2 * s + 1;
+            const int offA = ((tA / 3) * Cfg::IW + tA % 3) * 16, offB = ((tB / 3) * Cfg::IW + tB % 3) * 16;
+            return tap_sel ? offB : offA;
+        };
+        auto par = [](int q) { return ROWS == 1 ? 0 : q / CB; };
+        auto ld = [&](int buf, int s) {
+            const int toff = tap_off(s);
+#pragma unroll
+            for (int q = 0; q < NQ; ++q) bh[buf][q] = *reinterpret_cast<const h8*>(sb + boff[q] + par(q) * (Cfg::IW * 16) + toff);
+#pragma unroll
+            for (int p = 0; p < NP; ++p)
+#pragma unroll
+                for (int m = 0; m < NMT; ++m) ah[buf][p][m] = *reinterpret_cast<const h8*>(win + (((p * SPK_RS_STEPS + s) * NMT + m) * 2 + 0) * 1024);
+#pragma unroll
+            for (int q = 0; q < NQ; ++q) bl[buf][q] = *reinterpret_cast<const h8*>(sb + 2 * Cfg::PLANE + boff[q] + par(q) * (Cfg::IW * 16) + toff);
+        };
+        auto ld_al = [&](int s) {
+#pragma unroll
+            for (int p = 0; p < NP; ++p)
+#pragma unroll
+                for (int m = 0; m < NMT; ++m) al[p][m] = *reinterpret_cast<const h8*>(win + (((p * SPK_RS_STEPS + s) * NMT + m) * 2 + 1) * 1024);
+        };
+        constexpr int N_MFMA = NQ * 3 * NMT, N_DS = 2 * NQ + 2 * NMT * NP;
+        constexpr int N_TAIL = N_MFMA >= 12 ? 4 : (N_MFMA >= 6 ? 2 : 0);
+        ld(0, 0);
+        ld_al(0);
+        __builtin_amdgcn_sched_barrier(0);
+#pragma unroll
+        for (int s = 0; s < SPK_RS_STEPS; ++s) {
+            if (s > 0) ld_al(s);
+            if (s + 1 < SPK_RS_STEPS) ld((s + 1) & 1, s + 1);
+#pragma unroll
+            for (int term = 0; term < 3; ++term)
+#pragma unroll
+                for (int m = 0; m < NMT; ++m)
+#pragma unroll
+                    for (int q = 0; q < NQ; ++q) {
+                        const h8 av = term == 2 ? al[par(q)][m] : ah[s & 1][par(q)][m];
+                        const h8 bv = term == 1 ? bl[s & 1][q] : bh[s & 1][q];
+                        acc[m][q] = __builtin_amdgcn_mfma_f32_16x16x32_f16(av, bv, acc[m][q], 0, 0, 0);
+                    }
+            spk_step_pattern_n<N_MFMA, N_DS, N_TAIL, 0>(s + 1 < SPK_RS_STEPS);
+        }
+    };
+    const int rs_mask_c = RS ? a.rs_mask : 0;
     int g = 0;
 #ifdef RING_STAMPS
     unsigned long long c0 = 0, c1 = 0, c2 = 0;
@@ -657,7 +724,11 @@
         const bool last = cur_c == n_chunks - 1;
         if constexpr (HAS_RES) { if (last) residual_prefetch(); }
         iter_begin();
-        steps();
+        if constexpr (RS) {
+            if ((rs_mask_c >> cur_c) & 1) steps_rs(); else steps();
+        } else {
+            steps();
+        }
         iter_end();
         if (last) {
             if constexpr (HAS_RES) __builtin_amdgcn_s_waitcnt(0x0F70);
@@ -1206,14 +1277,14 @@
 static int g_ring_consumers = 8;
 FLDR_HOOK int fldr_debug_ring_consumers(int v) { if (v == 4 || v == 8) g_ring_consumers = v; return g_ring_consumers; }
 
-template <int NMT, int TERMS, bool HAS_RES, int NC, int TW, bool RW = false>
+template <int NMT, int TERMS, bool HAS_RES, int NC, int TW, bool RW = false, bool RS = false>
 static int ring_launch3(SpkArgs& a, int N, int wgs_per_xcd_max, hipStream_t s, int walk_h) {
-    using Cfg = RingCfg<NMT, TW, RW>;
+    using Cfg = RingCfg<NMT, TW, RW, RS>;
     static std::atomic<uint64_t> attr_done{0};
-    if (int e = fldr_set_max_lds(reinterpret_cast<const void*>(&conv3x3_ring_kernel<NMT, TERMS, HAS_RES, NC, TW, false, RW>), Cfg::LDS_BYTES, attr_done)) return e;
+    if (int e = fldr_set_max_lds(reinterpret_cast<const void*>(&conv3x3_ring_kernel<NMT, TERMS, HAS_RES, NC, TW, false, RW, RS>), Cfg::LDS_BYTES, attr_done)) return e;
     if (int e = spk_fill_geometry(a, N, wgs_per_xcd_max, TW, walk_h)) return e;
     a.spin_limit = g_ring_spin_limit;
-    hipLaunchKernelGGL((conv3x3_ring_kernel<NMT, TERMS, HAS_RES, NC, TW, false, RW>), dim3(8 * a.wgs_per_xcd), dim3((NC + RING_NLOAD) * 64), Cfg::LDS_BYTES, s, a);
+    hipLaunchKernelGGL((conv3x3_ring_kernel<NMT, TERMS, HAS_RES, NC, TW, false, RW, RS>), dim3(8 * a.wgs_per_xcd), dim3((NC + RING_NLOAD) * 64), Cfg::LDS_BYTES, s, a);
     FLDR_LAUNCH_RET();
 }
 
@@ -1243,6 +1314,15 @@
 
 template <int NMT, int TERMS, bool HAS_RES>
 static int ring_launch2(SpkArgs& a, int N, int wpx, hipStream_t s, int walk_h) {
+    if constexpr (NMT <= 2 && TERMS == 3 && !HAS_RES) {
+        if (a.rs_mask) {
+            const int64_t units = (int64_t)N * fldr_cdiv(a.W, SPK_TW) * fldr_cdiv(walk_h, SPK_TH) * a.groups;
+            if (g_ring_consumers == 4 || (NMT == 1 && g_ring_tile_width == 0 && units >= 32ll * wpx))
+                return ring_launch3<NMT, TERMS, HAS_RES, 4, 32, false, true>(a, N, wpx, s, walk_h);
+            if (ring_pick_tile_width(a, N, wpx, walk_h) == 16) return ring_launch3<NMT, TERMS, HAS_RES, 8, 16, false, true>(a, N, wpx, s, walk_h);
+            return ring_launch3<NMT, TERMS, HAS_RES, 8, 32, false, true>(a, N, wpx, s, walk_h);
+        }
+    }
 #ifdef FLDR_TEST_HOOKS
     if constexpr (NMT == 1 && TERMS == 3) {
         if (g_ring_resident && a.n_chunks <= RING_RW_MAX_CHUNKS && g_ring_tile_width != 16) {
diff --git a/fldr-vfi_amd/csrc/conv_spk_kernels.hip b/fldr-vfi_amd/csrc/conv_spk_kernels.hip
--- a/fldr-vfi_amd/csrc/conv_spk_kernels.hip
+++ b/fldr-vfi_amd/csrc/conv_spk_kernels.hip
@@ -13,6 +13,7 @@
 
 #include "spk_common.h"
 #include <mutex>
+#include <cstring>
 
 #ifdef FLDR_TEST_HOOKS
 template <int NMT, int TERMS, bool HAS_RES>
@@ -551,9 +552,58 @@
     reinterpret_cast<h8*>(dst)[i] = v;
 }
 
+static __host__ __device__ inline void spk_rs_record(const float* __restrict__ w, float scale, int cout, int cin, int nmt, int64_t i, _Float16* v) {
+    const int lane = (int)(i % 64), kind = (int)((i / 64) % 2), m = (int)((i / 128) % nmt);
+    const int s = (int)((i / (128 * nmt)) % SPK_RS_STEPS), py = (int)((i / (128 * nmt * SPK_RS_STEPS)) % 2);
+    const int ch = (int)(i / ((int64_t)128 * nmt * SPK_RS_STEPS * 2));
+    const int li = lane & 15, lg = lane >> 4;
+    const int co = m * 16 + li;
+    const int t = 2 * s + (lg >> 1), rp = t / 3, dx = t % 3;
+    const int dy_a = py == 0 ? (rp == 0 ? 0 : 1) : (rp == 0 ? 0 : 2), dy_b = py == 0 ? (rp == 0 ? -1 : 2) : (rp == 0 ? 1 : -1);
+    for (int j = 0; j < 8; ++j) {
+        const int c = ch * 16 + (lg & 1) * 8 + j;
+        float x = 0.0f;
+        if (co < cout && c < cin) {
+            const float* wt = w + ((int64_t)co * cin + c) * 9;
+            const float sum = dy_b < 0 ? wt[dy_a * 3 + dx] : (float)((double)wt[dy_a * 3 + dx] + (double)wt[dy_b * 3 + dx]);
+            x = sum * scale;
+        }
+        const _Float16 h = (_Float16)x;
+        v[j] = kind == 0 ? h : (_Float16)(x - (float)h);
+    }
+}
+__global__ void spk_prepack_rs_kernel(const float* __restrict__ w, const float* __restrict__ hdr, float* __restrict__ dst, int cout, int cin, int nmt,
+                                      int64_t total_h8) {
+    const int64_t i = (int64_t)blockIdx.x * 256 + threadIdx.x;
+    if (i >= total_h8) return;
+    _Float16 r[8];
+    spk_rs_record(w, hdr[1], cout, cin, nmt, i, r);
+    h8 v;
+#pragma unroll
+    for (int j = 0; j < 8; ++j) v[j] = r[j];
+    reinterpret_cast<h8*>(dst)[i] = v;
+}
+FLDR_HOOK int64_t fldr_debug_spk_rowsum_pack_halves(int cout, int cin) {
+    if (cout <= 0 || cin <= 0 || cout > 96 || cin > SPK_MAX_GROUPS * 8) return FLDR_E_ARG;
+    return spk_rs_section_floats(cout, cin) * 2;
+}
+FLDR_HOOK int fldr_debug_spk_rowsum_pack_host(const float* weight, float scale, unsigned short* out, int cout, int cin) {
+    FLDR_CHECK_ARG(weight && out);
+    const int64_t n = fldr_debug_spk_rowsum_pack_halves(cout, cin);
+    if (n < 0) return (int)n;
+    int nmt, groups;
+    spk_geometry(cout, nmt, groups);
+    for (int64_t i = 0; i < n / 8; ++i) {
+        _Float16 r[8];
+        spk_rs_record(weight, scale, cout, cin, nmt, i, r);
+        memcpy(out + i * 8, r, 16);
+    }
+    return 0;
+}
+
 extern "C" int64_t fldr_conv_spk_prepack_size(int cout, int cin) {
     if (cout <= 0 || cin <= 0 || cout > 96 || cin > SPK_MAX_GROUPS * 8) return FLDR_E_ARG;
-    return SPK_HDR + spk_first_section_floats(cout, cin) + spk_r32_section_floats(cout, cin);
+    return SPK_HDR + spk_first_section_floats(cout, cin) + spk_r32_section_floats(cout, cin) + spk_rs_section_floats(cout, cin);
 }
 
 extern "C" int fldr_conv_spk_prepack(const float* weight, float* wpack, int cout, int cin, fldr_stream_t stream) {
@@ -572,6 +622,11 @@
         hipLaunchKernelGGL(spk_prepack32_kernel, dim3(fldr_cdiv(r_h8, 256)), dim3(256), 0, fldr_s(stream), weight, wpack, wpack + SPK_HDR + first,
                            cout, cin, n_chunks, r_h8);
     }
+    if (spk_has_rs_section(cout, cin)) {
+        const int64_t s_h8 = spk_rs_section_floats(cout, cin) / 4;
+        hipLaunchKernelGGL(spk_prepack_rs_kernel, dim3(fldr_cdiv(s_h8, 256)), dim3(256), 0, fldr_s(stream), weight, wpack,
+                           wpack + SPK_HDR + first + spk_r32_section_floats(cout, cin), cout, cin, nmt, s_h8);
+    }
     FLDR_LAUNCH_RET();
 }
 
@@ -581,6 +636,13 @@
 FLDR_HOOK int fldr_debug_spk_wgs_per_xcd(int v) { if (v > 0) g_spk_wgs_per_xcd = v; return g_spk_wgs_per_xcd; }
 static int g_spk_variant = 1;
 FLDR_HOOK int fldr_debug_spk_variant(int v) { if (v >= 0) g_spk_variant = v; return g_spk_variant; }
+#ifdef FLDR_TEST_HOOKS
+#define SPK_ROWSUM_DEFAULT 0
+#else
+#define SPK_ROWSUM_DEFAULT 1
+#endif
+static int g_spk_rowsum = SPK_ROWSUM_DEFAULT;
+FLDR_HOOK int fldr_debug_spk_rowsum(int v) { if (v == 0 || v == 1) g_spk_rowsum = v; return g_spk_rowsum; }
 
 #ifdef FLDR_TEST_HOOKS
 template <int NMT, int TERMS, bool HAS_RES>
@@ -611,9 +673,11 @@
     SpkArgs a;
     a.res_spk = (d->precision & 2) ? 1 : 0;
     int gsum = 0, csum = 0;
+    bool up2_whole_chunks = true;
     for (int s = 0; s < d->n_src; ++s) {
         FLDR_CHECK_ARG(d->src[s] && d->src_c[s] > 0);
         if (d->src_up2[s] && ((d->H | d->W) & 1)) return FLDR_E_SHAPE;
+        if (d->src_up2[s] && ((csum | d->src_c[s]) & 15)) up2_whole_chunks = false;
         if (s + 1 < d->n_src && (d->src_c[s] & 7)) return FLDR_E_SHAPE;
         const int ng = (d->src_c[s] + 7) / 8;
         if (gsum + ng > SPK_MAX_GROUPS) return FLDR_E_ARG;
@@ -636,6 +700,12 @@
     spk_geometry(d->cout, nmt, groups);
     a.groups = groups; a.pack_nmt = nmt;
     a.w32_off = spk_has_r32_section(d->cout) ? (SPK_HDR + spk_first_section_floats(d->cout, d->cin)) * 4 : 0;
+    a.wrs_off = (SPK_HDR + spk_first_section_floats(d->cout, d->cin) + spk_r32_section_floats(d->cout, d->cin)) * 4;
+    a.rs_mask = 0; a.pad3 = 0;
+    if (g_spk_rowsum && g_spk_variant == 1 && !(d->precision & 1) && !d->residual && up2_whole_chunks && spk_has_rs_section(d->cout, d->cin)) {
+        for (int c = 0; 2 * c + 1 < gsum; ++c)
+            if ((a.grp_ptr[2 * c] & 1ull) && (a.grp_ptr[2 * c + 1] & 1ull)) a.rs_mask |= 1 << c;
+    }
     if (nmt > 1) {
         const int64_t units = (int64_t)d->N * fldr_cdiv(d->W, SPK_TW) * fldr_cdiv(walk_h, SPK_TH) * groups;
         if (units <= g_spk_small_units) { a.groups = (d->cout + 15) / 16; nmt = 1; }
@@ -687,7 +757,7 @@
     a.out_spk = reinterpret_cast<unsigned char*>(d->out_spk);
     a.out_spk_bstride = fldr_spk_bytes(d->cout_store, d->H, d->W);
     a.n_chunks = d->cin / 16; a.cout = d->cout; a.cout_store = d->cout_store;
-    a.H = d->H; a.W = d->W; a.relu = d->relu; a.pack_nmt = 0; a.w32_off = 0;
+    a.H = d->H; a.W = d->W; a.relu = d->relu; a.pack_nmt = 0; a.w32_off = 0; a.wrs_off = 0; a.rs_mask = 0; a.pad3 = 0;
     return fldr_spk_ringrow_dispatch(a, wrow, d->N, g_spk_wgs_per_xcd, fldr_s(stream));
 }
 #endif
@@ -712,7 +782,7 @@
     a.H = d0.H; a.W = d0.W; a.relu = d0.relu;
     int nmt, groups;
     spk_geometry(d0.cout, nmt, groups);
-    a.groups = groups; a.pack_nmt = nmt; a.w32_off = 0;
+    a.groups = groups; a.pack_nmt = nmt; a.w32_off = 0; a.wrs_off = 0; a.rs_mask = 0; a.pad3 = 0;
     a.n_levels = n_levels;
     int64_t units = 0;
     for (int l = 0; l < n_levels; ++l) {
diff --git a/fldr-vfi_amd/csrc/spk_common.h b/fldr-vfi_amd/csrc/spk_common.h
--- a/fldr-vfi_amd/csrc/spk_common.h
+++ b/fldr-vfi_amd/csrc/spk_common.h
@@ -18,6 +18,7 @@
 #define SPK_PLANE 5632
 #define SPK_IN_BYTES (4 * SPK_PLANE)
 #define SPK_STEPS 5
+#define SPK_RS_STEPS 3
 #define SPK_HDR 8
 
 struct SpkArgs {
@@ -45,6 +46,8 @@
     } lv[SPK_MAX_LEVELS];
     uint32_t m_groups, m_tiles, m_tiles_x;
     int64_t w32_off;
+    int64_t wrs_off;
+    int32_t rs_mask, pad3;
 };
 
 static inline void spk_geometry(int cout, int& nmt, int& groups) {
@@ -61,6 +64,12 @@
 }
 static inline bool spk_has_r32_section(int cout) { return cout == 64 || cout == 96; }
 static inline int64_t spk_r32_section_floats(int cout, int cin) { return spk_has_r32_section(cout) ? (int64_t)(cout / 32) * ((cin + 15) / 16) * 18 * 256 : 0; }
+static inline bool spk_has_rs_section(int cout, int cin) { return cout <= 32 && cin >= 16; }
+static inline int64_t spk_rs_section_floats(int cout, int cin) {
+    int nmt, groups;
+    spk_geometry(cout, nmt, groups);
+    return spk_has_rs_section(cout, cin) ? (int64_t)((cin + 15) / 16) * 2 * SPK_RS_STEPS * nmt * 2 * 64 * 4 : 0;
+}
 
 template <int NMT>
 struct SpkCfg {
diff --git a/fldr-vfi_amd/fldr_hip.py b/fldr-vfi_amd/fldr_hip.py
--- a/fldr-vfi_amd/fldr_hip.py
+++ b/fldr-vfi_amd/fldr_hip.py
@@ -167,6 +167,9 @@
     "fldr_ring_status": (ctypes.c_int, [ctypes.c_int]),
     "fldr_debug_spk_small_units": (ctypes.c_int, [ctypes.c_int]),
     "fldr_debug_spk_variant": (ctypes.c_int, [ctypes.c_int]),
+    "fldr_debug_spk_rowsum": (ctypes.c_int, [ctypes.c_int]),
+    "fldr_debug_spk_rowsum_pack_halves": (ctypes.c_int64, [ctypes.c_int] * 2),
+    "fldr_debug_spk_rowsum_pack_host": (ctypes.c_int, [ctypes.c_void_p, ctypes.c_float, ctypes.c_void_p, ctypes.c_int, ctypes.c_int]),
     "fldr_debug_ring_consumers": (ctypes.c_int, [ctypes.c_int]),
     "fldr_debug_ring32": (ctypes.c_int, [ctypes.c_int]),
     "fldr_debug_ring_resident": (ctypes.c_int, [ctypes.c_int]),
@@ -285,7 +288,8 @@
             _hooks_lib = _load(os.environ.get("FLDR_LIB") or TEST_LIB_PATH, want_hooks=True)
             for env, hook in (("FLDR_RING_CONSUMERS", "fldr_debug_ring_consumers"), ("FLDR_SPK_VARIANT", "fldr_debug_spk_variant"),
                               ("FLDR_PCA_WORKGROUPS", "fldr_debug_pca_workgroups"), ("FLDR_PCA_VARIANT", "fldr_debug_pca_variant"),
-                              ("FLDR_RING_TILE_WIDTH", "fldr_debug_ring_tile_width"), ("FLDR_S2_VEC4", "fldr_debug_s2_vec4")):
+                              ("FLDR_RING_TILE_WIDTH", "fldr_debug_ring_tile_width"), ("FLDR_S2_VEC4", "fldr_debug_s2_vec4"),
+                              ("FLDR_SPK_ROWSUM", "fldr_debug_spk_rowsum")):
                 if os.environ.get(env) and hasattr(_hooks_lib, hook):
                     getattr(_hooks_lib, hook)(int(os.environ[env]))
         self._prev = _lib
diff --git a/include/fldr_hip_test_hooks.h b/include/fldr_hip_test_hooks.h
--- a/include/fldr_hip_test_hooks.h
+++ b/include/fldr_hip_test_hooks.h
@@ -16,6 +16,9 @@
 FLDR_API int fldr_debug_spk_small_units(int v);
 FLDR_API int fldr_debug_spk_wgs_per_xcd(int v);
 FLDR_API int fldr_debug_spk_variant(int v);
+FLDR_API int fldr_debug_spk_rowsum(int v);
+FLDR_API int64_t fldr_debug_spk_rowsum_pack_halves(int cout, int cin);
+FLDR_API int fldr_debug_spk_rowsum_pack_host(const float* weight, float scale, unsigned short* out, int cout, int cin);
 FLDR_API int fldr_debug_ring_resident(int v);
 FLDR_API int fldr_debug_ring32(int v);
 FLDR_API int fldr_debug_ring_consumers(int v);
```

Result: no change. 547.1 frame-pairs/s (median of 3 runs) (+0.7%).
